# zamling/PSALM

Hardware: AMD Instinct MI355X
Metric: images/sec at 1024x1024 COCO-panoptic inference (higher is better)
Workload: dtype f16x3; 1 GPU; BASELINE.json configs[1]: COCO-panoptic 1024x1024 batch=1 per GPU, PSALM (Swin-B + Phi-1.5 24L + Mask2Former head), 134 class prompts, 100 queries, full semantic+instance+panoptic post-processing; parallelism=image-sharded x1 (replicated weights, RCCL broadcast at init), launch=hipGraph replay (one graph per input signature)

## Files before the change

### include/psalm_hip.h

```cpp
#ifndef PSALM_HIP_H
#define PSALM_HIP_H
#include <stdint.h>
#ifdef __cplusplus
extern "C" {
#endif

#define PSALM_F32 0
#define PSALM_BF16 1

const char* psalm_last_error(void);
#define PSALM_ABI_VERSION 18
int psalm_abi_version(void);
const char* psalm_backend(void);

#define PSALM_TUNE_GEMM_XCD_KSPLIT 0
#define PSALM_TUNE_ATTN_XCD_HEADS 1
#define PSALM_TUNE_GEMM_MID 2
#define PSALM_TUNE_DECODER_FUSE 3
#define PSALM_TUNE_ROW_GROUPS 4
#define PSALM_TUNE_MHA_QTILE_WAVES 5
#define PSALM_TUNE_PHI_ROPE_EPILOGUE 6
#define PSALM_TUNE_COUNT 8
int psalm_set_tuning(int key, int value);
int psalm_get_tuning(int key);

int psalm_msda_forward(const void* value, int value_dtype, const int64_t* spatial_shapes_host,
                       const int64_t* level_start_host, const float* sampling_loc, const float* attn_weight, void* out,
                       int out_dtype, int B, int S, int M, int D, int L, int Lq, int P, void* stream);
int psalm_msda_forward_dev(const void* value, int value_dtype, const int64_t* spatial_shapes_dev, const int64_t* level_start_dev,
                           const float* sampling_loc, const float* attn_weight, void* out, int out_dtype, int B, int S, int M, int D,
                           int L, int Lq, int P, void* stream);


int psalm_msda_fused(const void* value, int value_dtype, const int64_t* spatial_shapes_host,
                     const int64_t* level_start_host, const float* offsets_logits, void* out, int out_dtype, int B, int S,
                     int M, int D, int L, int P, void* stream);
int psalm_msda_set_policy(int v);


int psalm_gemm(const void* A, int a_dtype, long lda, const void* W, int w_dtype, long ldw, const float* bias,
               const void* residual, long ldr, void* C, int c_dtype, long ldc, int M, int N, int K, int act,
               int act_col_start, void* workspace, long workspace_bytes, void* stream);

int psalm_gemm_ln(const void* A, int a_dtype, long lda, const void* W, int w_dtype, long ldw, const float* bias,
                  const void* residual, long ldr, void* C, int c_dtype, long ldc, int M, int N, int K, int act, int act_col_start,
                  const float* ln_gamma, const float* ln_beta, float ln_eps, void* ln_out, int ln_dtype, long ld_ln, void* workspace,
                  long workspace_bytes, void* stream);
int psalm_conv2d_nhwc(const void* x, int B, int H, int W, int Cin, const void* Wt, int Cout, int ksize, int stride, int pad,
                      const float* bias, const void* residual, long ldr, void* out, int c_dtype, long ldc, int act,
                      const void* zeros, void* workspace, long workspace_bytes, void* stream);
int psalm_split_f16(const float* x, long ldx, void* out, long ldo, float* inv_scale, int rows, int K, void* stream);
int psalm_gemm_x3_set_products(int n);
int psalm_im2col_split_f16(const float* x, void* out, float* inv_scale, int B, int H, int W, int C, int k, int stride, int pad, void* stream);
int psalm_layernorm_split(const float* x, long ldx, float* y, long ldy, const float* gamma, const float* beta, int rows, int C, float eps,
                          void* split1, float* inv1, const float* add, long add_rows, void* split2, float* inv2, void* stream);
int psalm_swin_window_gather_split(const float* x, void* out, float* inv_out, const float* gamma, const float* beta, int B, int H, int W, int C,
                                   int ws, int shift, float eps, void* stream);
int psalm_swin_window_merge_ln_split(const float* win, const float* shortcut, float* out_x, void* h_split, float* h_inv, const float* gamma,
                                     const float* beta, int B, int H, int W, int C, int ws, int shift, float eps, void* stream);
int psalm_gemm_x3(const void* A2, long lda, const float* a_scale, const void* W2, long ldw, const float* w_scale, int Kp,
                  const float* bias, const void* residual, long ldr, void* C, long ldc, int M, int N, int act, int act_col_start,
                  void* workspace, long workspace_bytes, void* stream);
int psalm_gemm_x3_ln_split(const void* A2, long lda, const float* a_scale, const void* W2, long ldw, const float* w_scale, int Kp,
                           const float* bias, const void* residual, long ldr, void* C, long ldc, int M, int N, const float* ln_gamma,
                           const float* ln_beta, float ln_eps, void* ln_out, long ld_ln, void* split_out, float* split_inv,
                           void* workspace, long workspace_bytes, void* stream);
int psalm_gemm_x3_split(const void* A2, long lda, const float* a_scale, const void* W2, long ldw, const float* w_scale, int Kp,
                        const float* bias, void* C, long ldc, int M, int N, int act, int act_col_start, void* split_out, long ld_split,
                        int split_kp, int split_col_off, int split_col_start, int paired, float* split_inv, const float* bound_par,
                        int global_rows, void* workspace, long workspace_bytes, void* stream);
typedef struct psalm_rope_out {
    float* Qr;
    float* Kr;
    const float* cos_table;
    const float* sin_table;
    int q_col, k_col, heads, B, L, Lp;
    float scale;
    int pad_;
} psalm_rope_out;
int psalm_gemm_x3_split_rope(const void* A2, long lda, const float* a_scale, const void* W2, long ldw, const float* w_scale, int Kp,
                             const float* bias, void* C, long ldc, int M, int N, int act, int act_col_start, void* split_out, long ld_split,
                             int split_kp, int split_col_off, int split_col_start, int paired, float* split_inv, const float* bound_par,
                             int global_rows, const psalm_rope_out* rope, void* workspace, long workspace_bytes, void* stream);

int psalm_image_preprocess(const unsigned char* img, int H, int W, float* out, unsigned char* pad_mask, int S, int nh, int nw,
                           const int* bounds_h, const int* kk_h, int ksize_h, const int* bounds_v, const int* kk_v, int ksize_v,
                           unsigned char* tmp, const float* mean3_host, const float* std3_host, void* stream);

int psalm_semantic_labels(const float* sem, int* labels, int C, long HW, void* stream);
int psalm_confusion_accumulate(const int* pred, const int* gt, long n, int num_classes, int ignore_label, long long* conf, void* stream);
int psalm_panoptic_rgb(const int* ids, unsigned char* rgb, long n, void* stream);
int psalm_mask_rle_count(const void* masks, int dtype_is_u8, int n, int H, int W, int* col_cnt, int* col_off, int* total, void* stream);
int psalm_mask_rle_emit(const void* masks, int dtype_is_u8, int n, int H, int W, const int* col_off, const long* base, int* out, void* stream);
int psalm_iou_counts(const void* pred, int pred_is_u8, const unsigned char* tgt, const int* pred_idx, const int* tgt_idx, int npairs, long HW,
                     long long* counts_zeroed, void* stream);
int psalm_fuse_masks(const void* masks, int dtype_is_u8, const float* scores, int n, long HW, float thr, unsigned char* out, void* stream);

long psalm_mha_attention_f32_workspace(int B, int heads, int Lq, int Lk);
int psalm_mha_attention_f32(const float* q, long ldq, const float* k, long ldk, const float* v, long ldv, float* out, long ldo,
                            const unsigned char* mask, const unsigned char* row_all_masked, void* workspace, int B, int Lq, int Lk, int heads,
                            int head_dim, void* stream);
long psalm_mha_attention_f32_shared_workspace(int B, int heads, int Lq, int Lk);
int psalm_mha_attention_f32_shared(const float* q, long ldq, const float* k, long ldk, const float* v, long ldv, float* out, long ldo,
                                   const unsigned char* mask, const unsigned char* row_all_masked, void* workspace, int B, int Lq, int Lk,
                                   int heads, int head_dim, void* stream);

long psalm_causal_attention_f32_workspace(int B, int L, int heads);
int psalm_causal_attention_f32(const float* qkv, long ld, int q_off, int k_off, int v_off, float* out, long ldo, int o_off,
                               const float* cos_table, const float* sin_table, const unsigned char* key_mask, void* workspace, int B, int L,
                               int heads, int head_dim, int rot, void* stream);
int psalm_causal_attention_f32_split(const float* qkv, long ld, int q_off, int k_off, int v_off, void* split_out, long ld_split, int split_kp,
                                     int split_col_off, const float* split_inv, const float* cos_table, const float* sin_table,
                                     const unsigned char* key_mask, void* workspace, int B, int L, int heads, int head_dim, int rot,
                                     void* stream);
int psalm_phi_attention_tables(const unsigned char* key_mask, void* workspace, int B, int L, int heads, void* stream);
int psalm_causal_attention_f32_split_prepared(const float* qkv, long ld, int v_off, void* split_out, long ld_split, int split_kp,
                                              int split_col_off, const float* split_inv, void* workspace, int B, int L, int heads,
                                              int head_dim, void* stream);

long psalm_causal_attention_f32_prefix_workspace(int N, int S, int heads);
int psalm_causal_attention_f32_prefix(const float* qkv, long ld, int q_off, int k_off, int v_off, const float* k_cache, const float* v_cache,
                                      long ldv, float* out, long ldo, int o_off, const float* cos_table, const float* sin_table,
                                      const unsigned char* key_mask, void* workspace, int N, int S, int P, int heads, int head_dim, int rot,
                                      void* stream);
int psalm_causal_attention_f32_prefix_split(const float* qkv, long ld, int q_off, int k_off, int v_off, const float* k_cache,
                                            const float* v_cache, long ldv, void* split_out, long ld_split, int split_kp, int split_col_off,
                                            const float* split_inv, const float* cos_table, const float* sin_table,
                                            const unsigned char* key_mask, void* workspace, int N, int S, int P, int heads, int head_dim,
                                            int rot, void* stream);
typedef struct {
    const float* k_cache;
    const float* v_cache;
    long ldv;
    int P;
    int pad;
} psalm_prefix_ref;
long psalm_causal_attention_f32_prefix_grouped_workspace(int N, int S, int heads);
int psalm_causal_attention_f32_prefix_grouped(const float* qkv, long ld, int q_off, int k_off, int v_off, const psalm_prefix_ref* refs, int P_max,
                                              float* out, long ldo, int o_off, const float* cos_table, const float* sin_table,
                                              const unsigned char* key_mask, void* workspace, int N, int S, int heads, int head_dim, int rot,
                                              void* stream);
int psalm_causal_attention_f32_prefix_grouped_split(const float* qkv, long ld, int q_off, int k_off, int v_off, const psalm_prefix_ref* refs,
                                                    int P_max, void* split_out, long ld_split, int split_kp, int split_col_off,
                                                    const float* split_inv, const float* cos_table, const float* sin_table,
                                                    const unsigned char* key_mask, void* workspace, int N, int S, int heads, int head_dim,
                                                    int rot, void* stream);
int psalm_phi_prefix_kv_store(const float* qkv, long ld, int k_off, int v_off, const float* cos_table, const float* sin_table, float* k_cache,
                              float* v_cache, long ldv, int P, int heads, int head_dim, int rot, void* stream);

int psalm_memset_zero(void* p, long bytes, void* stream);
int psalm_copy_d2d(void* dst, const void* src, long bytes, void* stream);
int psalm_cast_i32_i64(const int* src, long long* dst, long n, void* stream);
const char* psalm_gemm_last_kernel(void);
int psalm_gemm_describe(int M, int N, int K, int a_dtype, int w_dtype, long workspace_bytes, int* out4);
int psalm_gemm_set_tile_policy(int bm);

int psalm_layernorm(const void* x, int x_dtype, long ldx, void* y, int y_dtype, long ldy, void* y2_bf16, long ldy2,
                    const float* gamma, const float* beta, int rows, int C, float eps, void* stream);
int psalm_layernorm3(const void* x, int x_dtype, long ldx, void* y, int y_dtype, long ldy, void* y2_bf16, long ldy2, const float* add,
                     long add_rows, void* y3_bf16, long ldy3, const float* gamma, const float* beta, int rows, int C, float eps,
                     void* stream);
int psalm_layernorm_chain(const float* x, long ldx, float* y1, long ldy1, const float* g1, const float* b1, const float* add, long add_rows,
                          float* y2, long ldy2, const float* g2, const float* b2, float* y3, long ldy3, int rows, int C, float eps, void* stream);
int psalm_gemm_f32_pair(const float* A0, const float* W0, const float* bias0, float* C0, int M0, int N0, int K0, int act0, const float* A1,
                        const float* W1, const float* bias1, float* C1, int M1, int N1, int K1, int act1, void* stream);
int psalm_gemm_f32_rows(const float* A, long lda, const float* W, long ldw, const float* bias, const float* residual, long ldr, float* C, long ldc,
                        int M, int N, int K, int act, void* stream);
int psalm_gemm_f32_rows_pair(const float* A0, const float* W0, const float* bias0, float* C0, int M0, int N0, int K0, int act0, const float* A1,
                             const float* W1, const float* bias1, float* C1, int M1, int N1, int K1, int act1, void* stream);
int psalm_gemm_f32_grouped(const float* const* A_host, const float* const* W_host, float* const* C_host, const int* M_host, const int* N_host, int K,
                           int count, void* stream);
int psalm_swin_window_gather(const void* x, int x_dtype, void* out, int out_dtype, const float* gamma,
                             const float* beta, int B, int H, int W, int C, int ws, int shift, float eps, void* stream);
int psalm_swin_window_merge(const void* win, int win_dtype, const void* shortcut, void* out, int x_dtype, int B, int H,
                            int W, int C, int ws, int shift, void* stream);
int psalm_swin_window_merge_ln(const void* win, int win_dtype, const float* shortcut, float* out_x, void* out_h, int h_dtype,
                               const float* gamma, const float* beta, int B, int H, int W, int C, int ws, int shift, float eps,
                               void* stream);
int psalm_patch_merge_ln(const void* x, int x_dtype, void* out, int out_dtype, const float* gamma, const float* beta,
                         int B, int H, int W, int C, float eps, void* stream);
int psalm_groupnorm_nhwc(const void* x, int x_dtype, void* y, int y_dtype, const float* gamma, const float* beta,
                         float* workspace, int B, int HW, int C, int G, float eps, int relu, void* stream);
int psalm_add_bcast(const void* a, int a_dtype, const void* b, int b_dtype, void* out, int out_dtype, long rows, int C,
                    long b_rows, void* stream);
int psalm_gather_rows(const void* src0, int dt0, const void* src1, int dt1, const void* src2, int dt2, const void* src3,
                      int dt3, const int* src_id, const int* src_row, void* dst, int dst_dtype, long rows, int C,
                      void* stream);
int psalm_segment_mean(const void* x, int x_dtype, long ldx, const int* seg_offsets, const int* seg_rows, void* out,
                       int out_dtype, int nseg, int C, void* stream);

// ... 255 lines not shown
```

### psalm_amd/csrc/api.hip

```cpp
#include "common.h"
#include "psalm_hip.h"

#include <atomic>
#include <cstring>

static thread_local char g_err[512] = "";

extern "C" void psalm_set_error(const char* msg) {
    strncpy(g_err, msg ? msg : "", sizeof(g_err) - 1);
    g_err[sizeof(g_err) - 1] = 0;
}
extern "C" const char* psalm_last_error() { return g_err; }
static std::atomic<int> g_tuning[PSALM_TUNE_COUNT] = {{1}, {1}, {1}, {1}, {1}, {1}, {1}, {0}};
extern "C" int psalm_set_tuning(int key, int value) {
    if (key < 0 || key >= PSALM_TUNE_COUNT) { psalm_set_error("psalm_set_tuning: unknown key"); return -1; }
    g_tuning[key].store(value, std::memory_order_relaxed);
    return 0;
}
extern "C" int psalm_get_tuning(int key) {
    if (key < 0 || key >= PSALM_TUNE_COUNT) return 0;
    return g_tuning[key].load(std::memory_order_relaxed);
}
extern "C" int psalm_abi_version() { return PSALM_ABI_VERSION; }
extern "C" const char* psalm_backend() {
#ifdef PSALM_EMU_BUILD
    return "emu";
#else
    return "hip-gfx950";
#endif
}

extern "C" int psalm_memset_zero(void* p, long bytes, void* stream) {
    if (bytes <= 0) return 0;
    PSALM_CHECK_ARG(p != nullptr, "psalm_memset_zero: null pointer");
    hipError_t e = hipMemsetAsync(p, 0, (size_t)bytes, (hipStream_t)stream);
    if (e != hipSuccess) { psalm_set_error("psalm_memset_zero: hipMemsetAsync failed"); return (int)e; }
    return 0;
}
__global__ void cast_i32_i64_kernel(const int* __restrict__ src, long long* __restrict__ dst, long n) {
    const long i = (long)blockIdx.x * blockDim.x + threadIdx.x;
    if (i < n) dst[i] = (long long)src[i];
}
extern "C" int psalm_cast_i32_i64(const int* src, long long* dst, long n, void* stream) {
    if (n <= 0) return 0;
    PSALM_CHECK_ARG(dst != nullptr && src != nullptr, "psalm_cast_i32_i64: null pointer");
    hipLaunchKernelGGL(cast_i32_i64_kernel, dim3((unsigned)((n + 255) / 256)), dim3(256), 0, (hipStream_t)stream, src, dst, n);
    PSALM_LAUNCH_END("psalm_cast_i32_i64");
}
extern "C" int psalm_copy_d2d(void* dst, const void* src, long bytes, void* stream) {
    if (bytes <= 0) return 0;
    PSALM_CHECK_ARG(dst != nullptr && src != nullptr, "psalm_copy_d2d: null pointer");
    hipError_t e = hipMemcpyAsync(dst, src, (size_t)bytes, hipMemcpyDeviceToDevice, (hipStream_t)stream);
    if (e != hipSuccess) { psalm_set_error("psalm_copy_d2d: hipMemcpyAsync failed"); return (int)e; }
    return 0;
}
```

### psalm_amd/csrc/common.h

```cpp
#pragma once
#include <hip/hip_runtime.h>

#include <cstdint>
#include <cstdio>

#define PSALM_F32 0
#define PSALM_BF16 1

typedef unsigned short bf16_t;

__device__ __forceinline__ float bf16_to_f32(bf16_t v) {
    unsigned u = ((unsigned)v) << 16;
    return __builtin_bit_cast(float, u);
}
__device__ __forceinline__ bf16_t f32_to_bf16(float f) {
    unsigned u = __builtin_bit_cast(unsigned, f);
    u += 0x7fffu + ((u >> 16) & 1u);
    return (bf16_t)(u >> 16);
}
typedef float psalm_f32x2_v __attribute__((ext_vector_type(2)));
typedef __bf16 psalm_bf16x2_v __attribute__((ext_vector_type(2)));
__device__ __forceinline__ unsigned pack_bf16x2(float a, float b) {
    const psalm_f32x2_v v = {a, b};
    return __builtin_bit_cast(unsigned, __builtin_convertvector(v, psalm_bf16x2_v));
}
__device__ __forceinline__ float ldf(const float* p) { return *p; }
__device__ __forceinline__ float ldf(const bf16_t* p) { return bf16_to_f32(*p); }
__device__ __forceinline__ void stf(float* p, float v) { *p = v; }
__device__ __forceinline__ void stf(bf16_t* p, float v) { *p = f32_to_bf16(v); }

struct alignas(16) psalm_u32x4 { unsigned x, y, z, w; };
struct alignas(8) psalm_u32x2 { unsigned x, y; };
struct alignas(16) psalm_f32x4 { float x, y, z, w; };
__device__ __forceinline__ void ld8(const float* p, float* d) {
    const psalm_f32x4 a = reinterpret_cast<const psalm_f32x4*>(p)[0], b = reinterpret_cast<const psalm_f32x4*>(p)[1];
    d[0] = a.x; d[1] = a.y; d[2] = a.z; d[3] = a.w; d[4] = b.x; d[5] = b.y; d[6] = b.z; d[7] = b.w;
}
__device__ __forceinline__ void ld8(const bf16_t* p, float* d) {
    const psalm_u32x4 a = *reinterpret_cast<const psalm_u32x4*>(p);
    const unsigned w[4] = {a.x, a.y, a.z, a.w};
#pragma unroll
    for (int i = 0; i < 4; ++i) {
        d[2 * i] = __builtin_bit_cast(float, w[i] << 16);
        d[2 * i + 1] = __builtin_bit_cast(float, w[i] & 0xffff0000u);
    }
}
__device__ __forceinline__ void st8(float* p, const float* v) {
    reinterpret_cast<psalm_f32x4*>(p)[0] = psalm_f32x4{v[0], v[1], v[2], v[3]};
    reinterpret_cast<psalm_f32x4*>(p)[1] = psalm_f32x4{v[4], v[5], v[6], v[7]};
}
__device__ __forceinline__ void st8(bf16_t* p, const float* v) {
    *reinterpret_cast<psalm_u32x4*>(p) =
        psalm_u32x4{pack_bf16x2(v[0], v[1]), pack_bf16x2(v[2], v[3]), pack_bf16x2(v[4], v[5]), pack_bf16x2(v[6], v[7])};
}

__device__ __forceinline__ float wave_sum(float v) {
#pragma unroll
    for (int o = 32; o > 0; o >>= 1) v += __shfl_xor(v, o);
    return v;
}
__device__ __forceinline__ float wave_max(float v) {
#pragma unroll
    for (int o = 32; o > 0; o >>= 1) v = fmaxf(v, __shfl_xor(v, o));
    return v;
}

template <int LPR> __device__ __forceinline__ float seg_sum(float v) {
#pragma unroll
    for (int o = LPR / 2; o > 0; o >>= 1) v += __shfl_xor(v, o);
    return v;
}
template <int LPR> __device__ __forceinline__ float seg_max(float v) {
#pragma unroll
    for (int o = LPR / 2; o > 0; o >>= 1) v = fmaxf(v, __shfl_xor(v, o));
    return v;
}

#ifdef PSALM_EMU_BUILD
#define PSALM_WAVES_PER_EU(n)
#else
#define PSALM_WAVES_PER_EU(n) __attribute__((amdgpu_waves_per_eu(n)))
#endif
#ifdef PSALM_EMU_BUILD
__device__ __forceinline__ void psalm_glds16(const void* g, void* lds_wave_base) { emu::global_load_lds(g, lds_wave_base, 16); }
#else
__device__ __forceinline__ void psalm_glds16(const void* g, void* lds_wave_base) {
    __builtin_amdgcn_global_load_lds((const __attribute__((address_space(1))) void*)g,
                                     (__attribute__((address_space(3))) void*)lds_wave_base, 16, 0, 0);
}
#endif

#ifdef PSALM_EMU_BUILD
#define PSALM_WAIT_VMCNT(N) do { } while (0)
#define PSALM_RAW_BARRIER() __syncthreads()
#define PSALM_SCHED_FENCE() do { } while (0)
#define PSALM_OPAQUE_VGPR(x) do { } while (0)
#define PSALM_OPAQUE_SGPR(x) do { } while (0)
__device__ __forceinline__ float psalm_rcp(float x) { return 1.0f / x; }
__device__ __forceinline__ float psalm_exp2(float x) { return exp2f(x); }
#else
#define PSALM_OPAQUE_VGPR(x) asm volatile("" : "+v"(x))
#define PSALM_OPAQUE_SGPR(x) asm volatile("" : "+s"(x))
#define PSALM_WAIT_VMCNT(N) asm volatile("s_waitcnt vmcnt(" #N ")" ::: "memory")
#define PSALM_RAW_BARRIER() do { asm volatile("s_waitcnt lgkmcnt(0)" ::: "memory"); __builtin_amdgcn_s_barrier(); } while (0)
#define PSALM_SCHED_FENCE() __builtin_amdgcn_sched_barrier(0)
__device__ __forceinline__ float psalm_rcp(float x) { return __builtin_amdgcn_rcpf(x); }
__device__ __forceinline__ float psalm_exp2(float x) { return __builtin_amdgcn_exp2f(x); }
#endif

__device__ __forceinline__ void psalm_split_words(float y, unsigned& hw, unsigned& sw) {
    const _Float16 h = (_Float16)y;
    hw = (unsigned)__builtin_bit_cast(unsigned short, h);
    sw = (unsigned)__builtin_bit_cast(unsigned short, (_Float16)(y - (float)h));
}

#define PSALM_BUF_OOB 0x80000000u
#ifdef PSALM_EMU_BUILD
__device__ __forceinline__ unsigned psalm_swap_adjacent(unsigned v) { return __shfl_xor(v, 1); }
__device__ __forceinline__ unsigned psalm_quad_swap2(unsigned v) { return __shfl_xor(v, 2); }
__device__ __forceinline__ unsigned psalm_swap_row16(unsigned v) { return __shfl_xor(v, 16); }
template <int P> __device__ __forceinline__ unsigned psalm_quad_bcast(unsigned v) { return __shfl(v, ((threadIdx.x & 63) & ~3) | P); }
struct psalm_rsrc { char* base; unsigned bytes; };
__device__ __forceinline__ psalm_rsrc psalm_make_rsrc(const void* p, unsigned bytes) { return psalm_rsrc{(char*)p, bytes}; }
__device__ __forceinline__ void psalm_buf_store_f32(float v, psalm_rsrc r, unsigned off) { if (off < r.bytes && r.bytes - off >= 4u) *reinterpret_cast<float*>(r.base + off) = v; }
__device__ __forceinline__ void psalm_buf_store_u32(unsigned v, psalm_rsrc r, unsigned off) { if (off < r.bytes && r.bytes - off >= 4u) *reinterpret_cast<unsigned*>(r.base + off) = v; }
__device__ __forceinline__ float psalm_buf_load_f32(psalm_rsrc r, unsigned off) { return (off < r.bytes && r.bytes - off >= 4u) ? *reinterpret_cast<const float*>(r.base + off) : 0.f; }
__device__ __forceinline__ psalm_u32x4 psalm_buf_load_b128(psalm_rsrc r, unsigned off) {
    return (off < r.bytes && r.bytes - off >= 16u) ? *reinterpret_cast<const psalm_u32x4*>(r.base + off) : psalm_u32x4{0u, 0u, 0u, 0u};
}
__device__ __forceinline__ void psalm_buf_store_f32_s(float v, psalm_rsrc r, unsigned voff, unsigned soff) { if (voff < PSALM_BUF_OOB) psalm_buf_store_f32(v, r, voff + soff); }
__device__ __forceinline__ float psalm_buf_load_f32_s(psalm_rsrc r, unsigned voff, unsigned soff) { return voff < PSALM_BUF_OOB ? psalm_buf_load_f32(r, voff + soff) : 0.f; }
__device__ __forceinline__ psalm_u32x4 psalm_buf_load_b128_s(psalm_rsrc r, unsigned voff, unsigned soff) {
    return voff < PSALM_BUF_OOB ? psalm_buf_load_b128(r, voff + soff) : psalm_u32x4{0u, 0u, 0u, 0u};
}
#else
__device__ __forceinline__ unsigned psalm_swap_adjacent(unsigned v) {
    return (unsigned)__builtin_amdgcn_mov_dpp((int)v, 0xB1, 0xF, 0xF, true);
}
__device__ __forceinline__ unsigned psalm_quad_swap2(unsigned v) {
    return (unsigned)__builtin_amdgcn_mov_dpp((int)v, 0x4E, 0xF, 0xF, true);
}
__device__ __forceinline__ unsigned psalm_swap_row16(unsigned v) { return (unsigned)__builtin_amdgcn_ds_swizzle((int)v, 0x401F); }
template <int P> __device__ __forceinline__ unsigned psalm_quad_bcast(unsigned v) {
    return (unsigned)__builtin_amdgcn_mov_dpp((int)v, P * 0x55, 0xF, 0xF, true);
}
typedef __amdgpu_buffer_rsrc_t psalm_rsrc;
__device__ __forceinline__ psalm_rsrc psalm_make_rsrc(const void* p, unsigned bytes) {
    return __builtin_amdgcn_make_buffer_rsrc(const_cast<void*>(p), 0, (int)bytes, 0x00020000);
}
__device__ __forceinline__ void psalm_buf_store_f32(float v, psalm_rsrc r, unsigned off) {
    __builtin_amdgcn_raw_buffer_store_b32(__builtin_bit_cast(unsigned, v), r, (int)off, 0, 0);
}
__device__ __forceinline__ void psalm_buf_store_u32(unsigned v, psalm_rsrc r, unsigned off) { __builtin_amdgcn_raw_buffer_store_b32(v, r, (int)off, 0, 0); }
__device__ __forceinline__ float psalm_buf_load_f32(psalm_rsrc r, unsigned off) {
    return __builtin_bit_cast(float, __builtin_amdgcn_raw_buffer_load_b32(r, (int)off, 0, 0));
}
typedef unsigned psalm_u32x4_v __attribute__((ext_vector_type(4)));
__device__ __forceinline__ psalm_u32x4 psalm_buf_load_b128(psalm_rsrc r, unsigned off) {
    const psalm_u32x4_v v = __builtin_amdgcn_raw_buffer_load_b128(r, (int)off, 0, 0);
    return psalm_u32x4{v.x, v.y, v.z, v.w};
}
__device__ __forceinline__ void psalm_buf_store_f32_s(float v, psalm_rsrc r, unsigned voff, unsigned soff) {
    __builtin_amdgcn_raw_buffer_store_b32(__builtin_bit_cast(unsigned, v), r, (int)voff, (int)soff, 0);
}
__device__ __forceinline__ float psalm_buf_load_f32_s(psalm_rsrc r, unsigned voff, unsigned soff) {
    return __builtin_bit_cast(float, __builtin_amdgcn_raw_buffer_load_b32(r, (int)voff, (int)soff, 0));
}
__device__ __forceinline__ psalm_u32x4 psalm_buf_load_b128_s(psalm_rsrc r, unsigned voff, unsigned soff) {
    const psalm_u32x4_v v = __builtin_amdgcn_raw_buffer_load_b128(r, (int)voff, (int)soff, 0);
    return psalm_u32x4{v.x, v.y, v.z, v.w};
}
#endif

__device__ __forceinline__ float psalm_rope_elem(float x, float xo, float cs, float sn, bool neg, bool fused) {
#pragma clang fp contract(off)
    const float t = (neg ? -xo : xo) * sn;
    const float p = x * cs;
    return fused ? fmaf(x, cs, t) : p + t;
}
__device__ __forceinline__ bool psalm_rope_fused_dim(int c) { return (c & 7) < 6; }

extern "C" void psalm_set_error(const char* msg);
extern "C" int psalm_get_tuning(int key);
#ifndef PSALM_TUNE_COUNT
#define PSALM_TUNE_GEMM_XCD_KSPLIT 0
#define PSALM_TUNE_ATTN_XCD_HEADS 1
#define PSALM_TUNE_GEMM_MID 2
#define PSALM_TUNE_DECODER_FUSE 3
#define PSALM_TUNE_ROW_GROUPS 4
#define PSALM_TUNE_MHA_QTILE_WAVES 5
#define PSALM_TUNE_PHI_ROPE_EPILOGUE 6
#define PSALM_TUNE_COUNT 8
#endif

#define PSALM_CHECK_ARG(cond, msg)                                  \
    do {                                                            \
        if (!(cond)) { psalm_set_error(msg); return -1; }           \
    } while (0)

#define PSALM_LAUNCH_END(name)                                      \
    do {                                                            \
        hipError_t e__ = hipGetLastError();                         \
        if (e__ != hipSuccess) {                                    \
            char buf__[256];                                        \
            snprintf(buf__, sizeof(buf__), "%s: launch failed: %s", name, hipGetErrorString(e__)); \
            psalm_set_error(buf__);                                 \
            return (int)e__ ? (int)e__ : -2;                        \
        }                                                           \
        return 0;                                                   \
    } while (0)

#define PSALM_DISPATCH(code, T, ...)                                \
    do {                                                            \
        if ((code) == PSALM_F32) { typedef float T; __VA_ARGS__; }  \
        else if ((code) == PSALM_BF16) { typedef bf16_t T; __VA_ARGS__; } \
        else { psalm_set_error("bad dtype code"); return -1; }      \
    } while (0)

static inline int cdiv(long a, long b) { return (int)((a + b - 1) / b); }
```

### psalm_amd/csrc/msda.hip

```cpp
#include "common.h"
#include <atomic>

struct alignas(16) f32x4_s { float x, y, z, w; };
struct alignas(8) bf16x4_s { bf16_t x, y, z, w; };

__device__ __forceinline__ f32x4_s ld4(const float* p) { return *reinterpret_cast<const f32x4_s*>(p); }
__device__ __forceinline__ f32x4_s ld4(const bf16_t* p) {
    bf16x4_s v = *reinterpret_cast<const bf16x4_s*>(p);
    return f32x4_s{bf16_to_f32(v.x), bf16_to_f32(v.y), bf16_to_f32(v.z), bf16_to_f32(v.w)};
}
__device__ __forceinline__ void st4(float* p, f32x4_s v) { *reinterpret_cast<f32x4_s*>(p) = v; }
__device__ __forceinline__ void st4(bf16_t* p, f32x4_s v) {
    *reinterpret_cast<bf16x4_s*>(p) = bf16x4_s{f32_to_bf16(v.x), f32_to_bf16(v.y), f32_to_bf16(v.z), f32_to_bf16(v.w)};
}

template <int V> struct msda_ic { static constexpr int value = V; };
#define MSDA_MAX_LEVELS 8
struct MsdaLevels {
    int H[MSDA_MAX_LEVELS], W[MSDA_MAX_LEVELS], start[MSDA_MAX_LEVELS];
};

template <typename TV>
__device__ __forceinline__ void msda_sample(const TV* __restrict__ vbase, int Hl, int Wl, int row_stride, float loc_x,
                                            float loc_y, float wgt, f32x4_s& acc) {
    const float h_im = loc_y * Hl - 0.5f;
    const float w_im = loc_x * Wl - 0.5f;
    const bool inb = h_im > -1.f && w_im > -1.f && h_im < (float)Hl && w_im < (float)Wl;
    const int h_low = (int)floorf(inb ? h_im : 0.f), w_low = (int)floorf(inb ? w_im : 0.f);
    const float lh = h_im - h_low, lw = w_im - w_low;
    const float hh = 1.f - lh, hw = 1.f - lw;
    const bool h0 = h_low >= 0, h1 = h_low + 1 <= Hl - 1, w0 = w_low >= 0, w1 = w_low + 1 <= Wl - 1;
    const int ha = max(h_low, 0), hb = min(h_low + 1, Hl - 1), wa = max(w_low, 0), wb = min(w_low + 1, Wl - 1);
    const f32x4_s v1 = ld4(vbase + ((long)ha * Wl + wa) * row_stride);
    const f32x4_s v2 = ld4(vbase + ((long)ha * Wl + wb) * row_stride);
    const f32x4_s v3 = ld4(vbase + ((long)hb * Wl + wa) * row_stride);
    const f32x4_s v4 = ld4(vbase + ((long)hb * Wl + wb) * row_stride);
    const float w1c = (inb && h0 && w0) ? hh * hw : 0.f, w2c = (inb && h0 && w1) ? hh * lw : 0.f;
    const float w3c = (inb && h1 && w0) ? lh * hw : 0.f, w4c = (inb && h1 && w1) ? lh * lw : 0.f;
    const float wg = inb ? wgt : 0.f;
    acc.x += wg * (w1c * v1.x + w2c * v2.x + w3c * v3.x + w4c * v4.x);
    acc.y += wg * (w1c * v1.y + w2c * v2.y + w3c * v3.y + w4c * v4.y);
    acc.z += wg * (w1c * v1.z + w2c * v2.z + w3c * v3.z + w4c * v4.z);
    acc.w += wg * (w1c * v1.w + w2c * v2.w + w3c * v3.w + w4c * v4.w);
}

template <typename TV>
struct MsdaTaps8 {
    const TV* p[4];
    float w[4];
};
template <typename TV>
__device__ __forceinline__ MsdaTaps8<TV> msda_taps8(const TV* __restrict__ vbase, int Hl, int Wl, int row_stride, float loc_x, float loc_y) {
    const float h_im = loc_y * Hl - 0.5f;
    const float w_im = loc_x * Wl - 0.5f;
    const bool inb = h_im > -1.f && w_im > -1.f && h_im < (float)Hl && w_im < (float)Wl;
    const int h_low = (int)floorf(inb ? h_im : 0.f), w_low = (int)floorf(inb ? w_im : 0.f);
    const float lh = h_im - h_low, lw = w_im - w_low;
    const float hh = 1.f - lh, hw = 1.f - lw;
    const bool h0 = h_low >= 0, h1 = h_low + 1 <= Hl - 1, w0 = w_low >= 0, w1 = w_low + 1 <= Wl - 1;
    const int ha = max(h_low, 0), hb = min(h_low + 1, Hl - 1), wa = max(w_low, 0), wb = min(w_low + 1, Wl - 1);
    MsdaTaps8<TV> t;
    t.p[0] = vbase + ((long)ha * Wl + wa) * row_stride;
    t.p[1] = vbase + ((long)ha * Wl + wb) * row_stride;
    t.p[2] = vbase + ((long)hb * Wl + wa) * row_stride;
    t.p[3] = vbase + ((long)hb * Wl + wb) * row_stride;
    t.w[0] = (inb && h0 && w0) ? hh * hw : 0.f;
    t.w[1] = (inb && h0 && w1) ? hh * lw : 0.f;
    t.w[2] = (inb && h1 && w0) ? lh * hw : 0.f;
    t.w[3] = (inb && h1 && w1) ? lh * lw : 0.f;
    return t;
}

template <typename TV, typename TO, int L, int P, bool XCD_BANDS = false, bool QUAD = false>
__global__ void __launch_bounds__(256) msda_fused8_kernel(const TV* __restrict__ value, MsdaLevels lv,
                                                          const float* __restrict__ ow, TO* __restrict__ out, int B, int S,
                                                          int M, int D) {
    const int G = D >> 3;
    const int Lq = S;
    const long total = (long)B * Lq * M * G;
    constexpr int LP = L * P;
    for (long idx0 = (long)blockIdx.x * blockDim.x + threadIdx.x; idx0 < total; idx0 += (long)gridDim.x * blockDim.x) {
        long idx = idx0;
        if constexpr (XCD_BANDS)
            idx = ((long)(blockIdx.x >> 3) * blockDim.x + threadIdx.x);
        const int g = (int)(idx % G);
        long t = idx / G;
        const int m = (int)(t % M);
        t /= M;
        int q = (int)(t % Lq);
        const int b = XCD_BANDS ? 0 : (int)(t / Lq);
        if constexpr (XCD_BANDS) {
            const int band = blockIdx.x & 7;
            int r = (int)t, lq_ = 0, base = 0;
#pragma unroll
            for (int l = 0; l < L; ++l) {
                const int nb = lv.H[l] * lv.W[l] / 8;
                if (l == lq_ && r >= nb && l + 1 < L) { r -= nb; ++lq_; }
            }
#pragma unroll
            for (int l = 0; l < L; ++l)
                if (l == lq_) base = lv.start[l] + band * (lv.H[l] * lv.W[l] / 8);
            q = base + r;
        }
        int lq = 0;
#pragma unroll
        for (int l = 1; l < L; ++l)
            if (q >= lv.start[l]) lq = l;
        const int qi = q - lv.start[lq];
        const float ref_x = ((qi % lv.W[lq]) + 0.5f) / lv.W[lq];
        const float ref_y = ((qi / lv.W[lq]) + 0.5f) / lv.H[lq];
        const float* row = ow + ((long)b * Lq + q) * (M * LP * 3);
        const float* offp = row + m * LP * 2;
        const float* lgp = row + M * LP * 2 + m * LP;
        const int row_stride = M * D;
        const TV* vb = value + (long)b * S * row_stride + m * D + g * 8;
        float acc[8];
#pragma unroll
        for (int k = 0; k < 8; ++k) acc[k] = 0.f;
        if constexpr (QUAD) {
            static_assert(P == 4, "one sampling point per lane of the quad");
            float lgq[L];
            float mx = -3.4e38f;
#pragma unroll
            for (int l = 0; l < L; ++l) { lgq[l] = lgp[l * P + g]; mx = fmaxf(mx, lgq[l]); }
            mx = fmaxf(mx, __builtin_bit_cast(float, psalm_swap_adjacent(__builtin_bit_cast(unsigned, mx))));
            mx = fmaxf(mx, __builtin_bit_cast(float, psalm_quad_swap2(__builtin_bit_cast(unsigned, mx))));
            float den = 0.f;
#pragma unroll
            for (int l = 0; l < L; ++l) { lgq[l] = __expf(lgq[l] - mx); den += lgq[l]; }
            den += __builtin_bit_cast(float, psalm_swap_adjacent(__builtin_bit_cast(unsigned, den)));
            den += __builtin_bit_cast(float, psalm_quad_swap2(__builtin_bit_cast(unsigned, den)));
            const float inv = 1.f / den;
            const psalm_rsrc vr = psalm_make_rsrc(value, (unsigned)((long)B * S * row_stride * (long)sizeof(TV)));
            const unsigned lane_b = (unsigned)(((long)b * S * row_stride + m * D + g * 8) * (long)sizeof(TV));
            auto fetch = [&](unsigned off, float* v8) {
                if constexpr (sizeof(TV) == 4) {
                    const psalm_u32x4 a = psalm_buf_load_b128(vr, lane_b + off), b2 = psalm_buf_load_b128(vr, lane_b + off + 16u);
                    v8[0] = __builtin_bit_cast(float, a.x); v8[1] = __builtin_bit_cast(float, a.y); v8[2] = __builtin_bit_cast(float, a.z);
                    v8[3] = __builtin_bit_cast(float, a.w); v8[4] = __builtin_bit_cast(float, b2.x); v8[5] = __builtin_bit_cast(float, b2.y);
                    v8[6] = __builtin_bit_cast(float, b2.z); v8[7] = __builtin_bit_cast(float, b2.w);
                } else {
                    const psalm_u32x4 a = psalm_buf_load_b128(vr, lane_b + off);
                    const unsigned w4[4] = {a.x, a.y, a.z, a.w};
#pragma unroll
                    for (int e = 0; e < 4; ++e) {
                        v8[2 * e] = __builtin_bit_cast(float, w4[e] << 16);
                        v8[2 * e + 1] = __builtin_bit_cast(float, w4[e] & 0xffff0000u);
                    }
                }
            };
#pragma unroll 1
            for (int l = 0; l < L; ++l) {
                int Hl = lv.H[0], Wl = lv.W[0], sl = lv.start[0];
                float lgl = lgq[0];
#pragma unroll
                for (int j = 1; j < L; ++j)
                    if (l == j) { Hl = lv.H[j]; Wl = lv.W[j]; sl = lv.start[j]; lgl = lgq[j]; }
                const int i = l * P + g;
                const float lx = ref_x + offp[2 * i] / Wl, ly = ref_y + offp[2 * i + 1] / Hl;
                const MsdaTaps8<TV> tp = msda_taps8<TV>(vb + (long)sl * row_stride, Hl, Wl, row_stride, lx, ly);
                const float wgt = lgl * inv;
                unsigned toff[4];
                float tw[4];
#pragma unroll
                for (int c = 0; c < 4; ++c) { toff[c] = (unsigned)((tp.p[c] - vb) * (long)sizeof(TV)); tw[c] = tp.w[c] * wgt; }
                auto pair = [&](auto PC0) {
                    constexpr int p0 = decltype(PC0)::value;
                    float w[2][4], v[2][4][8];
#pragma unroll
                    for (int c = 0; c < 4; ++c) {
                        fetch(psalm_quad_bcast<p0>(toff[c]), v[0][c]);
                        fetch(psalm_quad_bcast<p0 + 1>(toff[c]), v[1][c]);
                        w[0][c] = __builtin_bit_cast(float, psalm_quad_bcast<p0>(__builtin_bit_cast(unsigned, tw[c])));
                        w[1][c] = __builtin_bit_cast(float, psalm_quad_bcast<p0 + 1>(__builtin_bit_cast(unsigned, tw[c])));
                    }
#pragma unroll
                    for (int pp = 0; pp < 2; ++pp)
#pragma unroll
                        for (int k = 0; k < 8; ++k)
                            acc[k] += w[pp][0] * v[pp][0][k] + w[pp][1] * v[pp][1][k] + w[pp][2] * v[pp][2][k] + w[pp][3] * v[pp][3][k];
                };
                pair(msda_ic<0>{});
                pair(msda_ic<2>{});
            }
            static_assert(L <= 3, "levels of the quad form");
            st8(out + (((long)b * Lq + q) * M + m) * D + g * 8, acc);
            continue;
        }
        float lg[LP];
        float mx = -3.4e38f;
#pragma unroll
        for (int i = 0; i < LP; ++i) { lg[i] = lgp[i]; mx = fmaxf(mx, lg[i]); }
        float den = 0.f;
#pragma unroll
        for (int i = 0; i < LP; ++i) { lg[i] = __expf(lg[i] - mx); den += lg[i]; }
        const float inv = 1.f / den;
        constexpr int PB = (P % 2 == 0) ? 2 : 1;
#pragma unroll 1
        for (int l = 0; l < L; ++l) {
            int Hl = lv.H[0], Wl = lv.W[0], sl = lv.start[0];
#pragma unroll
            for (int j = 1; j < L; ++j)
                if (l == j) { Hl = lv.H[j]; Wl = lv.W[j]; sl = lv.start[j]; }
            const TV* vl = vb + (long)sl * row_stride;
#pragma unroll
            for (int p0 = 0; p0 < P; p0 += PB) {
                MsdaTaps8<TV> tp[PB];
                float v[PB][4][8];
#pragma unroll
                for (int pp = 0; pp < PB; ++pp) {
                    const int i = l * P + p0 + pp;
                    const float lx = ref_x + offp[2 * i] / Wl;
                    const float ly = ref_y + offp[2 * i + 1] / Hl;
                    tp[pp] = msda_taps8<TV>(vl, Hl, Wl, row_stride, lx, ly);
#pragma unroll
                    for (int c = 0; c < 4; ++c) ld8(tp[pp].p[c], v[pp][c]);
                }
                __builtin_amdgcn_sched_barrier(0);
#pragma unroll
                for (int pp = 0; pp < PB; ++pp) {
                    const float wgt = lg[l * P + p0 + pp] * inv;
#pragma unroll
                    for (int k = 0; k < 8; ++k)
                        acc[k] += wgt * (tp[pp].w[0] * v[pp][0][k] + tp[pp].w[1] * v[pp][1][k] + tp[pp].w[2] * v[pp][2][k] +
                                         tp[pp].w[3] * v[pp][3][k]);
                }
            }
        }
        st8(out + (((long)b * Lq + q) * M + m) * D + g * 8, acc);
    }
}

template <typename TV, typename TO, int LP_UNROLL, bool DEV = false>
__global__ void __launch_bounds__(256) msda_forward_kernel(const TV* __restrict__ value, MsdaLevels lv,
                                                           const float* __restrict__ loc, const float* __restrict__ attw,
                                                           TO* __restrict__ out, int B, int S, int M, int D, int L, int Lq,
                                                           int P, const long* __restrict__ shapes_dev = nullptr,
                                                           const long* __restrict__ starts_dev = nullptr) {
    const int G = D >> 2;
    const long total = (long)B * Lq * M * G;
    for (long idx = (long)blockIdx.x * blockDim.x + threadIdx.x; idx < total; idx += (long)gridDim.x * blockDim.x) {
        const int g = (int)(idx % G);
        long t = idx / G;
        const int m = (int)(t % M);
        t /= M;
        const int q = (int)(t % Lq);
        const int b = (int)(t / Lq);
        const long qm = ((long)b * Lq + q) * M + m;
        const float* lp = loc + qm * L * P * 2;
        const float* wp = attw + qm * L * P;
        const int row_stride = M * D;
        const TV* vb = value + (long)b * S * row_stride + m * D + g * 4;
        f32x4_s acc{0.f, 0.f, 0.f, 0.f};
        for (int l = 0; l < L; ++l) {
            const int Hl = DEV ? (int)shapes_dev[2 * l] : lv.H[l], Wl = DEV ? (int)shapes_dev[2 * l + 1] : lv.W[l];
            const long sl = DEV ? starts_dev[l] : (long)lv.start[l];
            if (DEV && !(Hl > 0 && Wl > 0 && sl >= 0 && sl + (long)Hl * Wl <= (long)S)) continue;
            const TV* vl = vb + sl * row_stride;
#pragma unroll LP_UNROLL
            for (int p = 0; p < P; ++p) {
                const int i = l * P + p;
                msda_sample<TV>(vl, Hl, Wl, row_stride, lp[2 * i], lp[2 * i + 1], wp[i], acc);
            }
        }
        st4(out + qm * D + g * 4, acc);
    }
}

template <typename TV, typename TO, int L, int P>
__global__ void __launch_bounds__(256) msda_fused_kernel(const TV* __restrict__ value, MsdaLevels lv,
                                                         const float* __restrict__ ow, TO* __restrict__ out, int B, int S,
                                                         int M, int D) {
    const int G = D >> 2;
    const int Lq = S;
    const long total = (long)B * Lq * M * G;
    constexpr int LP = L * P;
    for (long idx = (long)blockIdx.x * blockDim.x + threadIdx.x; idx < total; idx += (long)gridDim.x * blockDim.x) {
        const int g = (int)(idx % G);
        long t = idx / G;
        const int m = (int)(t % M);
        t /= M;
        const int q = (int)(t % Lq);
        const int b = (int)(t / Lq);
        int lq = 0;
#pragma unroll
        for (int l = 1; l < L; ++l)
            if (q >= lv.start[l]) lq = l;
        const int qi = q - lv.start[lq];
        const float ref_x = ((qi % lv.W[lq]) + 0.5f) / lv.W[lq];
        const float ref_y = ((qi / lv.W[lq]) + 0.5f) / lv.H[lq];
        const float* row = ow + ((long)b * Lq + q) * (M * LP * 3);
        const float* offp = row + m * LP * 2;
        const float* lgp = row + M * LP * 2 + m * LP;
        float lg[LP];
        float mx = -3.4e38f;
#pragma unroll
        for (int i = 0; i < LP; ++i) { lg[i] = lgp[i]; mx = fmaxf(mx, lg[i]); }
        float den = 0.f;
#pragma unroll
        for (int i = 0; i < LP; ++i) { lg[i] = __expf(lg[i] - mx); den += lg[i]; }
        const float inv = 1.f / den;
        const int row_stride = M * D;
        const TV* vb = value + (long)b * S * row_stride + m * D + g * 4;
        f32x4_s acc{0.f, 0.f, 0.f, 0.f};
#pragma unroll
        for (int l = 0; l < L; ++l) {
            const TV* vl = vb + (long)lv.start[l] * row_stride;
#pragma unroll
            for (int p = 0; p < P; ++p) {
                const int i = l * P + p;
                const float lx = ref_x + offp[2 * i] / lv.W[l];
                const float ly = ref_y + offp[2 * i + 1] / lv.H[l];
                msda_sample<TV>(vl, lv.H[l], lv.W[l], row_stride, lx, ly, lg[i] * inv, acc);
            }
        }
        st4(out + (((long)b * Lq + q) * M + m) * D + g * 4, acc);
    }
}

static std::atomic<int> g_msda_quad{1};
extern "C" int psalm_msda_set_policy(int v) {
    if (v != 0 && v != 1) { psalm_set_error("psalm_msda_set_policy: 0 / 1 (quad-shared taps off / on)"); return -1; }
    g_msda_quad = v;
    return 0;
}

static int fill_levels(MsdaLevels& lv, const int64_t* shapes, const int64_t* starts, int L, int S) {
    if (L > MSDA_MAX_LEVELS) return -1;
    long tot = 0;
    for (int l = 0; l < L; ++l) {
        lv.H[l] = (int)shapes[2 * l];
        lv.W[l] = (int)shapes[2 * l + 1];
        lv.start[l] = (int)starts[l];
        tot += (long)lv.H[l] * lv.W[l];
    }
    return tot == S ? 0 : -2;
}

extern "C" int psalm_msda_forward(const void* value, int value_dtype, const int64_t* spatial_shapes_host,
                                  const int64_t* level_start_host, const float* sampling_loc, const float* attn_weight,
                                  void* out, int out_dtype, int B, int S, int M, int D, int L, int Lq, int P, void* stream) {
    PSALM_CHECK_ARG(D % 4 == 0 && D > 0, "psalm_msda_forward: head dim must be a multiple of 4");
    MsdaLevels lv = {};
    int rc = fill_levels(lv, spatial_shapes_host, level_start_host, L, S);
    PSALM_CHECK_ARG(rc != -1, "psalm_msda_forward: too many levels (max 8)");
    PSALM_CHECK_ARG(rc == 0, "psalm_msda_forward: sum(H_l*W_l) != S");
    const long total = (long)B * Lq * M * (D / 4);
    if (total == 0) return 0;
    const int block = 256;
    const int grid = (int)((total + block - 1) / block < 65536 * 8 ? (total + block - 1) / block : 65536 * 8);
    PSALM_DISPATCH(value_dtype, TV, PSALM_DISPATCH(out_dtype, TO, {
        hipLaunchKernelGGL((msda_forward_kernel<TV, TO, 4>), dim3(grid), dim3(block), 0, (hipStream_t)stream,
                           (const TV*)value, lv, sampling_loc, attn_weight, (TO*)out, B, S, M, D, L, Lq, P);
    }));
    PSALM_LAUNCH_END("psalm_msda_forward");
}

extern "C" int psalm_msda_forward_dev(const void* value, int value_dtype, const int64_t* spatial_shapes_dev,
                                      const int64_t* level_start_dev, const float* sampling_loc, const float* attn_weight, void* out,
                                      int out_dtype, int B, int S, int M, int D, int L, int Lq, int P, void* stream) {
    PSALM_CHECK_ARG(D % 4 == 0 && D > 0, "psalm_msda_forward_dev: head dim must be a multiple of 4");
    PSALM_CHECK_ARG(L >= 1 && spatial_shapes_dev && level_start_dev, "psalm_msda_forward_dev: level table missing");
    MsdaLevels lv = {};
    const long total = (long)B * Lq * M * (D / 4);
    if (total == 0) return 0;
    const int block = 256;
    const int grid = (int)((total + block - 1) / block < 65536 * 8 ? (total + block - 1) / block : 65536 * 8);
    PSALM_DISPATCH(value_dtype, TV, PSALM_DISPATCH(out_dtype, TO, {
        hipLaunchKernelGGL((msda_forward_kernel<TV, TO, 4, true>), dim3(grid), dim3(block), 0, (hipStream_t)stream,
                           (const TV*)value, lv, sampling_loc, attn_weight, (TO*)out, B, S, M, D, L, Lq, P,
                           (const long*)spatial_shapes_dev, (const long*)level_start_dev);
    }));
    PSALM_LAUNCH_END("psalm_msda_forward_dev");
}

extern "C" int psalm_msda_fused(const void* value, int value_dtype, const int64_t* spatial_shapes_host,
                                const int64_t* level_start_host, const float* offsets_logits, void* out, int out_dtype,
                                int B, int S, int M, int D, int L, int P, void* stream) {
    PSALM_CHECK_ARG(D % 4 == 0 && D > 0, "psalm_msda_fused: head dim must be a multiple of 4");
    PSALM_CHECK_ARG(L == 3 && P == 4, "psalm_msda_fused: specialised for L=3 levels, P=4 points (PSALM pixel decoder)");
    MsdaLevels lv = {};
    int rc = fill_levels(lv, spatial_shapes_host, level_start_host, L, S);
    PSALM_CHECK_ARG(rc == 0, "psalm_msda_fused: bad level table");
    const int block = 256;
    if (D % 8 == 0 && (uintptr_t)value % 16 == 0 && (uintptr_t)out % 16 == 0) {
        const long total8 = (long)B * S * M * (D / 8);
        if (total8 == 0) return 0;
        bool bands = B == 1 && total8 % (block * 8) == 0;
        for (int l = 0; l < L; ++l) bands = bands && lv.H[l] % 8 == 0;
        const bool quad = g_msda_quad && D == 32 && value_dtype == PSALM_BF16 && (long)B * S * M * D * 2 < (1L << 31);
#define MSDA_LAUNCH8(BANDS_, QUAD_, GRID_)                                                                                              \
        PSALM_DISPATCH(value_dtype, TV, PSALM_DISPATCH(out_dtype, TO, {                                                                 \
            hipLaunchKernelGGL((msda_fused8_kernel<TV, TO, 3, 4, BANDS_, QUAD_>), dim3((unsigned)(GRID_)), dim3(block), 0,              \
                               (hipStream_t)stream, (const TV*)value, lv, offsets_logits, (TO*)out, B, S, M, D);                        \
        }))
        if (bands) {
            if (quad) MSDA_LAUNCH8(true, true, total8 / block); else MSDA_LAUNCH8(true, false, total8 / block);
            PSALM_LAUNCH_END("psalm_msda_fused");
        }
        if (quad) MSDA_LAUNCH8(false, true, (total8 + block - 1) / block); else MSDA_LAUNCH8(false, false, (total8 + block - 1) / block);
#undef MSDA_LAUNCH8
        PSALM_LAUNCH_END("psalm_msda_fused");
    }
    const long total = (long)B * S * M * (D / 4);
    if (total == 0) return 0;
    const int grid = (int)((total + block - 1) / block);
    PSALM_DISPATCH(value_dtype, TV, PSALM_DISPATCH(out_dtype, TO, {
        hipLaunchKernelGGL((msda_fused_kernel<TV, TO, 3, 4>), dim3(grid), dim3(block), 0, (hipStream_t)stream,
                           (const TV*)value, lv, offsets_logits, (TO*)out, B, S, M, D);
    }));
    PSALM_LAUNCH_END("psalm_msda_fused");
}
```

### psalm_amd/csrc/rowops.hip

```cpp
#include "common.h"
#include <type_traits>

__device__ __forceinline__ void emit_split8(const float* o8, float sc, unsigned short* hi_dst, unsigned short* lo_dst) {
    unsigned hw[4], lw[4];
#pragma unroll
    for (int k = 0; k < 4; ++k) {
        unsigned h0, h1, l0, l1;
        psalm_split_words(o8[2 * k] * sc, h0, l0);
        psalm_split_words(o8[2 * k + 1] * sc, h1, l1);
        hw[k] = h0 | (h1 << 16);
        lw[k] = l0 | (l1 << 16);
    }
    *reinterpret_cast<psalm_u32x4*>(hi_dst) = psalm_u32x4{hw[0], hw[1], hw[2], hw[3]};
    *reinterpret_cast<psalm_u32x4*>(lo_dst) = psalm_u32x4{lw[0], lw[1], lw[2], lw[3]};
}
__device__ __forceinline__ void split_scale(float amax, float& sc, float& inv) {
    int e = (int)((__builtin_bit_cast(unsigned, amax) >> 23) & 0xffu) - 127;
    int se = 13 - e;
    se = se > 100 ? 100 : (se < -100 ? -100 : se);
    const bool zero = !(amax > 0.f) || !(amax < 3.0e38f);
    sc = zero ? 1.f : __builtin_bit_cast(float, (unsigned)(127 + se) << 23);
    inv = zero ? 1.f : __builtin_bit_cast(float, (unsigned)(127 - se) << 23);
}
template <typename TI>
__device__ __forceinline__ void row_stats(const TI* __restrict__ x, int C, int lane, float eps, float& mean, float& rstd) {
    float s = 0.f;
    for (int c = lane; c < C; c += 64) s += ldf(x + c);
    mean = wave_sum(s) / C;
    float v = 0.f;
    for (int c = lane; c < C; c += 64) { const float d = ldf(x + c) - mean; v += d * d; }
    rstd = rsqrtf(wave_sum(v) / C + eps);
}

template <typename TI, typename TO>
__global__ void __launch_bounds__(256) layernorm_kernel(const TI* __restrict__ x, long ldx, TO* __restrict__ y, long ldy,
                                                        bf16_t* __restrict__ y2, long ldy2, const float* __restrict__ add, long add_rows,
                                                        bf16_t* __restrict__ y3, long ldy3, const float* __restrict__ gamma,
                                                        const float* __restrict__ beta, int rows, int C, float eps) {
    const int lane = threadIdx.x & 63;
    const long row = (long)blockIdx.x * 4 + (threadIdx.x >> 6);
    if (row >= rows) return;
    const TI* xr = x + row * ldx;
    float mean, rstd;
    row_stats(xr, C, lane, eps, mean, rstd);
    TO* yr = y + row * ldy;
    for (int c = lane; c < C; c += 64) {
        const float v = (ldf(xr + c) - mean) * rstd * gamma[c] + beta[c];
        stf(yr + c, v);
        if (y2) y2[row * ldy2 + c] = f32_to_bf16(v);
        if (y3) y3[row * ldy3 + c] = f32_to_bf16(v + add[(row % add_rows) * C + c]);
    }
}

template <typename TI, typename TO>
__global__ void __launch_bounds__(256) layernorm_vec_kernel(const TI* __restrict__ x, long ldx, TO* __restrict__ y, long ldy,
                                                            bf16_t* __restrict__ y2, long ldy2, const float* __restrict__ add,
                                                            long add_rows, bf16_t* __restrict__ y3, long ldy3,
                                                            const float* __restrict__ gamma, const float* __restrict__ beta, int rows,
                                                            int C, float eps) {
    const int lane = threadIdx.x & 63;
    const long row = (long)blockIdx.x * 4 + (threadIdx.x >> 6);
    if (row >= rows) return;
    const TI* xr = x + row * ldx;
    float v[4][8];
    float s = 0.f;
#pragma unroll
    for (int i = 0; i < 4; ++i) {
        const int c = (i * 64 + lane) * 8;
        if (c < C) {
            ld8(xr + c, v[i]);
#pragma unroll
            for (int k = 0; k < 8; ++k) s += v[i][k];
        }
    }
    const float mean = wave_sum(s) / C;
    float q = 0.f;
#pragma unroll
    for (int i = 0; i < 4; ++i) {
        const int c = (i * 64 + lane) * 8;
        if (c < C) {
#pragma unroll
            for (int k = 0; k < 8; ++k) { const float d = v[i][k] - mean; q += d * d; }
        }
    }
    const float rstd = rsqrtf(wave_sum(q) / C + eps);
#pragma unroll
    for (int i = 0; i < 4; ++i) {
        const int c = (i * 64 + lane) * 8;
        if (c < C) {
            float g8[8], b8[8], o8[8];
            ld8(gamma + c, g8);
            ld8(beta + c, b8);
#pragma unroll
            for (int k = 0; k < 8; ++k) o8[k] = (v[i][k] - mean) * rstd * g8[k] + b8[k];
            st8(y + row * ldy + c, o8);
            if (y2) st8(y2 + row * ldy2 + c, o8);
            if (y3) {
                float a8[8];
                ld8(add + (row % add_rows) * C + c, a8);
#pragma unroll
                for (int k = 0; k < 8; ++k) o8[k] += a8[k];
                st8(y3 + row * ldy3 + c, o8);
            }
        }
    }
}

extern "C" int psalm_layernorm3(const void* x, int x_dtype, long ldx, void* y, int y_dtype, long ldy, void* y2_bf16, long ldy2,
                                const float* add, long add_rows, void* y3_bf16, long ldy3, const float* gamma, const float* beta,
                                int rows, int C, float eps, void* stream) {
    if (rows == 0) return 0;
    const long xs = x_dtype == PSALM_F32 ? 4 : 2, ys = y_dtype == PSALM_F32 ? 4 : 2;
    PSALM_CHECK_ARG(!y3_bf16 || (add && add_rows > 0), "psalm_layernorm3: y3 needs the `add` table");
    const bool vec = C % 8 == 0 && C <= 2048 && (uintptr_t)x % 16 == 0 && (ldx * xs) % 16 == 0 && (uintptr_t)y % 16 == 0 &&
                     (ldy * ys) % 16 == 0 && (uintptr_t)gamma % 16 == 0 && (uintptr_t)beta % 16 == 0 &&
                     (!y2_bf16 || ((uintptr_t)y2_bf16 % 16 == 0 && (ldy2 * 2) % 16 == 0)) &&
                     (!y3_bf16 || ((uintptr_t)y3_bf16 % 16 == 0 && (ldy3 * 2) % 16 == 0 && (uintptr_t)add % 16 == 0));
    PSALM_DISPATCH(x_dtype, TI, PSALM_DISPATCH(y_dtype, TO, {
        if (vec)
            hipLaunchKernelGGL((layernorm_vec_kernel<TI, TO>), dim3(cdiv(rows, 4)), dim3(256), 0, (hipStream_t)stream,
                               (const TI*)x, ldx, (TO*)y, ldy, (bf16_t*)y2_bf16, ldy2, add, add_rows, (bf16_t*)y3_bf16, ldy3, gamma, beta,
                               rows, C, eps);
        else
            hipLaunchKernelGGL((layernorm_kernel<TI, TO>), dim3(cdiv(rows, 4)), dim3(256), 0, (hipStream_t)stream,
                               (const TI*)x, ldx, (TO*)y, ldy, (bf16_t*)y2_bf16, ldy2, add, add_rows, (bf16_t*)y3_bf16, ldy3, gamma, beta,
                               rows, C, eps);
    }));
    PSALM_LAUNCH_END("psalm_layernorm");
}

__global__ void __launch_bounds__(256) layernorm_chain_kernel(const float* __restrict__ x, long ldx, float* __restrict__ y1, long ldy1,
                                                              const float* __restrict__ g1, const float* __restrict__ b1,
                                                              const float* __restrict__ add, long add_rows, float* __restrict__ y2, long ldy2,
                                                              const float* __restrict__ g2, const float* __restrict__ b2, float* __restrict__ y3,
                                                              long ldy3, int rows, int C, float eps) {
    const int lane = threadIdx.x & 63;
    const long row = (long)blockIdx.x * 4 + (threadIdx.x >> 6);
    if (row >= rows) return;
    const float* xr = x + row * ldx;
    float v[4][8];
    auto stats = [&](float& mean, float& rstd) {
        float s = 0.f;
#pragma unroll
        for (int i = 0; i < 4; ++i) {
            const int c = (i * 64 + lane) * 8;
            if (c < C) {
#pragma unroll
                for (int k = 0; k < 8; ++k) s += v[i][k];
            }
        }
        mean = wave_sum(s) / C;
        float q = 0.f;
#pragma unroll
        for (int i = 0; i < 4; ++i) {
            const int c = (i * 64 + lane) * 8;
            if (c < C) {
#pragma unroll
                for (int k = 0; k < 8; ++k) { const float d = v[i][k] - mean; q += d * d; }
            }
        }
        rstd = rsqrtf(wave_sum(q) / C + eps);
    };
#pragma unroll
    for (int i = 0; i < 4; ++i) {
        const int c = (i * 64 + lane) * 8;
        if (c < C) ld8(xr + c, v[i]);
    }
    float mean, rstd;
    stats(mean, rstd);
#pragma unroll
    for (int i = 0; i < 4; ++i) {
        const int c = (i * 64 + lane) * 8;
        if (c < C) {
            float g8[8], b8[8];
            ld8(g1 + c, g8);
            ld8(b1 + c, b8);
// ... 386 lines not shown
}
extern "C" int psalm_swin_window_gather_split(const float* x, void* out, float* inv_out, const float* gamma, const float* beta, int B, int H,
                                              int W, int C, int ws, int shift, float eps, void* stream) {
    const long rows = (long)B * ((H + ws - 1) / ws) * ((W + ws - 1) / ws) * ws * ws;
    if (rows == 0) return 0;
    PSALM_CHECK_ARG(C % 8 == 0 && C <= 2048 && (uintptr_t)x % 16 == 0 && (uintptr_t)out % 16 == 0, "psalm_swin_window_gather_split: C % 8 == 0, C <= 2048, aligned");
#define WGS_LAUNCH(LPR_) hipLaunchKernelGGL((swin_window_gather_split_kernel<LPR_>), dim3(cdiv(rows, 4 * (64 / LPR_))), dim3(256), 0, (hipStream_t)stream, x, \
                                            (unsigned short*)out, inv_out, gamma, beta, B, H, W, C, ws, shift, eps, (C + 63) / 64 * 64)
    const int lpr = !psalm_get_tuning(PSALM_TUNE_ROW_GROUPS) ? 64 : (C <= 128 ? 16 : (C <= 256 ? 32 : 64));
    if (lpr == 16) WGS_LAUNCH(16); else if (lpr == 32) WGS_LAUNCH(32); else WGS_LAUNCH(64);
#undef WGS_LAUNCH
    PSALM_LAUNCH_END("psalm_swin_window_gather_split");
}

template <typename TI, typename TO>
__global__ void __launch_bounds__(256) patch_merge_ln_kernel(const TI* __restrict__ x, TO* __restrict__ out,
                                                             const float* __restrict__ gamma, const float* __restrict__ beta,
                                                             int B, int H, int W, int C, float eps) {
    const int lane = threadIdx.x & 63;
    const int H2 = (H + 1) / 2, W2 = (W + 1) / 2;
    const long rows = (long)B * H2 * W2;
    const long r = (long)blockIdx.x * 4 + (threadIdx.x >> 6);
    if (r >= rows) return;
    const int x2 = (int)(r % W2), y2 = (int)((r / W2) % H2), b = (int)(r / ((long)W2 * H2));
    const int C4 = 4 * C;
    auto get = [&](int c4) -> float {
        const int blk = c4 / C, c = c4 % C;
        const int y = 2 * y2 + (blk & 1), xx = 2 * x2 + (blk >> 1);
        return (y < H && xx < W) ? ldf(x + (((long)b * H + y) * W + xx) * C + c) : 0.f;
    };
    float s = 0.f;
    for (int c = lane; c < C4; c += 64) s += get(c);
    const float mean = wave_sum(s) / C4;
    float v = 0.f;
    for (int c = lane; c < C4; c += 64) { const float d = get(c) - mean; v = fmaf(d, d, v); }
    const float rstd = rsqrtf(wave_sum(v) / C4 + eps);
    TO* o = out + r * C4;
    for (int c = lane; c < C4; c += 64) stf(o + c, fmaf((get(c) - mean) * rstd, gamma[c], beta[c]));
}

template <int NJ>
__global__ void __launch_bounds__(256) patch_merge_ln_regs_kernel(const float* __restrict__ x, float* __restrict__ out, const float* __restrict__ gamma,
                                                                  const float* __restrict__ beta, int B, int H, int W, float eps) {
    constexpr int C4 = 64 * NJ, C = C4 / 4;
    const int lane = threadIdx.x & 63;
    const int H2 = (H + 1) / 2, W2 = (W + 1) / 2;
    const long rows = (long)B * H2 * W2;
    const long r = (long)blockIdx.x * 4 + (threadIdx.x >> 6);
    if (r >= rows) return;
    const int x2 = (int)(r % W2), y2 = (int)((r / W2) % H2), b = (int)(r / ((long)W2 * H2));
    float val[NJ];
#pragma unroll
    for (int j = 0; j < NJ; ++j) {
        const int blk = (64 * j) / C, c = (64 * j) % C + lane;
        const int y = 2 * y2 + (blk & 1), xx = 2 * x2 + (blk >> 1);
        val[j] = (y < H && xx < W) ? x[(((long)b * H + y) * W + xx) * C + c] : 0.f;
    }
    float s = 0.f;
#pragma unroll
    for (int j = 0; j < NJ; ++j) s += val[j];
    const float mean = wave_sum(s) / C4;
    float v = 0.f;
#pragma unroll
    for (int j = 0; j < NJ; ++j) { const float d = val[j] - mean; v = fmaf(d, d, v); }
    const float rstd = rsqrtf(wave_sum(v) / C4 + eps);
    float* o = out + r * C4;
#pragma unroll
    for (int j = 0; j < NJ; ++j) o[lane + 64 * j] = fmaf((val[j] - mean) * rstd, gamma[lane + 64 * j], beta[lane + 64 * j]);
}

extern "C" int psalm_patch_merge_ln(const void* x, int x_dtype, void* out, int out_dtype, const float* gamma,
                                    const float* beta, int B, int H, int W, int C, float eps, void* stream) {
    const long rows = (long)B * ((H + 1) / 2) * ((W + 1) / 2);
    if (rows == 0) return 0;
    if (x_dtype == PSALM_F32 && out_dtype == PSALM_F32 && (C == 128 || C == 256 || C == 512) && psalm_get_tuning(PSALM_TUNE_ROW_GROUPS)) {
#define PML_LAUNCH(NJ_) hipLaunchKernelGGL((patch_merge_ln_regs_kernel<NJ_>), dim3(cdiv(rows, 4)), dim3(256), 0, (hipStream_t)stream, (const float*)x, (float*)out, \
                                           gamma, beta, B, H, W, eps)
        if (C == 128) PML_LAUNCH(8); else if (C == 256) PML_LAUNCH(16); else PML_LAUNCH(32);
#undef PML_LAUNCH
        PSALM_LAUNCH_END("psalm_patch_merge_ln");
    }
    PSALM_DISPATCH(x_dtype, TI, PSALM_DISPATCH(out_dtype, TO, {
        hipLaunchKernelGGL((patch_merge_ln_kernel<TI, TO>), dim3(cdiv(rows, 4)), dim3(256), 0, (hipStream_t)stream,
                           (const TI*)x, (TO*)out, gamma, beta, B, H, W, C, eps);
    }));
    PSALM_LAUNCH_END("psalm_patch_merge_ln");
}

template <typename TI>
__global__ void __launch_bounds__(256) groupnorm_stats_kernel(const TI* __restrict__ x, float* __restrict__ partial, int HW,
                                                              int C, int G, int rows_per_chunk, int nchunks) {
    __shared__ float ssum[256], ssq[256];
    const int b = blockIdx.y, chunk = blockIdx.x, tid = threadIdx.x;
    const int cpg = C / G;
    const int r0 = chunk * rows_per_chunk;
    const int r1 = min(HW, r0 + rows_per_chunk);
    for (int c0 = 0; c0 < C; c0 += 256) {
        const int c = c0 + tid;
        float s = 0.f, q = 0.f;
        if (c < C)
            for (int r = r0; r < r1; ++r) { const float v = ldf(x + ((long)b * HW + r) * C + c); s += v; q += v * v; }
        ssum[tid] = s;
        ssq[tid] = q;
        __syncthreads();
        if (c < C && (c % cpg) == 0) {
            float gs = 0.f, gq = 0.f;
            for (int i = 0; i < cpg; ++i) { gs += ssum[tid + i]; gq += ssq[tid + i]; }
            float* p = partial + (((long)b * nchunks + chunk) * G + c / cpg) * 2;
            p[0] = gs;
            p[1] = gq;
        }
        __syncthreads();
    }
}

__global__ void __launch_bounds__(64) groupnorm_finalize_kernel(const float* __restrict__ partial, float* __restrict__ stats,
                                                                int HW, int C, int G, int nchunks, float eps) {
    const int g = blockIdx.x, b = blockIdx.y, lane = threadIdx.x;
    double s = 0.0, q = 0.0;
    for (int k = lane; k < nchunks; k += 64) {
        const float* p = partial + (((long)b * nchunks + k) * G + g) * 2;
        s += p[0];
        q += p[1];
    }
#pragma unroll
    for (int o = 32; o > 0; o >>= 1) { s += __shfl_xor(s, o); q += __shfl_xor(q, o); }
    if (lane == 0) {
        const double n = (double)HW * (C / G);
        const double m = s / n;
        double var = q / n - m * m;
        if (var < 0) var = 0;
        stats[((long)b * G + g) * 2] = (float)m;
        stats[((long)b * G + g) * 2 + 1] = (float)(1.0 / sqrt(var + (double)eps));
    }
}

template <typename TI, typename TO>
__global__ void __launch_bounds__(256) groupnorm_apply_kernel(const TI* __restrict__ x, TO* __restrict__ y,
                                                              const float* __restrict__ stats,
                                                              const float* __restrict__ gamma, const float* __restrict__ beta,
                                                              int HW, int C, int G, int relu) {
    const int b = blockIdx.y;
    const int cpg = C / G;
    const long total8 = (long)HW * C / 8;
    for (long i = (long)blockIdx.x * 256 + threadIdx.x; i < total8; i += (long)gridDim.x * 256) {
        const long e = i * 8;
        const int c0 = (int)(e % C);
        float v[8];
        ld8(x + (long)b * HW * C + e, v);
#pragma unroll
        for (int k = 0; k < 8; ++k) {
            const int c = c0 + k, g = c / cpg;
            const float m = stats[((long)b * G + g) * 2], r = stats[((long)b * G + g) * 2 + 1];
            float o = (v[k] - m) * r * gamma[c] + beta[c];
            if (relu) o = fmaxf(o, 0.f);
            v[k] = o;
        }
        st8(y + (long)b * HW * C + e, v);
    }
}

extern "C" int psalm_groupnorm_nhwc(const void* x, int x_dtype, void* y, int y_dtype, const float* gamma, const float* beta,
                                    float* workspace, int B, int HW, int C, int G, float eps, int relu, void* stream) {
    if (B == 0 || HW == 0) return 0;
    PSALM_CHECK_ARG(G <= 256 && C % G == 0 && C % 8 == 0, "psalm_groupnorm_nhwc: need G <= 256, C % G == 0, C % 8 == 0");
    PSALM_CHECK_ARG((uintptr_t)x % 16 == 0 && (uintptr_t)y % 16 == 0, "psalm_groupnorm_nhwc: 16-byte aligned tensors");
    const int rows_per_chunk = 64;
    const int nchunks = cdiv(HW, rows_per_chunk);
    float* stats = workspace + (long)B * nchunks * G * 2;
    hipStream_t s = (hipStream_t)stream;
    PSALM_DISPATCH(x_dtype, TI, {
        hipLaunchKernelGGL((groupnorm_stats_kernel<TI>), dim3(nchunks, B), dim3(256), 0, s, (const TI*)x, workspace, HW, C, G,
                           rows_per_chunk, nchunks);
    });
    hipLaunchKernelGGL(groupnorm_finalize_kernel, dim3(G, B), dim3(64), 0, s, workspace, stats, HW, C, G, nchunks, eps);
    long gx = ((long)HW * C / 8 + 255) / 256;
    if (gx > 8192) gx = 8192;
    PSALM_DISPATCH(x_dtype, TI, PSALM_DISPATCH(y_dtype, TO, {
        hipLaunchKernelGGL((groupnorm_apply_kernel<TI, TO>), dim3((unsigned)(gx < 1 ? 1 : gx), B), dim3(256), 0, s, (const TI*)x,
                           (TO*)y, stats, gamma, beta, HW, C, G, relu);
    }));
    PSALM_LAUNCH_END("psalm_groupnorm_nhwc");
}

template <typename TA, typename TB, typename TO>
__global__ void __launch_bounds__(256) add_bcast_kernel(const TA* __restrict__ a, const TB* __restrict__ b, TO* __restrict__ out,
                                                        long rows, int C, long b_rows) {
    const long total = rows * C;
    for (long i = (long)blockIdx.x * 256 + threadIdx.x; i < total; i += (long)gridDim.x * 256) {
        const long r = i / C;
        const int c = (int)(i % C);
        stf(out + i, ldf(a + i) + ldf(b + (r % b_rows) * C + c));
    }
}

extern "C" int psalm_add_bcast(const void* a, int a_dtype, const void* b, int b_dtype, void* out, int out_dtype, long rows,
                               int C, long b_rows, void* stream) {
    if (rows == 0) return 0;
    const long total = rows * C;
    const int grid = (int)((total + 2047) / 2048);
    PSALM_DISPATCH(a_dtype, TA, PSALM_DISPATCH(b_dtype, TB, PSALM_DISPATCH(out_dtype, TO, {
        hipLaunchKernelGGL((add_bcast_kernel<TA, TB, TO>), dim3(grid), dim3(256), 0, (hipStream_t)stream, (const TA*)a,
                           (const TB*)b, (TO*)out, rows, C, b_rows);
    })));
    PSALM_LAUNCH_END("psalm_add_bcast");
}

struct GatherSrc { const void* p[4]; int dtype[4]; };
template <typename TO>
__global__ void __launch_bounds__(256) gather_rows_kernel(GatherSrc src, const int* __restrict__ src_id,
                                                          const int* __restrict__ src_row, TO* __restrict__ dst, long rows,
                                                          int C) {
    const int lane = threadIdx.x & 63;
    const long r = (long)blockIdx.x * 4 + (threadIdx.x >> 6);
    if (r >= rows) return;
    const int id = src_id[r];
    TO* o = dst + r * C;
    if (id < 0) {
        for (int c = lane; c < C; c += 64) stf(o + c, 0.f);
    } else if (src.dtype[id] == PSALM_F32) {
        const float* s = (const float*)src.p[id] + (long)src_row[r] * C;
        for (int c = lane; c < C; c += 64) stf(o + c, s[c]);
    } else {
        const bf16_t* s = (const bf16_t*)src.p[id] + (long)src_row[r] * C;
        for (int c = lane; c < C; c += 64) stf(o + c, bf16_to_f32(s[c]));
    }
}

extern "C" int psalm_gather_rows(const void* src0, int dt0, const void* src1, int dt1, const void* src2, int dt2,
                                 const void* src3, int dt3, const int* src_id, const int* src_row, void* dst, int dst_dtype,
                                 long rows, int C, void* stream) {
    if (rows == 0) return 0;
    GatherSrc s;
    s.p[0] = src0; s.p[1] = src1; s.p[2] = src2; s.p[3] = src3;
    s.dtype[0] = dt0; s.dtype[1] = dt1; s.dtype[2] = dt2; s.dtype[3] = dt3;
    PSALM_DISPATCH(dst_dtype, TO, {
        hipLaunchKernelGGL((gather_rows_kernel<TO>), dim3(cdiv(rows, 4)), dim3(256), 0, (hipStream_t)stream, s, src_id,
                           src_row, (TO*)dst, rows, C);
    });
    PSALM_LAUNCH_END("psalm_gather_rows");
}

template <typename TI, typename TO>
__global__ void __launch_bounds__(256) segment_mean_kernel(const TI* __restrict__ x, long ldx, const int* __restrict__ off,
                                                           const int* __restrict__ rows, TO* __restrict__ out, int nseg,
                                                           int C) {
    const int lane = threadIdx.x & 63;
    const int s = blockIdx.x * 4 + (threadIdx.x >> 6);
    if (s >= nseg) return;
    const int i0 = off[s], i1 = off[s + 1];
    const float inv = i1 > i0 ? 1.f / (i1 - i0) : 0.f;
    if constexpr (std::is_same<TI, float>::value) {
        if (C % 256 == 0 && C <= 4096 && ldx % 4 == 0 && (uintptr_t)x % 16 == 0) {
            float acc[16][4];
            const int nv = C / 256;
#pragma unroll
            for (int v = 0; v < 16; ++v) acc[v][0] = acc[v][1] = acc[v][2] = acc[v][3] = 0.f;
            for (int i = i0; i < i1; ++i) {
                const float* xr = x + (long)rows[i] * ldx + lane * 4;
                psalm_f32x4 t[16];
#pragma unroll
                for (int v = 0; v < 16; ++v)
                    if (v < nv) t[v] = *reinterpret_cast<const psalm_f32x4*>(xr + v * 256);
#pragma unroll
                for (int v = 0; v < 16; ++v)
                    if (v < nv) { acc[v][0] += t[v].x; acc[v][1] += t[v].y; acc[v][2] += t[v].z; acc[v][3] += t[v].w; }
            }
#pragma unroll
            for (int v = 0; v < 16; ++v)
                if (v < nv) {
#pragma unroll
                    for (int k = 0; k < 4; ++k) stf(out + (long)s * C + v * 256 + lane * 4 + k, acc[v][k] * inv);
                }
            return;
        }
    }
    for (int c = lane; c < C; c += 64) {
        float acc = 0.f;
        for (int i = i0; i < i1; ++i) acc += ldf(x + (long)rows[i] * ldx + c);
        stf(out + (long)s * C + c, acc * inv);
    }
}

extern "C" int psalm_segment_mean(const void* x, int x_dtype, long ldx, const int* seg_offsets, const int* seg_rows, void* out,
                                  int out_dtype, int nseg, int C, void* stream) {
    if (nseg == 0) return 0;
    PSALM_DISPATCH(x_dtype, TI, PSALM_DISPATCH(out_dtype, TO, {
        hipLaunchKernelGGL((segment_mean_kernel<TI, TO>), dim3(cdiv(nseg, 4)), dim3(256), 0, (hipStream_t)stream,
                           (const TI*)x, ldx, seg_offsets, seg_rows, (TO*)out, nseg, C);
    }));
    PSALM_LAUNCH_END("psalm_segment_mean");
}
```

### psalm_amd/csrc/stages.hip

```cpp
#include "common.h"
#include "psalm_hip.h"

static inline long al256(long v) { return (v + 255) / 256 * 256; }

struct PhiLayout {
    long x0, x1, h, hinv, big, a2, inv2, attn, total;
    int Kp;
};
static PhiLayout phi_layout(const psalm_phi_desc* d, int B, int L) {
    PhiLayout o;
    const long M = (long)B * L, H = d->hidden, I = d->intermediate;
    o.Kp = (int)((H + 63) / 64 * 64);
    long p = 0;
    o.x0 = p; p += al256(M * H * 4);
    o.x1 = p; p += al256(M * H * 4);
    o.h = p; p += al256(M * 2 * o.Kp * 2);
    o.hinv = p; p += al256(M * 4);
    o.big = p; p += al256(M * 3 * H * 4);
    o.a2 = p; p += al256(M * 2 * (H + I) * 2);
    o.inv2 = p; p += al256(M * 4);
    o.attn = p; p += al256(psalm_causal_attention_f32_workspace(B, L, d->heads));
    o.total = p;
    return o;
}
// ... 365 lines not shown
            PSALM_CHECK_ARG(st->ds_w && st->ds_ws && st->ds_g && st->ds_b, "psalm_swin_forward: downsample weights missing");
            const int M2 = (int)g.rows[s + 1], K = 4 * C, Kq = c64(K), C2 = g.C[s + 1];
            SW(psalm_patch_merge_ln(x, PSALM_F32, cols, PSALM_F32, st->ds_g, st->ds_b, B, Hc, Wc, C, eps, stream));
            SW(psalm_split_f16(cols, K, colsp, 2L * Kq, colsinv, M2, K, stream));
            float* xn = X[(cur + 1) % 3];
            SW(psalm_gemm_x3(colsp, 2L * Kq, colsinv, st->ds_w, 2L * Kq, st->ds_ws, Kq, nullptr, nullptr, 0, xn, C2, M2, C2, 0, 0, gemm_workspace,
                             gemm_workspace_bytes, stream));
            cur = (cur + 1) % 3;
        }
    }
#undef SW
    return 0;
}

struct ProjLayout { long colsA, invA, y1, colsB, invB, y2, ds, y3, y3p, y3inv, total; int ho, wo; };
static ProjLayout proj_layout(const psalm_projector_desc* d, int B, int h, int w) {
    ProjLayout o;
    o.ho = (h + 2 - 3) / 2 + 1; o.wo = (w + 2 - 3) / 2 + 1;
    const long Mi = (long)B * o.ho * o.wo, Cin = d->in_dim, Cm = d->mid_dim;
    long p = 0;
    o.colsA = p; p += al256(Mi * 2 * c64((int)(9 * Cin)) * 2);
    o.invA = p; p += al256(Mi * 4);
    o.y1 = p; p += al256(Mi * Cm * 4);
    o.colsB = p; p += al256(Mi * 2 * c64((int)(9 * Cm)) * 2);
    o.invB = p; p += al256(Mi * 4);
    o.y2 = p; p += al256(Mi * Cm * 4);
    o.ds = p; p += al256(Mi * Cm * 4);
    o.y3 = p; p += al256(Mi * Cm * 4);
    o.y3p = p; p += al256(Mi * 2 * c64((int)Cm) * 2);
    o.y3inv = p; p += al256(Mi * 4);
    o.total = p;
    return o;
}
extern "C" long psalm_projector_forward_workspace(const psalm_projector_desc* d, int B, int h, int w) {
    if (!d || B <= 0 || h <= 0 || w <= 0 || d->in_dim % 8 || d->mid_dim % 8) return -1;
    return proj_layout(d, B, h, w).total;
}
extern "C" int psalm_projector_forward(const psalm_projector_desc* d, const float* res5, int B, int h, int w, float* out, void* workspace,
                                       long workspace_bytes, void* gemm_workspace, long gemm_workspace_bytes, void* stream) {
    PSALM_CHECK_ARG(d && res5 && out && workspace && B > 0 && d->in_dim % 8 == 0 && d->mid_dim % 8 == 0, "psalm_projector_forward: arguments (channel counts multiples of 8)");
    const ProjLayout lo = proj_layout(d, B, h, w);
    PSALM_CHECK_ARG(workspace_bytes >= lo.total && (uintptr_t)workspace % 256 == 0, "psalm_projector_forward: workspace of psalm_projector_forward_workspace() bytes, 256-byte aligned");
    char* ws = (char*)workspace;
    const int Mi = B * lo.ho * lo.wo, Cin = d->in_dim, Cm = d->mid_dim, KA = 9 * Cin, KB = 9 * Cm;
    void* colsA = ws + lo.colsA; float* invA = (float*)(ws + lo.invA);
    void* colsB = ws + lo.colsB; float* invB = (float*)(ws + lo.invB);
    float* y1 = (float*)(ws + lo.y1); float* y2 = (float*)(ws + lo.y2); float* ds = (float*)(ws + lo.ds); float* y3 = (float*)(ws + lo.y3);
    void* y3p = ws + lo.y3p; float* y3inv = (float*)(ws + lo.y3inv);
    int rc;
#define PJ(call) do { rc = (call); if (rc) return rc; } while (0)
    PJ(psalm_im2col_split_f16(res5, colsA, invA, B, h, w, Cin, 3, 2, 1, stream));
    PJ(psalm_gemm_x3(colsA, 2L * c64(KA), invA, d->c1_w, 2L * c64(KA), d->c1_ws, c64(KA), d->c1_b, nullptr, 0, y1, Cm, Mi, Cm,  1, 0, gemm_workspace, gemm_workspace_bytes, stream));
    PJ(psalm_im2col_split_f16(y1, colsB, invB, B, lo.ho, lo.wo, Cm, 3, 1, 1, stream));
    PJ(psalm_gemm_x3(colsB, 2L * c64(KB), invB, d->c2_w, 2L * c64(KB), d->c2_ws, c64(KB), nullptr, nullptr, 0, y2, Cm, Mi, Cm, 0, 0, gemm_workspace, gemm_workspace_bytes, stream));
    PJ(psalm_im2col_split_f16(res5, colsA, invA, B, h, w, Cin, 1, 2, 0, stream));
    PJ(psalm_gemm_x3(colsA, 2L * c64(Cin), invA, d->ds_w, 2L * c64(Cin), d->ds_ws, c64(Cin), d->ds_b, nullptr, 0, ds, Cm, Mi, Cm, 0, 0, gemm_workspace, gemm_workspace_bytes, stream));
    PJ(psalm_im2col_split_f16(y2, colsB, invB, B, lo.ho, lo.wo, Cm, 3, 1, 1, stream));
    PJ(psalm_gemm_x3(colsB, 2L * c64(KB), invB, d->c2f_w, 2L * c64(KB), d->c2f_ws, c64(KB), d->c2f_b, ds, Cm, y3, Cm, Mi, Cm,  1 | 16, 0,
                     gemm_workspace, gemm_workspace_bytes, stream));
    PJ(psalm_split_f16(y3, Cm, y3p, 2L * c64(Cm), y3inv, Mi, Cm, stream));
    PJ(psalm_gemm_x3(y3p, 2L * c64(Cm), y3inv, d->fc_w, 2L * c64(Cm), d->fc_ws, c64(Cm), d->fc_b, nullptr, 0, out, d->out_dim, Mi, d->out_dim, 0, 0, gemm_workspace,
                     gemm_workspace_bytes, stream));
#undef PJ
    return 0;
}

struct PdGeom { int h[4], w[4]; long start[3], S, HW2; };
static PdGeom pd_geom(const int* hw_host) {
    PdGeom g;
    for (int i = 0; i < 4; ++i) { g.h[i] = hw_host[2 * i]; g.w[i] = hw_host[2 * i + 1]; }
    g.start[0] = 0;
    g.start[1] = (long)g.h[3] * g.w[3];
    g.start[2] = g.start[1] + (long)g.h[2] * g.w[2];
    g.S = g.start[2] + (long)g.h[1] * g.w[1];
    g.HW2 = (long)g.h[0] * g.w[0];
    return g;
}
struct PdLayout { long tokp, tokinv, t, gnws, src[2], x1, sp1, inv1, sp2, inv2, sp3, inv3, qin, value, ow, att, hdd, hddinv, lat, lat2, y, cols, colsinv, y2, total; };
static PdLayout pd_layout(const psalm_pd_desc* d, const PdGeom& g) {
    const long D = d->D, S = g.S, HW2 = g.HW2, KpD = c64((int)D), Kf = c64(d->ffn);
    long mtok = 0, mrows = 0;
    for (int i = 0; i < 4; ++i) {
        const long r = (long)g.h[i] * g.w[i];
        mtok = std::max(mtok, r * 2 * c64(d->in_dims[i]) * 2);
        mrows = std::max(mrows, r);
    }
    mrows = std::max(mrows, S);
    PdLayout o;
    long p = 0;
    o.tokp = p; p += al256(mtok);
    o.tokinv = p; p += al256(mrows * 4);
    o.t = p; p += al256(std::max(S, HW2) * D * 4);
    o.gnws = p; p += al256((std::max(S, HW2) / 64 + 2) * (long)d->G * 2 * 4);
    o.src[0] = p; p += al256(S * D * 4);
    o.src[1] = p; p += al256(S * D * 4);
    o.x1 = p; p += al256(S * D * 4);
    o.sp1 = p; p += al256(S * 2 * KpD * 2); o.inv1 = p; p += al256(S * 4);
    o.sp2 = p; p += al256(S * 2 * KpD * 2); o.inv2 = p; p += al256(S * 4);
    o.sp3 = p; p += al256(S * 2 * KpD * 2); o.inv3 = p; p += al256(S * 4);
    o.qin = p; p += al256(S * D * 4);
    o.value = p; p += al256(S * D * 4);
    o.ow = p; p += al256(S * (long)d->M * 3 * 4 * 3 * 4);
    o.att = p; p += al256(S * D * 4);
    o.hdd = p; p += al256(S * 2 * Kf * 2); o.hddinv = p; p += al256(S * 4);
    o.lat = p; p += al256(HW2 * D * 4);
    o.lat2 = p; p += al256(HW2 * D * 4);
    o.y = p; p += al256(HW2 * D * 4);
    o.cols = p; p += al256(HW2 * 2 * c64((int)(9 * D)) * 2); o.colsinv = p; p += al256(HW2 * 4);
    o.y2 = p; p += al256(HW2 * D * 4);
    o.total = p;
    return o;
}
static int pd_check(const psalm_pd_desc* d) {
    PSALM_CHECK_ARG(d && d->layers && d->num_layers >= 1 && d->D % 8 == 0 && d->D <= 2048 && d->D == d->M * 32 && d->ffn % 8 == 0 && d->mask_dim % 8 == 0,
                    "psalm_pixel_decoder_forward: descriptor (D = 32 * heads, multiples of 8)");
    for (int i = 0; i < 4; ++i) PSALM_CHECK_ARG(d->in_dims[i] % 8 == 0, "psalm_pixel_decoder_forward: input channel counts multiples of 8");
    return 0;
}
extern "C" long psalm_pixel_decoder_forward_workspace(const psalm_pd_desc* d, const int* hw_host) {
    if (pd_check(d) != 0 || !hw_host) return -1;
    return pd_layout(d, pd_geom(hw_host)).total;
}
extern "C" int psalm_pixel_decoder_forward(const psalm_pd_desc* d, const float* const* feats_host, const int* hw_host, const float* lvl_pos,
                                           float* mask_features, float* ms_out, void* workspace, long workspace_bytes, void* gemm_workspace,
                                           long gemm_workspace_bytes, void* stream) {
    if (pd_check(d) != 0) return -1;
    PSALM_CHECK_ARG(feats_host && hw_host && lvl_pos && mask_features && ms_out && workspace, "psalm_pixel_decoder_forward: null argument");
    const PdGeom g = pd_geom(hw_host);
    const PdLayout lo = pd_layout(d, g);
    PSALM_CHECK_ARG(workspace_bytes >= lo.total && (uintptr_t)workspace % 256 == 0, "psalm_pixel_decoder_forward: workspace of psalm_pixel_decoder_forward_workspace() bytes, 256-byte aligned");
    char* ws = (char*)workspace;
    const int D = d->D, S = (int)g.S, HW2 = (int)g.HW2, KpD = c64(D), F = d->ffn, Kf = c64(F), NOW = d->M * 3 * 4 * 3;
    const float eps = 1e-5f;
    void* tokp = ws + lo.tokp; float* tokinv = (float*)(ws + lo.tokinv);
    float* t = (float*)(ws + lo.t); float* gnws = (float*)(ws + lo.gnws);
    float* src[2] = {(float*)(ws + lo.src[0]), (float*)(ws + lo.src[1])};
    float* x1 = (float*)(ws + lo.x1);
    void* sp1 = ws + lo.sp1; float* inv1 = (float*)(ws + lo.inv1);
    void* sp2 = ws + lo.sp2; float* inv2 = (float*)(ws + lo.inv2);
    void* sp3 = ws + lo.sp3; float* inv3 = (float*)(ws + lo.inv3);
    float* qin = (float*)(ws + lo.qin); float* value = (float*)(ws + lo.value); float* ow = (float*)(ws + lo.ow); float* att = (float*)(ws + lo.att);
    void* hdd = ws + lo.hdd; float* hddinv = (float*)(ws + lo.hddinv);
    float* lat = (float*)(ws + lo.lat); float* lat2 = (float*)(ws + lo.lat2); float* y = (float*)(ws + lo.y); float* y2 = (float*)(ws + lo.y2);
    void* cols = ws + lo.cols; float* colsinv = (float*)(ws + lo.colsinv);
    int rc;
#define PD(call) do { rc = (call); if (rc) return rc; } while (0)
    float* s0 = src[0];
    for (int l = 0; l < 3; ++l) {
        const int fi = 3 - l, hwl = g.h[fi] * g.w[fi], Cin = d->in_dims[fi], Kp = c64(Cin);
        PD(psalm_split_f16(feats_host[fi], Cin, tokp, 2L * Kp, tokinv, hwl, Cin, stream));
        PD(psalm_gemm_x3(tokp, 2L * Kp, tokinv, d->ip_w[l], 2L * Kp, d->ip_ws[l], Kp, d->ip_b[l], nullptr, 0, t, D, hwl, D, 0, 0, gemm_workspace, gemm_workspace_bytes, stream));
        PD(psalm_groupnorm_nhwc(t, PSALM_F32, s0 + g.start[l] * D, PSALM_F32, d->ip_gn_g[l], d->ip_gn_b[l], gnws, 1, hwl, D, d->G, eps, 0, stream));
    }
    PD(psalm_add_bcast(s0, PSALM_F32, lvl_pos, PSALM_F32, qin, PSALM_F32, S, D, S, stream));
    const int64_t shapes[6] = {g.h[3], g.w[3], g.h[2], g.w[2], g.h[1], g.w[1]};
    const int64_t starts[3] = {g.start[0], g.start[1], g.start[2]};
    int cur = 0;
    for (int i = 0; i < d->num_layers; ++i) {
        const psalm_pd_enc_layer* ly = &d->layers[i];
        const bool more = i + 1 < d->num_layers;
        float* sc = src[cur];
        float* sn = src[cur ^ 1];
        if (i == 0) {
            PD(psalm_split_f16(sc, D, sp2, 2L * KpD, inv2, S, D, stream));
            PD(psalm_gemm_x3(sp2, 2L * KpD, inv2, ly->value_w, 2L * KpD, ly->value_ws, KpD, ly->value_b, nullptr, 0, value, D, S, D, 0, 0, gemm_workspace, gemm_workspace_bytes, stream));
            PD(psalm_split_f16(qin, D, sp3, 2L * KpD, inv3, S, D, stream));
            PD(psalm_gemm_x3(sp3, 2L * KpD, inv3, ly->ow_w, 2L * KpD, ly->ow_ws, KpD, ly->ow_b, nullptr, 0, ow, NOW, S, NOW, 0, 0, gemm_workspace, gemm_workspace_bytes, stream));
        } else {
            PD(psalm_gemm_x3(sp2, 2L * KpD, inv2, ly->value_w, 2L * KpD, ly->value_ws, KpD, ly->value_b, nullptr, 0, value, D, S, D, 0, 0, gemm_workspace, gemm_workspace_bytes, stream));
            PD(psalm_gemm_x3(sp3, 2L * KpD, inv3, ly->ow_w, 2L * KpD, ly->ow_ws, KpD, ly->ow_b, nullptr, 0, ow, NOW, S, NOW, 0, 0, gemm_workspace, gemm_workspace_bytes, stream));
        }
        PD(psalm_msda_fused(value, PSALM_F32, shapes, starts, ow, att, PSALM_F32, 1, S, d->M, 32, 3, 4, stream));
        PD(psalm_split_f16(att, D, sp1, 2L * KpD, inv1, S, D, stream));
        PD(psalm_gemm_x3(sp1, 2L * KpD, inv1, ly->out_w, 2L * KpD, ly->out_ws, KpD, ly->out_b, sc, D, x1, D, S, D, 0, 0, gemm_workspace, gemm_workspace_bytes, stream));
        PD(psalm_layernorm_split(x1, D, sn, D, ly->n1_g, ly->n1_b, S, D, eps, sp1, inv1, nullptr, 0, nullptr, nullptr, stream));
        if (Kf != F) PD(psalm_memset_zero(hdd, (long)S * 2 * Kf * 2, stream));
        PD(psalm_gemm_x3_split(sp1, 2L * KpD, inv1, ly->l1_w, 2L * KpD, ly->l1_ws, KpD, ly->l1_b, nullptr, 0, S, F,  1, 0, hdd, 2L * Kf, Kf, 0, 0, ly->l1_paired, hddinv,
                               ly->l1_bnd, 0, gemm_workspace, gemm_workspace_bytes, stream));
        PD(psalm_gemm_x3(hdd, 2L * Kf, hddinv, ly->l2_w, 2L * Kf, ly->l2_ws, Kf, ly->l2_b, sn, D, x1, D, S, D, 0, 0, gemm_workspace, gemm_workspace_bytes, stream));
        PD(psalm_layernorm_split(x1, D, more ? sc : ms_out, D, ly->n2_g, ly->n2_b, S, D, eps, more ? sp2 : nullptr, more ? inv2 : nullptr, more ? lvl_pos : nullptr,
                                 more ? S : 0, more ? sp3 : nullptr, more ? inv3 : nullptr, stream));
    }
    {
        const int C2 = d->in_dims[0], Kp2 = c64(C2), hs = g.h[1], ws_ = g.w[1], H2 = g.h[0], W2 = g.w[0], K9 = 9 * D, Kp9 = c64(K9);
        PD(psalm_split_f16(feats_host[0], C2, tokp, 2L * Kp2, tokinv, HW2, C2, stream));
        PD(psalm_gemm_x3(tokp, 2L * Kp2, tokinv, d->adapter_w, 2L * Kp2, d->adapter_ws, Kp2, d->adapter_b, nullptr, 0, lat, D, HW2, D, 0, 0, gemm_workspace, gemm_workspace_bytes, stream));
        PD(psalm_groupnorm_nhwc(lat, PSALM_F32, lat2, PSALM_F32, d->adapter_gn_g, d->adapter_gn_b, gnws, 1, HW2, D, d->G, eps, 1, stream));
        PD(psalm_upsample_add_nhwc(lat2, PSALM_F32, ms_out + g.start[2] * D, PSALM_F32, y, PSALM_F32, 1, hs, ws_, H2, W2, D, stream));
        PD(psalm_im2col_split_f16(y, cols, colsinv, 1, H2, W2, D, 3, 1, 1, stream));
        PD(psalm_gemm_x3(cols, 2L * Kp9, colsinv, d->layer_w, 2L * Kp9, d->layer_ws, Kp9, d->layer_b, nullptr, 0, y2, D, HW2, D, 0, 0, gemm_workspace, gemm_workspace_bytes, stream));
        PD(psalm_groupnorm_nhwc(y2, PSALM_F32, y, PSALM_F32, d->layer_gn_g, d->layer_gn_b, gnws, 1, HW2, D, d->G, eps, 1, stream));
        PD(psalm_split_f16(y, D, cols, 2L * KpD, colsinv, HW2, D, stream));
        PD(psalm_gemm_x3(cols, 2L * KpD, colsinv, d->mf_w, 2L * KpD, d->mf_ws, KpD, d->mf_b, nullptr, 0, mask_features, d->mask_dim, HW2, d->mask_dim, 0, 0, gemm_workspace,
                         gemm_workspace_bytes, stream));
    }
#undef PD
    return 0;
}

struct PrLayout { long kin, vin, sp, spinv, K[3], V[3], mfp, mfinv, dec, me0, me1, me2, mes, mesinv, masks, amask, flags, outq, qp, a, x1, out[2], qk, v, hdd, mha, t0, t1, total; };
static PrLayout pr_layout(const psalm_pr_desc* d, const int* hwl, int H2, int W2, int n_extra) {
    const long D = d->D, Q = d->Q, HW2 = (long)H2 * W2;
    long mhw = 0, mmha = 0;
    for (int l = 0; l < d->num_levels; ++l) {
        const long hw = (long)hwl[2 * l] * hwl[2 * l + 1];
        mhw = std::max(mhw, hw);
        mmha = std::max(mmha, psalm_mha_attention_f32_workspace(1, d->heads, (int)Q, (int)hw));
    }
    mmha = std::max(mmha, psalm_mha_attention_f32_workspace(1, d->heads, (int)Q, (int)Q));
    PrLayout o;
    long p = 0;
    o.kin = p; p += al256(mhw * D * 4);
    o.vin = p; p += al256(mhw * D * 4);
    o.sp = p; p += al256(mhw * 2 * c64((int)D) * 2); o.spinv = p; p += al256(mhw * 4);
    for (int l = 0; l < 3; ++l) {
        const long hw = l < d->num_levels ? (long)hwl[2 * l] * hwl[2 * l + 1] : 0;
        const long nl_l = l < d->num_levels ? (d->num_layers - l + d->num_levels - 1) / d->num_levels : 0;
        o.K[l] = p; p += al256(hw * nl_l * D * 4);
        o.V[l] = p; p += al256(hw * nl_l * D * 4);
    }
    o.mfp = p; p += al256(HW2 * 2 * c64(d->mask_dim) * 2); o.mfinv = p; p += al256(HW2 * 4);
    o.dec = p; p += al256(Q * D * 4);
    o.me0 = p; p += al256(Q * D * 4); o.me1 = p; p += al256(Q * D * 4); o.me2 = p; p += al256(Q * std::max<long>(D, d->mask_dim) * 4);
    o.mes = p; p += al256(Q * 2 * c64(d->mask_dim) * 2); o.mesinv = p; p += al256(Q * 4);
    o.masks = p; p += al256(Q * HW2 * 4);
    o.amask = p; p += al256(Q * mhw); o.flags = p; p += al256(Q);
    o.outq = p; p += al256(Q * D * 4); o.qp = p; p += al256(Q * D * 4); o.a = p; p += al256(Q * D * 4); o.x1 = p; p += al256(Q * D * 4);
    o.out[0] = p; p += al256(Q * D * 4); o.out[1] = p; p += al256(Q * D * 4);
    o.qk = p; p += al256(Q * 2 * D * 4); o.v = p; p += al256(Q * D * 4);
    o.hdd = p; p += al256(Q * (long)d->ffn * 4);
    o.mha = p; p += al256(mmha);
    o.t0 = p; p += al256(std::max<long>(Q, n_extra) * D * 4); o.t1 = p; p += al256(std::max<long>(Q, n_extra) * D * 4);
    o.total = p;
    return o;
}
static int pr_check(const psalm_pr_desc* d) {
    PSALM_CHECK_ARG(d && d->layers && d->num_layers >= 1 && d->num_levels >= 1 && d->num_levels <= 3 && d->Q >= 1 && d->Q <= 128 && d->D == 32 * d->heads &&
                        d->D % 8 == 0 && d->mask_dim % 8 == 0 && d->ffn % 8 == 0, "psalm_predictor_forward: descriptor (Q <= 128, D = 32 * heads, <= 3 levels)");
    return 0;
}
extern "C" long psalm_predictor_forward_workspace(const psalm_pr_desc* d, const int* hw_levels_host, int H2, int W2, int n_extra_rows) {
    if (pr_check(d) != 0 || !hw_levels_host || H2 <= 0 || W2 <= 0) return -1;
    return pr_layout(d, hw_levels_host, H2, W2, n_extra_rows).total;
}
static int predictor_kv_impl(const psalm_pr_desc* d, const PrLayout& lo, const float* const* ms_host, const int* hw_levels_host, const float* const* prpos_host,
                             const float* mask_features, int H2, int W2, char* ws, void* gemm_workspace, long gemm_workspace_bytes, void* stream) {
    const int D = d->D, nl = d->num_layers, nlev = d->num_levels, HW2 = H2 * W2, MD = d->mask_dim;
    float* kin = (float*)(ws + lo.kin); float* vin = (float*)(ws + lo.vin);
    void* sp = ws + lo.sp; float* spinv = (float*)(ws + lo.spinv);
    const int KpD = c64(D), KpM = c64(MD);
    int rc;
#define PR(call) do { rc = (call); if (rc) return rc; } while (0)
    for (int l = 0; l < nlev; ++l) {
        const int hw = hw_levels_host[2 * l] * hw_levels_host[2 * l + 1];
        const int N = ((nl - l + nlev - 1) / nlev) * D;
        float* Kl = (float*)(ws + lo.K[l]); float* Vl = (float*)(ws + lo.V[l]);
        PR(psalm_add_bcast(ms_host[l], PSALM_F32, prpos_host[l], PSALM_F32, kin, PSALM_F32, hw, D, hw, stream));
        PR(psalm_add_bcast(ms_host[l], PSALM_F32, d->level_embed + (long)l * D, PSALM_F32, vin, PSALM_F32, hw, D, 1, stream));
        PR(psalm_split_f16(kin, D, sp, 2L * KpD, spinv, hw, D, stream));
        PR(psalm_gemm_x3(sp, 2L * KpD, spinv, d->lvl_k_w[l], 2L * KpD, d->lvl_k_ws[l], KpD, d->lvl_k_b[l], nullptr, 0, Kl, N, hw, N, 0, 0, gemm_workspace, gemm_workspace_bytes, stream));
        PR(psalm_split_f16(vin, D, sp, 2L * KpD, spinv, hw, D, stream));
        PR(psalm_gemm_x3(sp, 2L * KpD, spinv, d->lvl_v_w[l], 2L * KpD, d->lvl_v_ws[l], KpD, d->lvl_v_b[l], nullptr, 0, Vl, N, hw, N, 0, 0, gemm_workspace, gemm_workspace_bytes, stream));
    }
    if (HW2 > 4096) PR(psalm_split_f16(mask_features, MD, ws + lo.mfp, 2L * KpM, (float*)(ws + lo.mfinv), HW2, MD, stream));
#undef PR
    return 0;
}
extern "C" int psalm_predictor_kv(const psalm_pr_desc* d, const float* const* ms_host, const int* hw_levels_host, const float* const* prpos_host,
                                  const float* mask_features, int H2, int W2, int n_extra_rows, void* workspace, long workspace_bytes,
                                  void* gemm_workspace, long gemm_workspace_bytes, void* stream) {
    if (pr_check(d) != 0) return -1;
    PSALM_CHECK_ARG(ms_host && hw_levels_host && prpos_host && mask_features && workspace, "psalm_predictor_kv: null argument");
    const PrLayout lo = pr_layout(d, hw_levels_host, H2, W2, std::max(n_extra_rows, 0));
    PSALM_CHECK_ARG(workspace_bytes >= lo.total && (uintptr_t)workspace % 256 == 0, "psalm_predictor_kv: workspace of psalm_predictor_forward_workspace() bytes, 256-byte aligned");
    return predictor_kv_impl(d, lo, ms_host, hw_levels_host, prpos_host, mask_features, H2, W2, (char*)workspace, gemm_workspace, gemm_workspace_bytes, stream);
}
extern "C" int psalm_predictor_forward(const psalm_pr_desc* d, const float* const* ms_host, const int* hw_levels_host, const float* const* prpos_host,
                                       const float* mask_features, int H2, int W2, const float* seg_query, const float* class_emb, int n_cls,
                                       const float* seg_emb, int n_seg, const float* region_emb, int n_reg, float* pred_masks, float* cls_logits,
                                       float* seg_logits, float* region_logits, void* workspace, long workspace_bytes, void* gemm_workspace,
                                       long gemm_workspace_bytes, int kv_ready, void* stream) {
    if (pr_check(d) != 0) return -1;
    PSALM_CHECK_ARG(ms_host && hw_levels_host && prpos_host && mask_features && seg_query && pred_masks && workspace, "psalm_predictor_forward: null argument");
    const int D = d->D, Q = d->Q, nh = d->heads, nl = d->num_layers, nlev = d->num_levels, HW2 = H2 * W2, MD = d->mask_dim, F = d->ffn;
    const PrLayout lo = pr_layout(d, hw_levels_host, H2, W2, std::max(n_reg, 0));
    PSALM_CHECK_ARG(workspace_bytes >= lo.total && (uintptr_t)workspace % 256 == 0, "psalm_predictor_forward: workspace of psalm_predictor_forward_workspace() bytes, 256-byte aligned");
    char* ws = (char*)workspace;
    const float eps = 1e-5f;
    float* Kl[3]; float* Vl[3];
    for (int l = 0; l < 3; ++l) { Kl[l] = (float*)(ws + lo.K[l]); Vl[l] = (float*)(ws + lo.V[l]); }
    void* mfp = ws + lo.mfp; float* mfinv = (float*)(ws + lo.mfinv);
    float* dec = (float*)(ws + lo.dec); float* me0 = (float*)(ws + lo.me0); float* me1 = (float*)(ws + lo.me1); float* me2 = (float*)(ws + lo.me2);
    void* mes = ws + lo.mes; float* mesinv = (float*)(ws + lo.mesinv);
    float* masks = (float*)(ws + lo.masks);
    unsigned char* amask = (unsigned char*)(ws + lo.amask); unsigned char* flags = (unsigned char*)(ws + lo.flags);
    float* outq = (float*)(ws + lo.outq); float* qp = (float*)(ws + lo.qp); float* a = (float*)(ws + lo.a); float* x1 = (float*)(ws + lo.x1);
    float* outb[2] = {(float*)(ws + lo.out[0]), (float*)(ws + lo.out[1])};
    float* qk = (float*)(ws + lo.qk); float* v = (float*)(ws + lo.v); float* hdd = (float*)(ws + lo.hdd);
    void* mha = ws + lo.mha;
    float* t0 = (float*)(ws + lo.t0); float* t1 = (float*)(ws + lo.t1);
    int rc;
#define PR(call) do { rc = (call); if (rc) return rc; } while (0)
    auto g32 = [&](const float* A, int M, int K, const float* W, const float* b, const float* res, float* C, int N, int act) -> int {
        return psalm_gemm(A, PSALM_F32, K, W, PSALM_F32, K, b, res, res ? N : 0, C, PSALM_F32, N, M, N, K, act, 0, gemm_workspace, gemm_workspace_bytes, stream);
    };
    auto ln = [&](const float* x, const float* g_, const float* b_, float* y, int rows) -> int {
        return psalm_layernorm3(x, PSALM_F32, D, y, PSALM_F32, D, nullptr, 0, nullptr, 0, nullptr, 0, g_, b_, rows, D, eps, stream);
    };
    const int KpM = c64(MD);
    int nl_l[3] = {0, 0, 0};
    for (int l = 0; l < nlev; ++l) nl_l[l] = (nl - l + nlev - 1) / nlev;
    if (!kv_ready) PR(predictor_kv_impl(d, lo, ms_host, hw_levels_host, prpos_host, mask_features, H2, W2, ws, gemm_workspace, gemm_workspace_bytes, stream));
    const bool mf_split = HW2 > 4096;
    const bool fuse = D % 8 == 0 && D <= 2048 && Q <= 192 && psalm_get_tuning(PSALM_TUNE_DECODER_FUSE) != 0;
    auto mask_head = [&](const float* out_, bool have_dec, const psalm_pr_layer* next, float* dst) -> int {
        int r;
        if (!have_dec && (r = ln(out_, d->dn_g, d->dn_b, dec, Q))) return r;
        if (fuse && next) {
            if ((r = psalm_gemm_f32_pair(dec, d->mask_embed_w[0], d->mask_embed_b[0], me0, Q, D, D, 1, outq, next->cq_w, next->cq_b, qp, Q, D, D, 0, stream))) return r;
        } else if ((r = g32(dec, Q, D, d->mask_embed_w[0], d->mask_embed_b[0], nullptr, me0, D, 1))) return r;
        if ((r = g32(me0, Q, D, d->mask_embed_w[1], d->mask_embed_b[1], nullptr, me1, D, 1))) return r;
        if ((r = g32(me1, Q, D, d->mask_embed_w[2], d->mask_embed_b[2], nullptr, me2, MD, 0))) return r;
        if (mf_split) {
            if ((r = psalm_split_f16(me2, MD, mes, 2L * KpM, mesinv, Q, MD, stream))) return r;
            return psalm_gemm_x3(mes, 2L * KpM, mesinv, mfp, 2L * KpM, mfinv, KpM, nullptr, nullptr, 0, dst, HW2, Q, HW2, 0, 0, gemm_workspace, gemm_workspace_bytes, stream);
        }
        return g32(me2, Q, MD, mask_features, nullptr, nullptr, dst, HW2, 0);
    };
    const float* out = seg_query;
    if (fuse) PR(psalm_add_bcast(out, PSALM_F32, d->query_embed, PSALM_F32, outq, PSALM_F32, Q, D, Q, stream));
    PR(mask_head(out, false, &d->layers[0], masks));
    if (!fuse) PR(psalm_add_bcast(out, PSALM_F32, d->query_embed, PSALM_F32, outq, PSALM_F32, Q, D, Q, stream));
    int cur = 0;
    for (int i = 0; i < nl; ++i) {
        const psalm_pr_layer* ly = &d->layers[i];
        const int l = i % nlev, j = i / nlev, h = hw_levels_host[2 * l], w = hw_levels_host[2 * l + 1], hw = h * w, N = nl_l[l] * D;
        PR(psalm_attn_mask(masks, amask, flags, Q, H2, W2, h, w, stream));
        if (!fuse) PR(g32(outq, Q, D, ly->cq_w, ly->cq_b, nullptr, qp, D, 0));
        PR(psalm_mha_attention_f32(qp, D, Kl[l] + (long)j * D, N, Vl[l] + (long)j * D, N, a, D, amask, flags, mha, 1, Q, hw, nh, 32, stream));
        PR(g32(a, Q, D, ly->co_w, ly->co_b, out, x1, D, 0));
        float* o1 = outb[cur];
        if (fuse) {
            PR(psalm_layernorm_chain(x1, D, o1, D, ly->cn_g, ly->cn_b, d->query_embed, Q, outq, D, nullptr, nullptr, nullptr, 0, Q, D, eps, stream));
            PR(psalm_gemm_f32_pair(outq, ly->sqk_w, ly->sqk_b, qk, Q, 2 * D, D, 0, o1, ly->sv_w, ly->sv_b, v, Q, D, D, 0, stream));
        } else {
            PR(ln(x1, ly->cn_g, ly->cn_b, o1, Q));
            PR(psalm_add_bcast(o1, PSALM_F32, d->query_embed, PSALM_F32, outq, PSALM_F32, Q, D, Q, stream));
            PR(g32(outq, Q, D, ly->sqk_w, ly->sqk_b, nullptr, qk, 2 * D, 0));
            PR(g32(o1, Q, D, ly->sv_w, ly->sv_b, nullptr, v, D, 0));
        }
        PR(psalm_mha_attention_f32(qk, 2L * D, qk + D, 2L * D, v, D, a, D, nullptr, nullptr, mha, 1, Q, Q, nh, 32, stream));
        PR(g32(a, Q, D, ly->so_w, ly->so_b, o1, x1, D, 0));
        float* o2 = outb[cur ^ 1];
        PR(ln(x1, ly->sn_g, ly->sn_b, o2, Q));
        PR(g32(o2, Q, D, ly->f1_w, ly->f1_b, nullptr, hdd, F, 1));
        PR(g32(hdd, Q, F, ly->f2_w, ly->f2_b, o2, x1, D, 0));
        if (fuse) {
            PR(psalm_layernorm_chain(x1, D, o1, D, ly->fn_g, ly->fn_b, d->query_embed, Q, outq, D, d->dn_g, d->dn_b, dec, D, Q, D, eps, stream));
        } else {
            PR(ln(x1, ly->fn_g, ly->fn_b, o1, Q));
            PR(psalm_add_bcast(o1, PSALM_F32, d->query_embed, PSALM_F32, outq, PSALM_F32, Q, D, Q, stream));
        }
        out = o1;
        PR(mask_head(out, fuse, i + 1 < nl ? &d->layers[i + 1] : nullptr, i + 1 < nl ? masks : pred_masks));
        cur ^= 1;
    }
    struct Head { const float* w0; const float* b0; const float* w1; const float* b1; const float* A; const float* W; float* C; int M, N; float* h0; float* h1; };
    Head hd[3];
    int nh_ = 0;
    if (class_emb && n_cls > 0) {
        PSALM_CHECK_ARG(cls_logits != nullptr, "psalm_predictor_forward: cls_logits output missing");
        hd[nh_++] = Head{d->CLASS_w[0], d->CLASS_b[0], d->CLASS_w[1], d->CLASS_b[1], nullptr, class_emb, cls_logits, Q, n_cls, nullptr, nullptr};
    }
    if (seg_emb && n_seg > 0) {
        PSALM_CHECK_ARG(seg_logits != nullptr, "psalm_predictor_forward: seg_logits output missing");
        hd[nh_++] = Head{d->SEG_w[0], d->SEG_b[0], d->SEG_w[1], d->SEG_b[1], nullptr, seg_emb, seg_logits, Q, n_seg, nullptr, nullptr};
    }
    if (region_emb && n_reg > 0) {
        PSALM_CHECK_ARG(region_logits != nullptr, "psalm_predictor_forward: region_logits output missing");
        hd[nh_++] = Head{d->REGION_w[0], d->REGION_b[0], d->REGION_w[1], d->REGION_b[1], region_emb, nullptr, region_logits, n_reg, Q, nullptr, nullptr};
    }
    auto emb = [&](const Head& x) -> int {
        return g32(x.A ? x.A : x.h1, x.M, D, x.W ? x.W : x.h1, nullptr, nullptr, x.C, x.N, 0);
    };
    const bool pair = fuse && nh_ >= 2;
    int first = 0;
    if (pair) {
        Head& x = hd[0]; Head& y = hd[1];
        x.h0 = t0; x.h1 = t1; y.h0 = me0; y.h1 = me1;
        PR(psalm_gemm_f32_pair(dec, x.w0, x.b0, x.h0, Q, D, D, 1, dec, y.w0, y.b0, y.h0, Q, D, D, 1, stream));
        PR(psalm_gemm_f32_pair(x.h0, x.w1, x.b1, x.h1, Q, D, D, 0, y.h0, y.w1, y.b1, y.h1, Q, D, D, 0, stream));
        if (x.M <= 192 && y.M <= 192 && x.N <= 8192 && y.N <= 8192)
            PR(psalm_gemm_f32_pair(x.A ? x.A : x.h1, x.W ? x.W : x.h1, nullptr, x.C, x.M, x.N, D, 0, y.A ? y.A : y.h1, y.W ? y.W : y.h1, nullptr, y.C, y.M, y.N, D, 0, stream));
        else { PR(emb(x)); PR(emb(y)); }
        first = 2;
    }
    for (int i = first; i < nh_; ++i) {
        Head& x = hd[i];
        x.h0 = t0; x.h1 = t1;
        PR(g32(dec, Q, D, x.w0, x.b0, nullptr, x.h0, D, 1));
        PR(g32(x.h0, Q, D, x.w1, x.b1, nullptr, x.h1, D, 0));
        PR(emb(x));
    }
#undef PR
    return 0;
}

int gemm_x3_select_rows(const void* A2, long lda, const float* a_scale, const void* W2, long ldw, const float* w_scale, int Kp, void* C, long ldc,
                        int M, int N, int select_m, void* workspace, long workspace_bytes, void* stream);
// ... 334 lines not shown
```

### psalm_amd/hip_ops.py

```python
from __future__ import annotations

import ctypes
import math
import os
import sys
from ctypes import c_char_p, c_float, c_int, c_long, c_void_p
from typing import Optional, Sequence

import numpy as np
import torch

_HERE = os.path.dirname(os.path.abspath(__file__))
DEFAULT_LIB = os.path.join(_HERE, "lib", "libpsalm_hip.so")

F32, BF16 = 0, 1
ACT_NONE, ACT_RELU, ACT_GELU, ACT_GELU_NEW = 0, 1, 2, 3
ACT_POST_RESIDUAL = 16
ACT_BIAS_ROW = 32
_DT = {torch.float32: F32, torch.bfloat16: BF16}


_DEBUG_SYNC = os.environ.get("PSALM_DEBUG_SYNC", "0") not in ("", "0")
_DEBUG_BOUNDS = os.environ.get("PSALM_DEBUG_BOUNDS", "0") not in ("", "0")
BOUND_LOOSENESS_LIMIT = 2.0 ** 14


class PsalmHipError(RuntimeError):
    pass


def _dt(t: torch.Tensor) -> int:
    try:
        return _DT[t.dtype]
    except KeyError:
        raise PsalmHipError(f"unsupported dtype {t.dtype} (float32 / bfloat16 only)")


ABI_VERSION = 18


class _ProfiledLib:

    def __init__(self, cdll):
        object.__setattr__(self, "_cdll", cdll)
        object.__setattr__(self, "records", None)
        object.__setattr__(self, "calls", None)

    def __getattr__(self, name):
        fn = getattr(self._cdll, name)
        if not name.startswith("psalm_") or name in ("psalm_last_error", "psalm_backend", "psalm_abi_version", "psalm_gemm_last_kernel",
                                                         "psalm_gemm_set_tile_policy", "psalm_gemm_x3_set_products", "psalm_set_tuning",
                                                         "psalm_get_tuning") or name.endswith("_workspace"):
            return fn

        def call(*args):
            rec = self.records
            if self.calls is not None:
                self.calls.append(name)
            if _DEBUG_SYNC:
                sys.stderr.write(f"[psalm launch] {name}\n"); sys.stderr.flush()
                rc = fn(*args)
                if torch.cuda.is_available() and not torch.cuda.is_current_stream_capturing():
                    torch.cuda.synchronize()
                sys.stderr.write(f"[psalm ok] {name}\n"); sys.stderr.flush()
                return rc
            if rec is None:
                return fn(*args)
            e0, e1 = torch.cuda.Event(enable_timing=True), torch.cuda.Event(enable_timing=True)
            e0.record()
            rc = fn(*args)
            e1.record()
            kern = None
            if name.startswith(("psalm_gemm", "psalm_conv2d")):
                kern = self._cdll.psalm_gemm_last_kernel().decode()
            rec.append((name, tuple(a.value if hasattr(a, "value") else a for a in args), e0, e1, kern))
            return rc
        return call

    def __setattr__(self, k, v):
        if k in ("records", "calls"):
            object.__setattr__(self, k, v)
        else:
            setattr(self._cdll, k, v)


class SplitF16:
    __slots__ = ("t", "inv_scale", "K", "Kp")

    def __init__(self, t, inv_scale, K):
        self.t, self.inv_scale, self.K, self.Kp = t, inv_scale, K, t.shape[1] // 2

    @property
    def shape(self):
        return (self.t.shape[0], self.K)

    @property
    def dtype(self):
        return torch.float32


class _PostDesc(ctypes.Structure):
    _fields_ = [(n, c_int) for n in ("task", "Q", "h", "w", "Hpad", "Wpad", "crop_h", "crop_w", "out_h", "out_w", "C1", "n_region")] + \
               [("obj_thr", c_float), ("overlap_thr", c_float)]


class _PostIO(ctypes.Structure):
    _fields_ = [(n, c_void_p) for n in ("pred_masks", "mask_up", "cls_logits", "seg_logits", "region_logits", "is_thing", "mask_pred", "sem_seg", "scores",
                                        "classes", "query", "inst_masks", "boxes", "pan", "counts")]


class _PhiLayer(ctypes.Structure):
    _fields_ = [("w1", c_void_p), ("w1_scale", c_void_p), ("b1", c_void_p), ("w2", c_void_p), ("w2_scale", c_void_p), ("b2", c_void_p),
                ("ln_g", c_void_p), ("ln_b", c_void_p), ("bnd", c_void_p), ("paired", c_int)]


class _RopeOut(ctypes.Structure):
    _fields_ = [("Qr", c_void_p), ("Kr", c_void_p), ("cos_table", c_void_p), ("sin_table", c_void_p), ("q_col", c_int), ("k_col", c_int),
                ("heads", c_int), ("B", c_int), ("L", c_int), ("Lp", c_int), ("scale", c_float), ("pad_", c_int)]


class _PhiDesc(ctypes.Structure):
    _fields_ = [("num_layers", c_int), ("hidden", c_int), ("intermediate", c_int), ("heads", c_int), ("head_dim", c_int), ("rot", c_int),
                ("ln_eps", c_float), ("layers", ctypes.POINTER(_PhiLayer)), ("final_g", c_void_p), ("final_b", c_void_p)]


class _SwinBlock(ctypes.Structure):
    _fields_ = [(n, c_void_p) for n in ("n1_g", "n1_b", "n2_g", "n2_b", "qkv_w", "qkv_ws", "qkv_b", "qkv_bnd", "proj_w", "proj_ws", "proj_b",
                                         "fc1_w", "fc1_ws", "fc1_b", "fc1_bnd")] + [("fc1_paired", c_int)] + \
               [(n, c_void_p) for n in ("fc2_w", "fc2_ws", "fc2_b", "rpb")]


class _SwinStage(ctypes.Structure):
    _fields_ = [("depth", c_int), ("heads", c_int), ("dim", c_int), ("blocks", ctypes.POINTER(_SwinBlock)), ("out_g", c_void_p), ("out_b", c_void_p),
                ("ds_g", c_void_p), ("ds_b", c_void_p), ("ds_w", c_void_p), ("ds_ws", c_void_p)]


class _SwinDesc(ctypes.Structure):
    _fields_ = [("num_stages", c_int), ("patch", c_int), ("window", c_int), ("pe_kpad", c_int), ("mlp_ratio", c_int), ("pe_w", c_void_p),
                ("pe_ws", c_void_p), ("pe_b", c_void_p), ("pe_ln_g", c_void_p), ("pe_ln_b", c_void_p), ("stages", ctypes.POINTER(_SwinStage))]


class _ProjDesc(ctypes.Structure):
    _fields_ = [("in_dim", c_int), ("mid_dim", c_int), ("out_dim", c_int)] + \
               [(n, c_void_p) for n in ("c1_w", "c1_ws", "c1_b", "c2_w", "c2_ws", "c2f_w", "c2f_ws", "c2f_b", "ds_w", "ds_ws", "ds_b", "fc_w", "fc_ws", "fc_b")]


class _PdEncLayer(ctypes.Structure):
    _fields_ = [(n, c_void_p) for n in ("value_w", "value_ws", "value_b", "ow_w", "ow_ws", "ow_b", "out_w", "out_ws", "out_b", "n1_g", "n1_b",
                                         "l1_w", "l1_ws", "l1_b", "l1_bnd")] + [("l1_paired", c_int)] + \
               [(n, c_void_p) for n in ("l2_w", "l2_ws", "l2_b", "n2_g", "n2_b")]


class _PdDesc(ctypes.Structure):
    _fields_ = [("D", c_int), ("G", c_int), ("M", c_int), ("num_layers", c_int), ("ffn", c_int), ("mask_dim", c_int), ("in_dims", c_int * 4),
                ("ip_w", c_void_p * 3), ("ip_ws", c_void_p * 3), ("ip_b", c_void_p * 3), ("ip_gn_g", c_void_p * 3), ("ip_gn_b", c_void_p * 3)] + \
               [(n, c_void_p) for n in ("adapter_w", "adapter_ws", "adapter_b", "adapter_gn_g", "adapter_gn_b", "layer_w", "layer_ws", "layer_b",
                                         "layer_gn_g", "layer_gn_b", "mf_w", "mf_ws", "mf_b")] + [("layers", ctypes.POINTER(_PdEncLayer))]


class _PrLayer(ctypes.Structure):
    _fields_ = [(n, c_void_p) for n in ("cq_w", "cq_b", "co_w", "co_b", "cn_g", "cn_b", "sqk_w", "sqk_b", "sv_w", "sv_b", "so_w", "so_b", "sn_g", "sn_b",
                                         "f1_w", "f1_b", "f2_w", "f2_b", "fn_g", "fn_b")]


class _PrDesc(ctypes.Structure):
    _fields_ = [(n, c_int) for n in ("D", "heads", "Q", "num_layers", "num_levels", "ffn", "mask_dim")] + \
               [(n, c_void_p * 3) for n in ("lvl_k_w", "lvl_k_ws", "lvl_k_b", "lvl_v_w", "lvl_v_ws", "lvl_v_b")] + \
               [(n, c_void_p) for n in ("level_embed", "query_embed", "dn_g", "dn_b")] + [("mask_embed_w", c_void_p * 3), ("mask_embed_b", c_void_p * 3)] + \
               [(n, c_void_p * 2) for n in ("SEG_w", "SEG_b", "CLASS_w", "CLASS_b", "REGION_w", "REGION_b")] + [("layers", ctypes.POINTER(_PrLayer))]


class Ops:
    GEMM_X3_256_DEFAULT = 2582

    def __init__(self, lib_path: str = DEFAULT_LIB):
        if not os.path.exists(lib_path):
            raise PsalmHipError(
                f"{lib_path} not found: build the HIP kernels first (python -m psalm_amd.build). "
                "psalm_amd has no CPU / PyTorch fallback by design.")
        cdll = ctypes.CDLL(lib_path)
        got = cdll.psalm_abi_version() if hasattr(cdll, "psalm_abi_version") else -1
        if got != ABI_VERSION:
            raise PsalmHipError(f"{lib_path}: psalm_abi_version() = {got}, this binding needs {ABI_VERSION}: rebuild the library "
                                "(python -m psalm_amd.build --force)")
        cdll.psalm_last_error.restype = c_char_p
        cdll.psalm_backend.restype = c_char_p
        cdll.psalm_gemm_last_kernel.restype = c_char_p
        self._cdll_raw = cdll
        self.lib = _ProfiledLib(cdll)
        self.backend = self.lib.psalm_backend().decode()
        self.is_emu = self.backend == "emu"
# ... 526 lines not shown

    def postprocess(self, task, sizes, pred_masks=None, mask_up=None, cls_logits=None, seg_logits=None, region_logits=None, is_thing=None,
                    obj_thr=0.8, overlap_thr=0.8, counts_extra=0):
        Hpad, Wpad, oh, ow, height, width = [int(v) for v in sizes]
        src = pred_masks if pred_masks is not None else mask_up
        Q = int(src.shape[0])
        h_, w_ = (int(pred_masks.shape[1]), int(pred_masks.shape[2])) if pred_masks is not None else (Hpad, Wpad)
        C1 = int(cls_logits.shape[1]) if cls_logits is not None else 0
        k = int(region_logits.shape[0]) if region_logits is not None else 0
        code = self.POST_TASKS[task]
        d = _PostDesc(code, Q, h_, w_, Hpad, Wpad, oh, ow, height, width, C1, k, float(obj_thr), float(overlap_thr))
        self.lib.psalm_postprocess_workspace.restype = c_long
        nbytes = self.lib.psalm_postprocess_workspace(ctypes.byref(d), 1 if mask_up is not None else 0)
        if nbytes < 0:
            raise PsalmHipError(f"psalm_postprocess_workspace: {self.lib.psalm_last_error().decode()}")
        ws = self._stage_ws("postprocess", nbytes + 256)
        off = (-ws.data_ptr()) % 256
        resize_after = (oh, ow, height, width) != (Hpad, Wpad, Hpad, Wpad)
        out = {}
        if task == "semantic":
            if mask_up is None:
                out["mask_pred"] = self.empty(Q, Hpad, Wpad)
            out["sem_seg"] = self.empty(C1 - 1, height, width)
        else:
            if resize_after or mask_up is None:
                out["mask_pred"] = self.empty(Q, height, width)
            out["scores"] = self.empty(Q, k) if task == "region" else self.empty(Q)
            out["inst_masks"] = self.empty(Q, height, width)
            out["boxes"] = self.empty(Q, 4)
            out["counts"] = self.empty(2 + 3 * Q + int(counts_extra), dtype=torch.int32)
            if task in ("instance", "panoptic"):
                out["classes"] = self.empty(Q, dtype=torch.int64)
            if task != "region":
                out["query"] = self.empty(Q, dtype=torch.int64)
            if task == "panoptic":
                out["sem_seg"] = self.empty(C1 - 1, height, width)
                out["pan"] = self.empty(height, width, dtype=torch.int32)
        io = _PostIO(*[self._pi(t) for t in (pred_masks, mask_up, cls_logits, seg_logits, region_logits, is_thing, out.get("mask_pred"), out.get("sem_seg"),
                                             out.get("scores"), out.get("classes"), out.get("query"), out.get("inst_masks"), out.get("boxes"), out.get("pan"),
                                             out.get("counts"))])
        which = c_int(0)
        fn = getattr(self.lib, "psalm_postprocess_" + task)
        rc = fn(ctypes.byref(d), ctypes.byref(io), ctypes.byref(which), c_void_p(ws.data_ptr() + off), c_long(nbytes), self._stream())
        self._check(rc, "psalm_postprocess_" + task)
        if which.value == 1:
            out["mask_pred"] = mask_up
        return out

    @staticmethod
    def _pi(t):
        return None if t is None else t.data_ptr()

    def phi_forward_plan(self, desc, B, L):
        out = (c_int * 3)()
        self._check(self._cdll_raw.psalm_phi_forward_plan(ctypes.byref(desc), B, L, out), "psalm_phi_forward_plan")
        return bool(out[0]), out[1], out[2]

    def phi_forward(self, desc, embeds, key_mask, cos, sin, B, L):
        if embeds.dtype != torch.float32 or embeds.dim() != 2 or embeds.shape[0] != B * L or embeds.shape[1] != desc.hidden:
            raise PsalmHipError("phi_forward: float32 (B*L, hidden) embeddings")
        self.lib.psalm_phi_forward_workspace.restype = c_long
        nbytes = self.lib.psalm_phi_forward_workspace(ctypes.byref(desc), B, L)
        if nbytes < 0:
            raise PsalmHipError(f"psalm_phi_forward_workspace: {self.lib.psalm_last_error().decode()}")
        ws = self._stage_ws("phi", nbytes + 256)
        off = (-ws.data_ptr()) % 256
        out = self.empty(B * L, desc.hidden, dtype=torch.float32)
        rc = self.lib.psalm_phi_forward(ctypes.byref(desc), self._p(embeds), self._p(key_mask), self._p(cos), self._p(sin), B, L, self._p(out),
                                        c_void_p(ws.data_ptr() + off), c_long(nbytes), self._p(self._gemm_ws()), c_long(self.GEMM_WS_BYTES),
                                        self._stream())
        self._check(rc, "psalm_phi_forward")
        return out

    def phi_prefix_cache(self, hidden, heads, P, num_layers):
        self.lib.psalm_phi_prefix_cache_layer_bytes.restype = c_long
        kb, vb = c_long(0), c_long(0)
        stride = self.lib.psalm_phi_prefix_cache_layer_bytes(hidden, heads, P, ctypes.byref(kb), ctypes.byref(vb))
        if stride <= 0:
            raise PsalmHipError("phi_prefix_cache: hidden, heads, P >= 1")
        kb, Pp = kb.value, (P + 31) // 32 * 32
        raw = torch.empty(stride * num_layers + 256, dtype=torch.uint8, device=self.device)
        off = (-raw.data_ptr()) % 256
        buf = raw[off:off + stride * num_layers]
        views = []
        for i in range(num_layers):
            o0 = stride * i
            views.append((buf[o0:o0 + heads * Pp * 64 * 4].view(torch.float32).view(heads, Pp, 64),
                          buf[o0 + kb:o0 + kb + P * hidden * 4].view(torch.float32).view(P, hidden)))
        return buf, views

    def phi_prefix(self, desc, embeds, key_mask, cos, sin, P, cache):
        if embeds.dtype != torch.float32 or embeds.dim() != 2 or embeds.shape[0] != P or embeds.shape[1] != desc.hidden or key_mask.numel() != P:
            raise PsalmHipError("phi_prefix: float32 (P, hidden) embeddings, key mask of P bytes")
        self.lib.psalm_phi_prefix_workspace.restype = c_long
        self.lib.psalm_phi_prefix_cache_bytes.restype = c_long
        nbytes = self.lib.psalm_phi_prefix_workspace(ctypes.byref(desc), P)
        cbytes = self.lib.psalm_phi_prefix_cache_bytes(ctypes.byref(desc), P)
        if nbytes < 0 or cbytes < 0:
            raise PsalmHipError(f"psalm_phi_prefix_workspace: {self.lib.psalm_last_error().decode()}")
        if cache.numel() < cbytes or cache.data_ptr() % 256:
            raise PsalmHipError("phi_prefix: cache of psalm_phi_prefix_cache_bytes() bytes, 256-byte aligned")
        ws = self._stage_ws("phi_prefix", nbytes + 256)
        off = (-ws.data_ptr()) % 256
        rc = self.lib.psalm_phi_prefix(ctypes.byref(desc), self._p(embeds), self._p(key_mask), self._p(cos), self._p(sin), P, self._p(cache),
                                       c_long(cache.numel()), c_void_p(ws.data_ptr() + off), c_long(nbytes), self._p(self._gemm_ws()),
                                       c_long(self.GEMM_WS_BYTES), self._stream())
        self._check(rc, "psalm_phi_prefix")

    def phi_suffix(self, desc, embeds, key_mask, cos, sin, N, S, P, cache):
        if embeds.dtype != torch.float32 or embeds.dim() != 2 or embeds.shape[0] != N * S or embeds.shape[1] != desc.hidden or key_mask.numel() != N * S \
                or cos.shape[0] < P + S:
            raise PsalmHipError("phi_suffix: float32 (N*S, hidden) embeddings, key mask (N, S), tables of >= P + S rows")
        self.lib.psalm_phi_suffix_workspace.restype = c_long
        self.lib.psalm_phi_prefix_cache_bytes.restype = c_long
        nbytes = self.lib.psalm_phi_suffix_workspace(ctypes.byref(desc), N, S)
        cbytes = self.lib.psalm_phi_prefix_cache_bytes(ctypes.byref(desc), P)
        if nbytes < 0 or cbytes < 0:
            raise PsalmHipError(f"psalm_phi_suffix_workspace: {self.lib.psalm_last_error().decode()}")
        if cache.numel() < cbytes or cache.data_ptr() % 256:
            raise PsalmHipError("phi_suffix: cache of psalm_phi_prefix_cache_bytes() bytes, 256-byte aligned")
        ws = self._stage_ws("phi_suffix", nbytes + 256)
        off = (-ws.data_ptr()) % 256
        out = self.empty(N * S, desc.hidden, dtype=torch.float32)
        rc = self.lib.psalm_phi_suffix(ctypes.byref(desc), self._p(embeds), self._p(key_mask), self._p(cos), self._p(sin), N, S, P, self._p(cache),
                                       c_long(cache.numel()), self._p(out), c_void_p(ws.data_ptr() + off), c_long(nbytes),
                                       self._p(self._gemm_ws()), c_long(self.GEMM_WS_BYTES), self._stream())
        self._check(rc, "psalm_phi_suffix")
        return out

    def phi_suffix_grouped(self, desc, embeds, key_mask, cos, sin, N, S, refs, P_max, table=None):
        if embeds.dtype != torch.float32 or embeds.dim() != 2 or embeds.shape[0] != N * S or embeds.shape[1] != desc.hidden or key_mask.numel() != N * S \
                or cos.shape[0] < P_max + S:
            raise PsalmHipError("phi_suffix_grouped: float32 (N*S, hidden) embeddings, key mask (N, S), tables of >= P_max + S rows")
        refs = self._prefix_refs(refs, table, desc.num_layers * N, P_max, desc.heads, "phi_suffix_grouped")
        self.lib.psalm_phi_suffix_grouped_workspace.restype = c_long
        nbytes = self.lib.psalm_phi_suffix_grouped_workspace(ctypes.byref(desc), N, S)
        if nbytes < 0:
            raise PsalmHipError(f"psalm_phi_suffix_grouped_workspace: {self.lib.psalm_last_error().decode()}")
        ws = self._stage_ws("phi_suffix", nbytes + 256)
        off = (-ws.data_ptr()) % 256
        out = self.empty(N * S, desc.hidden, dtype=torch.float32)
        rc = self.lib.psalm_phi_suffix_grouped(ctypes.byref(desc), self._p(embeds), self._p(key_mask), self._p(cos), self._p(sin), N, S,
                                               self._p(refs) if refs is not None else None, P_max, self._p(out),
                                               c_void_p(ws.data_ptr() + off), c_long(nbytes), self._p(self._gemm_ws()),
                                               c_long(self.GEMM_WS_BYTES), self._stream())
        self._check(rc, "psalm_phi_suffix_grouped")
        return out

    def x3_products(self, n: int):
        self._check(self.lib.psalm_gemm_x3_set_products(int(n)), "psalm_gemm_x3_set_products")

    TUNE_GEMM_XCD_KSPLIT, TUNE_ATTN_XCD_HEADS, TUNE_GEMM_MID, TUNE_DECODER_FUSE, TUNE_ROW_GROUPS, TUNE_MHA_QTILE_WAVES = 0, 1, 2, 3, 4, 5
    TUNE_PHI_ROPE_EPILOGUE = 6

    def set_tuning(self, key: int, value: int):
        self._check(self.lib.psalm_set_tuning(int(key), int(value)), "psalm_set_tuning")

    def get_tuning(self, key: int) -> int:
        return int(self.lib.psalm_get_tuning(int(key)))

    def gemm_tile_policy(self, bm: int):
        self._check(self.lib.psalm_gemm_set_tile_policy(bm), "psalm_gemm_set_tile_policy")

    def layernorm(self, x, gamma, beta, eps=1e-5, out=None, out_dtype=None, out2=None, add=None, out3=None):
        rows, C = x.shape
        if out is None:
            out = self.empty(rows, C, dtype=out_dtype or x.dtype)
        for t in (out2, out3):
            if t is not None and t.dtype != torch.bfloat16:
                raise PsalmHipError("layernorm: out2 / out3 must be bfloat16")
        if out3 is not None and (add is None or add.dtype != torch.float32 or add.shape[1] != C):
            raise PsalmHipError("layernorm: out3 needs a float32 (r,C) `add` table")
        rc = self.lib.psalm_layernorm3(self._pv(x), _dt(x), c_long(x.stride(0)), self._pv(out), _dt(out), c_long(out.stride(0)),
                                       self._pv(out2), c_long(out2.stride(0) if out2 is not None else 0),
                                       self._p(add) if out3 is not None else c_void_p(0), c_long(add.shape[0] if out3 is not None else 0),
                                       self._pv(out3), c_long(out3.stride(0) if out3 is not None else 0),
                                       self._p(gamma), self._p(beta), rows, C, c_float(eps), self._stream())
        self._check(rc, "psalm_layernorm3")
        return out

    def layernorm_split(self, x, gamma, beta, eps=1e-5, want_y=False, want_split=True, add=None):
        rows, C = x.shape
        if x.dtype != torch.float32 or x.stride(1) != 1:
            raise PsalmHipError("layernorm_split: float32 rows")
        Kp = (C + 63) // 64 * 64
        y = self.empty(rows, C, dtype=torch.float32) if want_y else None
        s1 = i1 = s2 = i2 = None
        if want_split:
            s1, i1 = self.empty(rows, 2 * Kp, dtype=torch.float16), self.empty(rows, dtype=torch.float32)
        if add is not None:
            if add.dtype != torch.float32 or add.shape[1] != C:
                raise PsalmHipError("layernorm_split: float32 (r,C) `add` table")
            s2, i2 = self.empty(rows, 2 * Kp, dtype=torch.float16), self.empty(rows, dtype=torch.float32)
        rc = self.lib.psalm_layernorm_split(self._pv(x), c_long(x.stride(0)), self._p(y), c_long(C), self._p(gamma), self._p(beta), rows, C,
                                            c_float(eps), self._p(s1), self._p(i1), self._p(add), c_long(add.shape[0] if add is not None else 0),
                                            self._p(s2), self._p(i2), self._stream())
        self._check(rc, "psalm_layernorm_split")
        return y, (SplitF16(s1, i1, C) if want_split else None), (SplitF16(s2, i2, C) if add is not None else None)

    def swin_window_gather(self, x, gamma, beta, B, H, W, ws, shift, eps=1e-5, out_dtype=None):
        C = x.shape[-1]
        nWh, nWw = (H + ws - 1) // ws, (W + ws - 1) // ws
        out = self.empty(B * nWh * nWw * ws * ws, C, dtype=out_dtype or x.dtype)
        rc = self.lib.psalm_swin_window_gather(self._p(x), _dt(x), self._p(out), _dt(out), self._p(gamma), self._p(beta), B, H, W,
                                               C, ws, shift, c_float(eps), self._stream())
        self._check(rc, "psalm_swin_window_gather")
        return out

    def swin_window_gather_split(self, x, gamma, beta, B, H, W, ws, shift, eps=1e-5):
        C = x.shape[-1]
        if x.dtype != torch.float32 or C % 8 or C > 2048:
            raise PsalmHipError("swin_window_gather_split: float32, C % 8 == 0, C <= 2048")
        nWh, nWw = (H + ws - 1) // ws, (W + ws - 1) // ws
        rows, Kp = B * nWh * nWw * ws * ws, (C + 63) // 64 * 64
        t = self.empty(rows, 2 * Kp, dtype=torch.float16)
        inv = self.empty(rows, dtype=torch.float32)
        rc = self.lib.psalm_swin_window_gather_split(self._p(x), self._p(t), self._p(inv), self._p(gamma), self._p(beta), B, H, W, C, ws, shift,
                                                     c_float(eps), self._stream())
        self._check(rc, "psalm_swin_window_gather_split")
        return SplitF16(t, inv, C)

    def swin_window_merge_ln_split(self, win, shortcut, gamma, beta, B, H, W, ws, shift, eps=1e-5):
        C = shortcut.shape[-1]
        if shortcut.dtype != torch.float32 or win.dtype != torch.float32 or C % 8 or C > 2048:
            raise PsalmHipError("swin_window_merge_ln_split: float32 operands, C % 8 == 0, C <= 2048")
        rows, Kp = shortcut.shape[0], (C + 63) // 64 * 64
        out_x = torch.empty_like(shortcut)
        t = self.empty(rows, 2 * Kp, dtype=torch.float16)
        inv = self.empty(rows, dtype=torch.float32)
        rc = self.lib.psalm_swin_window_merge_ln_split(self._p(win), self._p(shortcut), self._p(out_x), self._p(t), self._p(inv), self._p(gamma),
                                                       self._p(beta), B, H, W, C, ws, shift, c_float(eps), self._stream())
        self._check(rc, "psalm_swin_window_merge_ln_split")
        return out_x, SplitF16(t, inv, C)

    def swin_window_merge(self, win, shortcut, B, H, W, ws, shift, out=None):
        C = shortcut.shape[-1]
        if out is None:
            out = torch.empty_like(shortcut)
        rc = self.lib.psalm_swin_window_merge(self._p(win), _dt(win), self._p(shortcut), self._p(out), _dt(shortcut), B, H, W, C,
                                              ws, shift, self._stream())
        self._check(rc, "psalm_swin_window_merge")
        return out

    def swin_window_merge_ln(self, win, shortcut, gamma, beta, B, H, W, ws, shift, eps=1e-5, h_dtype=None):
        C = shortcut.shape[-1]
        if shortcut.dtype != torch.float32:
            raise PsalmHipError("swin_window_merge_ln: the residual stream must be float32")
        out_x = torch.empty_like(shortcut)
        out_h = self.empty(shortcut.shape[0], C, dtype=h_dtype or win.dtype)
        rc = self.lib.psalm_swin_window_merge_ln(self._p(win), _dt(win), self._p(shortcut), self._p(out_x), self._p(out_h), _dt(out_h),
                                                 self._p(gamma), self._p(beta), B, H, W, C, ws, shift, c_float(eps), self._stream())
        self._check(rc, "psalm_swin_window_merge_ln")
        return out_x, out_h

    def patch_merge_ln(self, x, gamma, beta, B, H, W, eps=1e-5, out_dtype=None):
        C = x.shape[-1]
        out = self.empty(B * ((H + 1) // 2) * ((W + 1) // 2), 4 * C, dtype=out_dtype or x.dtype)
        rc = self.lib.psalm_patch_merge_ln(self._p(x), _dt(x), self._p(out), _dt(out), self._p(gamma), self._p(beta), B, H, W, C,
                                           c_float(eps), self._stream())
        self._check(rc, "psalm_patch_merge_ln")
        return out

    def groupnorm_nhwc(self, x, gamma, beta, B, HW, groups, eps=1e-5, relu=False, out_dtype=None, out=None):
        C = x.shape[-1]
        if out is None:
            out = self.empty(B * HW, C, dtype=out_dtype or x.dtype)
        ws = self.empty(B * ((HW + 63) // 64 + 1) * groups * 2, dtype=torch.float32)
        rc = self.lib.psalm_groupnorm_nhwc(self._p(x), _dt(x), self._p(out), _dt(out), self._p(gamma), self._p(beta), self._p(ws),
                                           B, HW, C, groups, c_float(eps), int(relu), self._stream())
        self._check(rc, "psalm_groupnorm_nhwc")
        return out

    def layernorm_chain(self, x, g1, b1, add=None, g2=None, b2=None, eps=1e-5):
        rows, C = x.shape
        y1 = self.empty(rows, C, dtype=torch.float32)
        y2 = self.empty(rows, C, dtype=torch.float32) if add is not None else None
        y3 = self.empty(rows, C, dtype=torch.float32) if g2 is not None else None
        rc = self.lib.psalm_layernorm_chain(self._p(x), c_long(x.stride(0)), self._p(y1), c_long(C), self._p(g1), self._p(b1), self._pv(add),
                                            c_long(add.shape[0] if add is not None else 0), self._pv(y2), c_long(C), self._pv(g2), self._pv(b2),
                                            self._pv(y3), c_long(C), rows, C, c_float(eps), self._stream())
        self._check(rc, "psalm_layernorm_chain")
        return y1, y2, y3

    def gemm_f32_pair(self, a0, w0, bias0, a1, w1, bias1, act0=ACT_NONE, act1=ACT_NONE):
        c0 = self.empty(a0.shape[0], w0.shape[0], dtype=torch.float32)
        c1 = self.empty(a1.shape[0], w1.shape[0], dtype=torch.float32)
        rc = self.lib.psalm_gemm_f32_pair(self._p(a0), self._p(w0), self._pv(bias0), self._p(c0), a0.shape[0], w0.shape[0], a0.shape[1], act0,
                                          self._p(a1), self._p(w1), self._pv(bias1), self._p(c1), a1.shape[0], w1.shape[0], a1.shape[1], act1, self._stream())
        self._check(rc, "psalm_gemm_f32_pair")
        return c0, c1

    def gemm_f32_rows(self, a, w, bias=None, residual=None, act=ACT_NONE):
        M, K = a.shape
        N = w.shape[0]
        out = self.empty(M, N, dtype=torch.float32)
        rc = self.lib.psalm_gemm_f32_rows(self._pv(a), c_long(a.stride(0)), self._pv(w), c_long(w.stride(0)), self._pv(bias), self._pv(residual),
                                          c_long(residual.stride(0) if residual is not None else 0), self._p(out), c_long(N), M, N, K, act, self._stream())
        self._check(rc, "psalm_gemm_f32_rows")
        return out

    def gemm_f32_rows_pair(self, a0, w0, bias0, a1, w1, bias1, act0=ACT_NONE, act1=ACT_NONE):
        c0 = self.empty(a0.shape[0], w0.shape[0], dtype=torch.float32)
        c1 = self.empty(a1.shape[0], w1.shape[0], dtype=torch.float32)
        rc = self.lib.psalm_gemm_f32_rows_pair(self._p(a0), self._p(w0), self._pv(bias0), self._p(c0), a0.shape[0], w0.shape[0], a0.shape[1], act0,
                                               self._p(a1), self._p(w1), self._pv(bias1), self._p(c1), a1.shape[0], w1.shape[0], a1.shape[1], act1, self._stream())
        self._check(rc, "psalm_gemm_f32_rows_pair")
        return c0, c1

    def gemm_f32_grouped(self, a_list, w_list):
        n = len(a_list)
        if n != len(w_list) or not 1 <= n <= 16:
            raise PsalmHipError("gemm_f32_grouped: 1..16 problems")
        K = int(a_list[0].shape[1])
        for a, w in zip(a_list, w_list):
            if a.dtype != torch.float32 or w.dtype != torch.float32 or a.dim() != 2 or w.dim() != 2 or a.shape[1] != K or w.shape[1] != K:
                raise PsalmHipError("gemm_f32_grouped: float32 (M_i, K) x (N_i, K) operands of one K")
        outs = [self.empty(a.shape[0], w.shape[0], dtype=torch.float32) for a, w in zip(a_list, w_list)]
        VP, VI = c_void_p * n, c_int * n
        rc = self.lib.psalm_gemm_f32_grouped(VP(*[self._p(a).value or 0 for a in a_list]), VP(*[self._p(w).value or 0 for w in w_list]),
                                             VP(*[self._p(c).value or 0 for c in outs]), VI(*[int(a.shape[0]) for a in a_list]),
                                             VI(*[int(w.shape[0]) for w in w_list]), K, n, self._stream())
        self._check(rc, "psalm_gemm_f32_grouped")
        return outs

    def add_bcast(self, a, b, out_dtype=None):
        rows, C = a.shape
        out = self.empty(rows, C, dtype=out_dtype or a.dtype)
        rc = self.lib.psalm_add_bcast(self._p(a), _dt(a), self._p(b), _dt(b), self._p(out), _dt(out), c_long(rows), C,
                                      c_long(b.shape[0]), self._stream())
        self._check(rc, "psalm_add_bcast")
        return out

    def gather_rows(self, srcs, src_id, src_row, C, out_dtype=torch.float32):
        srcs = list(srcs) + [None] * (4 - len(srcs))
        rows = src_id.numel()
        out = self.empty(rows, C, dtype=out_dtype)
        args = []
        for t in srcs:
            args += [self._p(t), _dt(t) if t is not None else 0]
        rc = self.lib.psalm_gather_rows(*args, self._p(src_id), self._p(src_row), self._p(out), _dt(out), c_long(rows), C,
                                        self._stream())
        self._check(rc, "psalm_gather_rows")
        return out

    def segment_mean(self, x, seg_offsets, seg_rows, out_dtype=None):
        nseg = seg_offsets.numel() - 1
        C = x.shape[-1]
        out = self.empty(nseg, C, dtype=out_dtype or x.dtype)
        rc = self.lib.psalm_segment_mean(self._pv(x), _dt(x), c_long(x.stride(0)), self._p(seg_offsets), self._p(seg_rows),
                                         self._p(out), _dt(out), nseg, C, self._stream())
        self._check(rc, "psalm_segment_mean")
        return out

    def window_attention(self, qkv, bias_table, B, nWh, nWw, heads, ws, shift):
        C = qkv.shape[-1] // 3
        out = self.empty(qkv.shape[0], C, dtype=qkv.dtype)
        if qkv.dtype == torch.bfloat16 and ws == 12:
            rc = self.lib.psalm_window_attention_mfma(self._p(qkv), self._p(bias_table), self._p(out), B, nWh, nWw, C, heads, ws,
                                                      shift, self._stream())
            self._check(rc, "psalm_window_attention_mfma")
            return out
        rc = self.lib.psalm_window_attention(self._p(qkv), self._p(bias_table), self._p(out), _dt(qkv), B, nWh, nWw, C, heads, ws,
                                             shift, self._stream())
        self._check(rc, "psalm_window_attention")
        return out

    def window_attention_split(self, qkv, bias_table, a_inv, bound_par, B, nWh, nWw, heads, ws, shift):
        C = qkv.shape[-1] // 3
        if qkv.dtype != torch.float32 or ws != 12 or a_inv.numel() != qkv.shape[0]:
            raise PsalmHipError("window_attention_split: float32 qkv, 12 x 12 windows, one operand scale per row")
        Kp = (C + 63) // 64 * 64
        so = (self.empty if Kp == C else self.zeros)(qkv.shape[0], 2 * Kp, dtype=torch.float16)
        inv = self.empty(qkv.shape[0], dtype=torch.float32)
        rc = self.lib.psalm_window_attention_split(self._p(qkv), self._p(bias_table), self._p(a_inv), self._p(bound_par), self._p(so), Kp,
                                                   self._p(inv), B, nWh, nWw, C, heads, ws, shift, self._stream())
        self._check(rc, "psalm_window_attention_split")
        return SplitF16(so, inv, C)

    def causal_attention(self, buf, q_off, k_off, v_off, out, o_off, cos, sin, key_mask, B, L, heads, head_dim, rot):
        if buf.dtype != out.dtype:
            raise PsalmHipError("causal_attention: buf/out dtype mismatch")
        if buf.dtype == torch.bfloat16:
            self.lib.psalm_causal_attention_mfma_workspace.restype = c_long
            nbytes = self.lib.psalm_causal_attention_mfma_workspace(B, L, heads)
            key = ("causal_ws", nbytes)
            ws = self._ws.get(key)
            if ws is None:
                ws = self._ws[key] = torch.empty(nbytes, dtype=torch.uint8, device=self.device)
            rc = self.lib.psalm_causal_attention_mfma(self._pv(buf), c_long(buf.stride(0)), q_off, k_off, v_off, self._pv(out),
                                                      c_long(out.stride(0)), o_off, self._p(cos), self._p(sin), self._p(key_mask),
                                                      self._p(ws), B, L, heads, head_dim, rot, self._stream())
            self._check(rc, "psalm_causal_attention_mfma")
            return out
        if (buf.dtype == torch.float32 and head_dim == 64 and rot == 32 and buf.stride(0) % 4 == 0 and out.stride(0) % 4 == 0
                and all(v % 4 == 0 for v in (q_off, k_off, v_off, o_off)) and buf.data_ptr() % 16 == 0 and out.data_ptr() % 16 == 0):
            self.lib.psalm_causal_attention_f32_workspace.restype = c_long
            nbytes = self.lib.psalm_causal_attention_f32_workspace(B, L, heads)
            key = ("causal_f32_ws", nbytes)
            ws = self._ws.get(key)
            if ws is None:
                ws = self._ws[key] = torch.empty(nbytes, dtype=torch.uint8, device=self.device)
            rc = self.lib.psalm_causal_attention_f32(self._pv(buf), c_long(buf.stride(0)), q_off, k_off, v_off, self._pv(out),
                                                     c_long(out.stride(0)), o_off, self._p(cos), self._p(sin), self._p(key_mask), self._p(ws),
                                                     B, L, heads, head_dim, rot, self._stream())
            self._check(rc, "psalm_causal_attention_f32")
            return out
        rc = self.lib.psalm_causal_attention(self._pv(buf), _dt(buf), c_long(buf.stride(0)), q_off, k_off, v_off, self._pv(out),
                                             c_long(out.stride(0)), o_off, self._p(cos), self._p(sin), self._p(key_mask), B, L,
                                             heads, head_dim, rot, self._stream())
        self._check(rc, "psalm_causal_attention")
        return out

    def causal_attention_workspace_bytes(self, B, L, heads):
        self.lib.psalm_causal_attention_f32_workspace.restype = c_long
        return self.lib.psalm_causal_attention_f32_workspace(B, L, heads)

    def causal_attention_workspace(self, B, L, heads):
        nbytes = self.causal_attention_workspace_bytes(B, L, heads)
        key = ("causal_f32_ws", nbytes)
        ws = self._ws.get(key)
        if ws is None:
            ws = self._ws[key] = torch.empty(nbytes, dtype=torch.uint8, device=self.device)
        return ws

    def phi_attention_tables(self, key_mask, ws, B, L, heads):
        if key_mask.dtype != torch.uint8 or key_mask.numel() != B * L or not key_mask.is_contiguous():
            raise PsalmHipError("phi_attention_tables: contiguous uint8 key mask (B, L)")
        if ws.dtype != torch.uint8 or ws.numel() < self.causal_attention_workspace_bytes(B, L, heads):
            raise PsalmHipError("phi_attention_tables: workspace of causal_attention_workspace(B, L, heads)")
        self._check(self.lib.psalm_phi_attention_tables(self._p(key_mask), self._p(ws), B, L, heads, self._stream()), "psalm_phi_attention_tables")

    def causal_attention_split_prepared(self, buf, v_off, split_out, split_inv, split_col_off, ws, B, L, heads, head_dim):
        if buf.dtype != torch.float32 or split_out.dtype != torch.float16 or split_inv.dtype != torch.float32:
            raise PsalmHipError("causal_attention_split_prepared: float32 v buffer, float16 split buffer, float32 scales")
        if ws.dtype != torch.uint8 or ws.numel() < self.causal_attention_workspace_bytes(B, L, heads):
            raise PsalmHipError("causal_attention_split_prepared: workspace of causal_attention_workspace(B, L, heads)")
        rc = self.lib.psalm_causal_attention_f32_split_prepared(self._pv(buf), c_long(buf.stride(0)), v_off, self._p(split_out),
                                                                c_long(split_out.stride(0)), split_out.shape[1] // 2, split_col_off,
                                                                self._p(split_inv), self._p(ws), B, L, heads, head_dim, self._stream())
        self._check(rc, "psalm_causal_attention_f32_split_prepared")
        return split_out

    def causal_attention_split(self, buf, q_off, k_off, v_off, split_out, split_inv, split_col_off, cos, sin, key_mask, B, L, heads,
                               head_dim, rot):
        if buf.dtype != torch.float32 or split_out.dtype != torch.float16 or split_inv.dtype != torch.float32:
            raise PsalmHipError("causal_attention_split: float32 qkv buffer, float16 split buffer, float32 scales")
        self.lib.psalm_causal_attention_f32_workspace.restype = c_long
        nbytes = self.lib.psalm_causal_attention_f32_workspace(B, L, heads)
        key = ("causal_f32_ws", nbytes)
        ws = self._ws.get(key)
        if ws is None:
            ws = self._ws[key] = torch.empty(nbytes, dtype=torch.uint8, device=self.device)
        rc = self.lib.psalm_causal_attention_f32_split(self._pv(buf), c_long(buf.stride(0)), q_off, k_off, v_off, self._p(split_out),
                                                       c_long(split_out.stride(0)), split_out.shape[1] // 2, split_col_off,
                                                       self._p(split_inv), self._p(cos), self._p(sin), self._p(key_mask), self._p(ws),
                                                       B, L, heads, head_dim, rot, self._stream())
        self._check(rc, "psalm_causal_attention_f32_split")
        return split_out

    def _prefix_attn_ws(self, N, S, heads):
        self.lib.psalm_causal_attention_f32_prefix_workspace.restype = c_long
        nbytes = self.lib.psalm_causal_attention_f32_prefix_workspace(N, S, heads)
        key = ("causal_prefix_ws", nbytes)
        ws = self._ws.get(key)
        if ws is None:
            ws = self._ws[key] = torch.empty(nbytes, dtype=torch.uint8, device=self.device)
        return ws

    @staticmethod
    def _check_prefix_cache(k_cache, v_cache, P, heads):
        Pp = (P + 31) // 32 * 32
        if (k_cache.dtype != torch.float32 or v_cache.dtype != torch.float32 or not k_cache.is_contiguous() or k_cache.numel() != heads * Pp * 64
                or v_cache.dim() != 2 or v_cache.shape[0] != P or v_cache.shape[1] < heads * 64 or v_cache.stride(1) != 1):
            raise PsalmHipError("prefix cache: K (heads, ceil32(P), 64) float32 contiguous, V (P, >= heads*64) float32 rows")

    def phi_prefix_kv_store(self, buf, k_off, v_off, cos, sin, k_cache, v_cache, P, heads, head_dim, rot):
        if buf.dtype != torch.float32 or buf.shape[0] < P:
            raise PsalmHipError("phi_prefix_kv_store: float32 buffer of >= P rows")
        self._check_prefix_cache(k_cache, v_cache, P, heads)
        rc = self.lib.psalm_phi_prefix_kv_store(self._pv(buf), c_long(buf.stride(0)), k_off, v_off, self._p(cos), self._p(sin), self._p(k_cache),
                                                self._pv(v_cache), c_long(v_cache.stride(0)), P, heads, head_dim, rot, self._stream())
        self._check(rc, "psalm_phi_prefix_kv_store")

    def causal_attention_prefix(self, buf, q_off, k_off, v_off, k_cache, v_cache, out, o_off, cos, sin, key_mask, N, S, P, heads, head_dim, rot):
# ... 237 lines not shown
        self._check(rc, "psalm_upsample_add_nhwc")
        return out

    def region_pool(self, tokens, img_of_region, pts, h, w, n_img):
        R, n = pts.shape[0], pts.shape[1]
        C = tokens.shape[-1]
        out = self.empty(R, C, dtype=torch.float32)
        if tokens.dtype != torch.float32:
            raise PsalmHipError("region_pool expects fp32 image tokens")
        rc = self.lib.psalm_region_pool(self._p(tokens), self._p(img_of_region), self._p(pts), self._p(out), R, h, w, C, n,
                                        self._stream())
        self._check(rc, "psalm_region_pool")
        return out

    def permute_layout(self, x, B, C, HW, to_nhwc, out_dtype=None):
        out = self.empty((B * HW, C) if to_nhwc else (B, C, HW), dtype=out_dtype or x.dtype)
        rc = self.lib.psalm_permute_layout(self._p(x), _dt(x), self._p(out), _dt(out), B, C, c_long(HW), int(to_nhwc), self._stream())
        self._check(rc, "psalm_permute_layout")
        return out

    def class_softmax(self, cls, Kpad, probsT_dtype=torch.float32):
        Q, C1 = cls.shape
        probs = self.empty(Q, C1)
        probsT = self.zeros(C1 - 1, Kpad, dtype=probsT_dtype)
        score = self.empty(Q)
        label = self.empty(Q, dtype=torch.int32)
        rc = self.lib.psalm_class_softmax(self._p(cls), self._p(probs), self._p(probsT), _dt(probsT), self._p(score), self._p(label),
                                          Q, C1, Kpad, self._stream())
        self._check(rc, "psalm_class_softmax")
        return probs, probsT, score, label

    def sigmoid_transpose(self, mask, Kpad, out_dtype):
        Q, HW = mask.shape
        out = self.empty(HW, Kpad, dtype=out_dtype)
        rc = self.lib.psalm_sigmoid_transpose(self._p(mask), self._p(out), _dt(out), Q, c_long(HW), Kpad, self._stream())
        self._check(rc, "psalm_sigmoid_transpose")
        return out

    def semantic_from_masks(self, mask, probsT, want_mask_score=False):
        Q, HW = mask.shape
        C, Kpad = probsT.shape
        if probsT.dtype not in (torch.bfloat16, torch.float32) or mask.dtype != torch.float32:
            raise PsalmHipError("semantic_from_masks: f32 logits, bf16 probsT (bf16 MFMA) or f32 probsT (split-f16, fp32-class)")
        out = self.empty(C, HW, dtype=torch.float32)
        ms = self.empty(Q) if want_mask_score else None
        ws = self.empty(Q * 512 * 2) if want_mask_score else None
        fn = self.lib.psalm_semantic_from_masks_x3 if probsT.dtype == torch.float32 else self.lib.psalm_semantic_from_masks
        rc = fn(self._p(mask), self._p(probsT), self._p(out), self._p(ms) if want_mask_score else None,
                self._p(ws) if want_mask_score else None, Q, C, c_long(HW), Kpad, self._stream())
        self._check(rc, "psalm_semantic_from_masks")
        return (out, ms) if want_mask_score else out

    def mask_scores(self, mask):
        Q, HW = mask.shape
        score = self.empty(Q)
        ws = self.empty(Q * 64 * 2)
        rc = self.lib.psalm_mask_scores(self._p(mask), self._p(score), self._p(ws), Q, c_long(HW), self._stream())
        self._check(rc, "psalm_mask_scores")
        return score

    def topk_select(self, vals, C, k, is_thing=None, mask_score=None, apply_sigmoid=False, count_out=None):
        Q, stride = vals.shape
        sc = self.zeros(k)
        cl = self.zeros(k, dtype=torch.int32)
        qq = self.zeros(k, dtype=torch.int32)
        cnt = count_out if count_out is not None else self.zeros(1, dtype=torch.int32)
        rc = self.lib.psalm_topk_select(self._p(vals), Q, C, stride, k, self._p(is_thing), self._p(mask_score), self._p(sc), self._p(cl),
                                        self._p(qq), self._p(cnt), int(apply_sigmoid), self._stream())
        self._check(rc, "psalm_topk_select")
        return sc, cl, qq, cnt

    def binarize_gather(self, mask, n, query=None, count=None):
        Q, Hh, Ww = mask.shape
        out = self.empty(n, Hh, Ww)
        rc = self.lib.psalm_binarize_gather(self._p(mask), self._p(query), self._p(count), self._p(out), n, c_long(Hh * Ww), self._stream())
        self._check(rc, "psalm_binarize_gather")
        return out

    def panoptic(self, mask, score, label, is_thing, num_classes, obj_thr, overlap_thr, info_out=None, ninfo_out=None):
        Q, Hh, Ww = mask.shape
        HW = Hh * Ww
        argq = self.empty(HW, dtype=torch.int32)
        counts = self.empty(Q * 3, dtype=torch.int32)
        final_id = self.empty(Q + num_classes + 1, dtype=torch.int32)
        pan = self.empty(Hh, Ww, dtype=torch.int32)
        info = info_out if info_out is not None else self.zeros(Q, 3, dtype=torch.int32)
        ninfo = ninfo_out if ninfo_out is not None else self.zeros(1, dtype=torch.int32)
        rc = self.lib.psalm_panoptic(self._p(mask), self._p(score), self._p(label), self._p(is_thing), self._p(argq), self._p(counts),
                                     self._p(final_id), self._p(pan), self._p(info), self._p(ninfo), Q, c_long(HW), num_classes,
                                     c_float(obj_thr), c_float(overlap_thr), self._stream())
        self._check(rc, "psalm_panoptic")
        return pan, info, ninfo

    def region_scores(self, logits, mask_score):
        K, Q = logits.shape
        out = self.empty(Q, K)
        rc = self.lib.psalm_region_scores(self._p(logits), self._p(mask_score), self._p(out), K, Q, self._stream())
        self._check(rc, "psalm_region_scores")
        return out

    def msda_forward(self, value, spatial_shapes: Sequence[Sequence[int]], level_start: Sequence[int], loc, attw,
                     out_dtype=None):
        B, S, M, D = value.shape
        _, Lq, _, L, P, _ = loc.shape
        if loc.dtype != torch.float32 or attw.dtype != torch.float32:
            raise PsalmHipError("sampling locations / attention weights must be float32")
        out = self.empty(B, Lq, M * D, dtype=out_dtype or value.dtype)
        sh = (ctypes.c_int64 * (2 * L))(*[int(x) for hw in spatial_shapes for x in hw])
        st = (ctypes.c_int64 * L)(*[int(x) for x in level_start])
        rc = self.lib.psalm_msda_forward(self._p(value), _dt(value), sh, st, self._p(loc), self._p(attw), self._p(out),
                                         _dt(out), B, S, M, D, L, Lq, P, self._stream())
        self._check(rc, "psalm_msda_forward")
        return out

    def msda_forward_dev(self, value, spatial_shapes, level_start, loc, attw, out_dtype=None):
        B, S, M, D = value.shape
        _, Lq, _, L, P, _ = loc.shape
        for t in (spatial_shapes, level_start):
            if t.dtype != torch.int64 or t.device != value.device:
                raise PsalmHipError("msda_forward_dev: int64 level tensors on the value's device")
        if tuple(spatial_shapes.shape) != (L, 2) or level_start.numel() != L:
            raise PsalmHipError(f"msda_forward_dev: level table shapes {tuple(spatial_shapes.shape)} / {tuple(level_start.shape)} for L = {L}")
        key = (spatial_shapes.data_ptr(), spatial_shapes._version, level_start.data_ptr(), level_start._version, S, L)
        if key not in self._msda_tables and not (value.is_cuda and torch.cuda.is_current_stream_capturing()):
            hw, st = spatial_shapes.cpu().tolist(), level_start.reshape(-1).cpu().tolist()
            if any(h <= 0 or w_ <= 0 or s0 < 0 or s0 + h * w_ > S for (h, w_), s0 in zip(hw, st)) or sum(h * w_ for h, w_ in hw) != S:
                raise PsalmHipError(f"msda_forward_dev: level table {hw} / starts {st} does not describe the {S} rows of value")
            if len(self._msda_tables) > 64:
                self._msda_tables.clear()
            self._msda_tables.add(key)
        out = self.empty(B, Lq, M * D, dtype=out_dtype or value.dtype)
        rc = self.lib.psalm_msda_forward_dev(self._p(value), _dt(value), self._p(spatial_shapes.contiguous()), self._p(level_start.contiguous()),
                                             self._p(loc), self._p(attw), self._p(out), _dt(out), B, S, M, D, L, Lq, P, self._stream())
        self._check(rc, "psalm_msda_forward_dev")
        return out

    def msda_policy(self, v: int):
        self._check(self._cdll_raw.psalm_msda_set_policy(int(v)), "psalm_msda_set_policy")

    def msda_fused(self, value, spatial_shapes, level_start, offsets_logits, M, out_dtype=None):
        B, S, C = value.shape
        L, P = len(spatial_shapes), 4
        D = C // M
        if offsets_logits.dtype != torch.float32 or offsets_logits.shape[-1] != M * L * P * 3:
            raise PsalmHipError("offsets_logits must be float32 (B,S,M*L*P*3)")
        out = self.empty(B, S, C, dtype=out_dtype or value.dtype)
        sh = (ctypes.c_int64 * (2 * L))(*[int(x) for hw in spatial_shapes for x in hw])
        st = (ctypes.c_int64 * L)(*[int(x) for x in level_start])
        rc = self.lib.psalm_msda_fused(self._p(value), _dt(value), sh, st, self._p(offsets_logits), self._p(out), _dt(out),
                                       B, S, M, D, L, P, self._stream())
        self._check(rc, "psalm_msda_fused")
        return out


    @staticmethod
    def _want(t, dtype, shape, what):
        if t.dtype != dtype or tuple(t.shape) != tuple(shape) or not t.is_contiguous():
            raise PsalmHipError(f"{what}: contiguous {dtype} tensor of shape {tuple(shape)}, got {t.dtype} {tuple(t.shape)}")
        return t

    def video_pick(self, scores, pick_query=None, pick_score=None):
        if scores.dim() != 2 or scores.dtype != torch.float32:
            raise PsalmHipError("video_pick: scores (Q,R) float32")
        Q, R = scores.shape
        pick_query = self.empty(R, dtype=torch.int32) if pick_query is None else self._want(pick_query, torch.int32, (R,), "video_pick pick_query")
        pick_score = self.empty(R, dtype=torch.float32) if pick_score is None else self._want(pick_score, torch.float32, (R,), "video_pick pick_score")
        self._check(self.lib.psalm_video_pick(self._p(scores), Q, R, self._p(pick_query), self._p(pick_score), self._stream()), "psalm_video_pick")
        return pick_query, pick_score

    def video_fuse(self, pred_masks, pick_query, fill, inter=None, union=None, nonzero=None, flag=None):
        if pred_masks.dim() != 3 or pred_masks.dtype != torch.float32:
            raise PsalmHipError("video_fuse: pred_masks (Q,H,W) float32")
        Q, Hh, Ww = pred_masks.shape
        R = int(pick_query.numel())
        self._want(pick_query, torch.int32, (R,), "video_fuse pick_query")
        self._want(fill, torch.int32, (R,), "video_fuse fill")
        inter = self.empty(R, R, dtype=torch.int32) if inter is None else self._want(inter, torch.int32, (R, R), "video_fuse inter")
        union = self.empty(R, R, dtype=torch.int32) if union is None else self._want(union, torch.int32, (R, R), "video_fuse union")
        nonzero = self.empty(R, dtype=torch.int32) if nonzero is None else self._want(nonzero, torch.int32, (R,), "video_fuse nonzero")
        flag = self.empty(1, dtype=torch.int32) if flag is None else self._want(flag, torch.int32, (1,), "video_fuse flag")
        self.lib.psalm_video_fuse_workspace.restype = c_long
        nbytes = self.lib.psalm_video_fuse_workspace(R)
        if nbytes < 0:
            raise PsalmHipError(f"video_fuse: {R} objects (1..32)")
        ws = self._stage_ws("video_fuse", nbytes)
        picked = self.empty(R, Hh, Ww, dtype=torch.uint8)
        fused = self.empty(Hh, Ww, dtype=torch.uint8)
        rc = self.lib.psalm_video_fuse(self._p(pred_masks), self._p(pick_query), self._p(fill), Q, R, c_long(Hh * Ww), self._p(picked), self._p(fused),
                                       self._p(inter), self._p(union), self._p(nonzero), self._p(flag), self._p(ws), c_long(nbytes), self._stream())
        self._check(rc, "psalm_video_fuse")
        return picked, fused, inter, union, nonzero, flag

    def mask_resize_nearest_pad(self, masks, row_tab, col_tab, total=None):
        if masks.dim() != 3 or masks.dtype != torch.uint8:
            raise PsalmHipError("mask_resize_nearest_pad: masks (R,h,w) uint8")
        R, h, w = masks.shape
        Sh, Sw = int(row_tab.numel()), int(col_tab.numel())
        self._want(row_tab, torch.int32, (Sh,), "mask_resize_nearest_pad row_tab")
        self._want(col_tab, torch.int32, (Sw,), "mask_resize_nearest_pad col_tab")
        if total is not None:
            self._want(total, torch.int32, (R,), "mask_resize_nearest_pad total")
        out = self.empty(R, Sh, Sw, dtype=torch.uint8)
        row_cnt = self.empty(R, Sh, dtype=torch.int32)
        rc = self.lib.psalm_mask_resize_nearest_pad(self._p(masks), R, h, w, self._p(row_tab), self._p(col_tab), Sh, Sw, self._p(out), self._p(row_cnt),
                                                    self._p(total), self._stream())
        self._check(rc, "psalm_mask_resize_nearest_pad")
        return out, row_cnt

    def mask_select_points(self, masks, row_cnt, idx):
        if masks.dim() != 3 or masks.dtype != torch.uint8:
            raise PsalmHipError("mask_select_points: masks (R,Sh,Sw) uint8")
        R, Sh, Sw = masks.shape
        n = int(idx.shape[-1])
        self._want(row_cnt, torch.int32, (R, Sh), "mask_select_points row_cnt")
        self._want(idx, torch.int32, (R, n), "mask_select_points idx")
        pts = self.empty(R, n, 2, dtype=torch.float32)
        rc = self.lib.psalm_mask_select_points(self._p(masks), self._p(row_cnt), self._p(idx), R, Sh, Sw, n, self._p(pts), self._stream())
        self._check(rc, "psalm_mask_select_points")
        return pts

    def mask_rasterize(self, prims, R, h, w, out=None):
        n = int(prims.shape[0])
        self._want(prims, torch.int32, (n, 6), "mask_rasterize prims")
        out = self.empty(R, h, w, dtype=torch.uint8) if out is None else self._want(out, torch.uint8, (R, h, w), "mask_rasterize out")
        rc = self.lib.psalm_mask_rasterize(self._p(prims) if n else c_void_p(0), n, int(R), int(h), int(w), self._p(out), self._stream())
        self._check(rc, "psalm_mask_rasterize")
        return out

    def mask_dilate_disc(self, masks, radius, max_radius, out=None):
        if masks.dim() != 3 or masks.dtype != torch.uint8:
            raise PsalmHipError("mask_dilate_disc: masks (R,h,w) uint8")
        R, h, w = masks.shape
        self._want(radius, torch.int32, (R,), "mask_dilate_disc radius")
        out = self.empty(R, h, w, dtype=torch.uint8) if out is None else self._want(out, torch.uint8, (R, h, w), "mask_dilate_disc out")
        rc = self.lib.psalm_mask_dilate_disc(self._p(masks), self._p(radius), int(max_radius), R, h, w, self._p(out), self._stream())
        self._check(rc, "psalm_mask_dilate_disc")
        return out

    def region_best(self, scores, best_query=None, best_score=None):
        if scores.dim() != 2 or scores.dtype != torch.float32:
            raise PsalmHipError("region_best: scores (Q,R) float32")
        Q, R = scores.shape
        best_query = self.empty(R, dtype=torch.int32) if best_query is None else self._want(best_query, torch.int32, (R,), "region_best best_query")
        best_score = self.empty(R, dtype=torch.float32) if best_score is None else self._want(best_score, torch.float32, (R,), "region_best best_score")
        self._check(self.lib.psalm_region_best(self._p(scores), Q, R, self._p(best_query), self._p(best_score), self._stream()), "psalm_region_best")
        return best_query, best_score

    def mask_gather_u8(self, masks, query):
        if masks.dim() != 3 or masks.dtype != torch.float32:
            raise PsalmHipError("mask_gather_u8: masks (Q,H,W) float32")
        Q, Hh, Ww = masks.shape
        R = int(query.numel())
        self._want(query, torch.int32, (R,), "mask_gather_u8 query")
        out = self.empty(R, Hh, Ww, dtype=torch.uint8)
        rc = self.lib.psalm_mask_gather_u8(self._p(masks), self._p(query), Q, R, c_long(Hh * Ww), self._p(out), self._stream())
        self._check(rc, "psalm_mask_gather_u8")
        return out

    def mask_boxes(self, masks, index=None, out_boxes=None, out_areas=None, workspace=None):
        if masks.dim() != 3 or masks.dtype not in (torch.float32, torch.uint8, torch.bool):
            raise PsalmHipError(f"mask_boxes: masks (n,H,W) float32 / uint8 / bool, got {masks.dtype} {tuple(masks.shape)}")
        if masks.dtype == torch.bool:
            masks = masks.view(torch.uint8)
        n, Hh, Ww = masks.shape
        m = n if index is None else int(index.numel())
        if index is not None:
            self._want(index, torch.int32, (m,), "mask_boxes index")
        boxes = self.empty(m, 4) if out_boxes is None else self._want(out_boxes, torch.float32, (m, 4), "mask_boxes out_boxes")
        areas = self.empty(m, dtype=torch.int32) if out_areas is None else self._want(out_areas, torch.int32, (m,), "mask_boxes out_areas")
        self.lib.psalm_mask_boxes_workspace.restype = c_long
        nbytes = self.lib.psalm_mask_boxes_workspace(m)
        if nbytes < 0:
            raise PsalmHipError(f"mask_boxes: {m} output rows (at most 65535)")
        if workspace is None:
            ws, have = self._stage_ws("mask_boxes", max(nbytes, 4)), nbytes
        else:
            if workspace.dtype != torch.uint8:
                raise PsalmHipError("mask_boxes: workspace must be a uint8 buffer")
            ws, have = workspace, int(workspace.numel())
        rc = self.lib.psalm_mask_boxes(self._p(masks), 1 if masks.dtype == torch.uint8 else 0, n, Hh, Ww, self._p(index), m, self._p(boxes),
                                       self._p(areas), self._p(ws), c_long(have), self._stream())
        self._check(rc, "psalm_mask_boxes")
        return boxes, areas

    def label_boxes(self, labels, n_ids, out=None):
        if labels.dim() != 2 or labels.dtype not in (torch.int32, torch.uint8):
            raise PsalmHipError(f"label_boxes: labels (H,W) int32 / uint8, got {labels.dtype} {tuple(labels.shape)}")
        n_ids = int(n_ids)
        if not 1 <= n_ids <= 256:
            raise PsalmHipError(f"label_boxes: n_ids = {n_ids} (1..256)")
        Hh, Ww = labels.shape
        table = self.empty(n_ids, 5, dtype=torch.int32) if out is None else self._want(out, torch.int32, (n_ids, 5), "label_boxes out")
        rc = self.lib.psalm_label_boxes(self._p(labels), 1 if labels.dtype == torch.uint8 else 0, Hh, Ww, n_ids, self._p(table), self._stream())
        self._check(rc, "psalm_label_boxes")
        return table

    MASK_PAIRS_MAX = 1024

    def mask_bits_words(self, HW) -> int:
        fn = self._cdll_raw.psalm_mask_bits_words
        fn.restype = c_long
        nw = fn(c_long(int(HW)))
        if nw < 0:
            raise PsalmHipError(f"mask bit planes: {HW} pixels per plane (1 .. 2^31 - 1)")
        return int(nw)

# ... 367 lines not shown
```

Measured before the change: 55.82 images/s.

## Fuse fp16 split emission into MSDA, groupnorm and level-embed adds

Adds fused kernels that emit the hi/lo fp16 split representation (with per-row scale) directly from the MSDA output, from the groupnorm apply pass, and from the broadcast-add of positional/level embeddings for the K and V projections. Separate add_bcast, groupnorm and split_f16 launches, along with their fp32 intermediate round trips, are removed in the pixel decoder and predictor, gated by a new PD_FUSE tuning key that defaults to on. The cost is extra workspace for a second split buffer and new kernels specialised to particular shapes, with fallbacks for other shapes.

```diff
diff --git a/include/psalm_hip.h b/include/psalm_hip.h
--- a/include/psalm_hip.h
+++ b/include/psalm_hip.h
@@ -9,7 +9,7 @@
 #define PSALM_BF16 1
 
 const char* psalm_last_error(void);
-#define PSALM_ABI_VERSION 18
+#define PSALM_ABI_VERSION 19
 int psalm_abi_version(void);
 const char* psalm_backend(void);
 
@@ -20,6 +20,7 @@
 #define PSALM_TUNE_ROW_GROUPS 4
 #define PSALM_TUNE_MHA_QTILE_WAVES 5
 #define PSALM_TUNE_PHI_ROPE_EPILOGUE 6
+#define PSALM_TUNE_PD_FUSE 7
 #define PSALM_TUNE_COUNT 8
 int psalm_set_tuning(int key, int value);
 int psalm_get_tuning(int key);
@@ -36,6 +37,13 @@
                      const int64_t* level_start_host, const float* offsets_logits, void* out, int out_dtype, int B, int S,
                      int M, int D, int L, int P, void* stream);
 int psalm_msda_set_policy(int v);
+int psalm_msda_fused_split_ok(int M, int D);
+int psalm_msda_fused_split(const float* value, const int64_t* spatial_shapes_host, const int64_t* level_start_host, const float* offsets_logits,
+                           void* split_out, float* inv_scale, int B, int S, int M, int D, int L, int P, void* stream);
+int psalm_rows_split2(const float* x, long ldx, const float* add_a, long add_a_rows, const float* add_b, long add_b_rows, void* sp_a, float* inv_a,
+                      void* sp_b, float* inv_b, long ld_sp, int rows, int C, void* stream);
+int psalm_groupnorm_nhwc_split(const float* x, float* y, const float* gamma, const float* beta, float* workspace, void* split_out, float* inv_scale,
+                               int B, int HW, int C, int G, float eps, int relu, void* stream);
 
 
 int psalm_gemm(const void* A, int a_dtype, long lda, const void* W, int w_dtype, long ldw, const float* bias,
diff --git a/psalm_amd/csrc/api.hip b/psalm_amd/csrc/api.hip
--- a/psalm_amd/csrc/api.hip
+++ b/psalm_amd/csrc/api.hip
@@ -11,7 +11,7 @@
     g_err[sizeof(g_err) - 1] = 0;
 }
 extern "C" const char* psalm_last_error() { return g_err; }
-static std::atomic<int> g_tuning[PSALM_TUNE_COUNT] = {{1}, {1}, {1}, {1}, {1}, {1}, {1}, {0}};
+static std::atomic<int> g_tuning[PSALM_TUNE_COUNT] = {{1}, {1}, {1}, {1}, {1}, {1}, {1}, {1}};
 extern "C" int psalm_set_tuning(int key, int value) {
     if (key < 0 || key >= PSALM_TUNE_COUNT) { psalm_set_error("psalm_set_tuning: unknown key"); return -1; }
     g_tuning[key].store(value, std::memory_order_relaxed);
diff --git a/psalm_amd/csrc/common.h b/psalm_amd/csrc/common.h
--- a/psalm_amd/csrc/common.h
+++ b/psalm_amd/csrc/common.h
@@ -112,6 +112,34 @@
     const _Float16 h = (_Float16)y;
     hw = (unsigned)__builtin_bit_cast(unsigned short, h);
     sw = (unsigned)__builtin_bit_cast(unsigned short, (_Float16)(y - (float)h));
+}
+
+__device__ __forceinline__ void emit_split8(const float* o8, float sc, unsigned short* hi_dst, unsigned short* lo_dst) {
+    unsigned hw[4], lw[4];
+#pragma unroll
+    for (int k = 0; k < 4; ++k) {
+        unsigned h0, h1, l0, l1;
+        psalm_split_words(o8[2 * k] * sc, h0, l0);
+        psalm_split_words(o8[2 * k + 1] * sc, h1, l1);
+        hw[k] = h0 | (h1 << 16);
+        lw[k] = l0 | (l1 << 16);
+    }
+    *reinterpret_cast<psalm_u32x4*>(hi_dst) = psalm_u32x4{hw[0], hw[1], hw[2], hw[3]};
+    *reinterpret_cast<psalm_u32x4*>(lo_dst) = psalm_u32x4{lw[0], lw[1], lw[2], lw[3]};
+}
+__device__ __forceinline__ void split_scale(float amax, float& sc, float& inv) {
+    int e = (int)((__builtin_bit_cast(unsigned, amax) >> 23) & 0xffu) - 127;
+    int se = 13 - e;
+    se = se > 100 ? 100 : (se < -100 ? -100 : se);
+    const bool zero = !(amax > 0.f) || !(amax < 3.0e38f);
+    sc = zero ? 1.f : __builtin_bit_cast(float, (unsigned)(127 + se) << 23);
+    inv = zero ? 1.f : __builtin_bit_cast(float, (unsigned)(127 - se) << 23);
+}
+
+__device__ __forceinline__ float psalm_gn_elem(float v, float m, float r, float gm, float bt, int relu) {
+    float o = (v - m) * r * gm + bt;
+    if (relu) o = fmaxf(o, 0.f);
+    return o;
 }
 
 #define PSALM_BUF_OOB 0x80000000u
@@ -190,6 +218,7 @@
 #define PSALM_TUNE_ROW_GROUPS 4
 #define PSALM_TUNE_MHA_QTILE_WAVES 5
 #define PSALM_TUNE_PHI_ROPE_EPILOGUE 6
+#define PSALM_TUNE_PD_FUSE 7
 #define PSALM_TUNE_COUNT 8
 #endif
 
diff --git a/psalm_amd/csrc/msda.hip b/psalm_amd/csrc/msda.hip
--- a/psalm_amd/csrc/msda.hip
+++ b/psalm_amd/csrc/msda.hip
@@ -71,10 +71,12 @@
     return t;
 }
 
-template <typename TV, typename TO, int L, int P, bool XCD_BANDS = false, bool QUAD = false>
+template <typename TV, typename TO, int L, int P, bool XCD_BANDS = false, bool QUAD = false, bool SPLIT = false>
 __global__ void __launch_bounds__(256) msda_fused8_kernel(const TV* __restrict__ value, MsdaLevels lv,
                                                           const float* __restrict__ ow, TO* __restrict__ out, int B, int S,
-                                                          int M, int D) {
+                                                          int M, int D, unsigned short* __restrict__ sp = nullptr,
+                                                          float* __restrict__ sp_inv = nullptr) {
+    static_assert(!(SPLIT && QUAD), "the split output belongs to the per-lane form");
     const int G = D >> 3;
     const int Lq = S;
     const long total = (long)B * Lq * M * G;
@@ -227,7 +229,20 @@
                 }
             }
         }
-        st8(out + (((long)b * Lq + q) * M + m) * D + g * 8, acc);
+        if constexpr (SPLIT) {
+            float amax = 0.f;
+#pragma unroll
+            for (int k = 0; k < 8; ++k) amax = fmaxf(amax, fabsf(acc[k]));
+            for (int o = (M * G) >> 1; o > 0; o >>= 1) amax = fmaxf(amax, __shfl_xor(amax, o));
+            float sc, iv;
+            split_scale(amax, sc, iv);
+            const long r = (long)b * Lq + q;
+            const int Kp = M * D, c = m * D + g * 8;
+            if (c == 0) sp_inv[r] = iv;
+            emit_split8(acc, sc, sp + r * 2L * Kp + c, sp + r * 2L * Kp + Kp + c);
+        } else {
+            st8(out + (((long)b * Lq + q) * M + m) * D + g * 8, acc);
+        }
     }
 }
 
@@ -411,3 +426,32 @@
     }));
     PSALM_LAUNCH_END("psalm_msda_fused");
 }
+
+extern "C" int psalm_msda_fused_split_ok(int M, int D) {
+    const int lpr = M * (D / 8);
+    return M > 0 && D > 0 && D % 8 == 0 && (M * D) % 64 == 0 && lpr <= 64 && (lpr & (lpr - 1)) == 0;
+}
+extern "C" int psalm_msda_fused_split(const float* value, const int64_t* spatial_shapes_host, const int64_t* level_start_host,
+                                      const float* offsets_logits, void* split_out, float* inv_scale, int B, int S, int M, int D, int L, int P,
+                                      void* stream) {
+    PSALM_CHECK_ARG(L == 3 && P == 4, "psalm_msda_fused_split: specialised for L=3 levels, P=4 points (PSALM pixel decoder)");
+    PSALM_CHECK_ARG(psalm_msda_fused_split_ok(M, D), "psalm_msda_fused_split: M * D / 8 a power of two <= 64, M * D % 64 == 0");
+    PSALM_CHECK_ARG(value && offsets_logits && split_out && inv_scale && (uintptr_t)value % 16 == 0 && (uintptr_t)split_out % 16 == 0,
+                    "psalm_msda_fused_split: 16-byte aligned tensors");
+    MsdaLevels lv = {};
+    int rc = fill_levels(lv, spatial_shapes_host, level_start_host, L, S);
+    PSALM_CHECK_ARG(rc == 0, "psalm_msda_fused_split: bad level table");
+    const int block = 256;
+    PSALM_CHECK_ARG(block % (M * (D / 8)) == 0, "psalm_msda_fused_split: a query row's lanes must divide the block");
+    const long total8 = (long)B * S * M * (D / 8);
+    if (total8 == 0) return 0;
+    bool bands = B == 1 && total8 % (block * 8) == 0;
+    for (int l = 0; l < L; ++l) bands = bands && lv.H[l] % 8 == 0;
+    if (bands)
+        hipLaunchKernelGGL((msda_fused8_kernel<float, float, 3, 4, true, false, true>), dim3((unsigned)(total8 / block)), dim3(block), 0, (hipStream_t)stream,
+                           value, lv, offsets_logits, (float*)nullptr, B, S, M, D, (unsigned short*)split_out, inv_scale);
+    else
+        hipLaunchKernelGGL((msda_fused8_kernel<float, float, 3, 4, false, false, true>), dim3((unsigned)((total8 + block - 1) / block)), dim3(block), 0,
+                           (hipStream_t)stream, value, lv, offsets_logits, (float*)nullptr, B, S, M, D, (unsigned short*)split_out, inv_scale);
+    PSALM_LAUNCH_END("psalm_msda_fused_split");
+}
diff --git a/psalm_amd/csrc/rowops.hip b/psalm_amd/csrc/rowops.hip
--- a/psalm_amd/csrc/rowops.hip
+++ b/psalm_amd/csrc/rowops.hip
@@ -1,27 +1,6 @@
 #include "common.h"
 #include <type_traits>
 
-__device__ __forceinline__ void emit_split8(const float* o8, float sc, unsigned short* hi_dst, unsigned short* lo_dst) {
-    unsigned hw[4], lw[4];
-#pragma unroll
-    for (int k = 0; k < 4; ++k) {
-        unsigned h0, h1, l0, l1;
-        psalm_split_words(o8[2 * k] * sc, h0, l0);
-        psalm_split_words(o8[2 * k + 1] * sc, h1, l1);
-        hw[k] = h0 | (h1 << 16);
-        lw[k] = l0 | (l1 << 16);
-    }
-    *reinterpret_cast<psalm_u32x4*>(hi_dst) = psalm_u32x4{hw[0], hw[1], hw[2], hw[3]};
-    *reinterpret_cast<psalm_u32x4*>(lo_dst) = psalm_u32x4{lw[0], lw[1], lw[2], lw[3]};
-}
-__device__ __forceinline__ void split_scale(float amax, float& sc, float& inv) {
-    int e = (int)((__builtin_bit_cast(unsigned, amax) >> 23) & 0xffu) - 127;
-    int se = 13 - e;
-    se = se > 100 ? 100 : (se < -100 ? -100 : se);
-    const bool zero = !(amax > 0.f) || !(amax < 3.0e38f);
-    sc = zero ? 1.f : __builtin_bit_cast(float, (unsigned)(127 + se) << 23);
-    inv = zero ? 1.f : __builtin_bit_cast(float, (unsigned)(127 - se) << 23);
-}
 template <typename TI>
 __device__ __forceinline__ void row_stats(const TI* __restrict__ x, int C, int lane, float eps, float& mean, float& rstd) {
     float s = 0.f;
@@ -714,12 +693,23 @@
         for (int k = 0; k < 8; ++k) {
             const int c = c0 + k, g = c / cpg;
             const float m = stats[((long)b * G + g) * 2], r = stats[((long)b * G + g) * 2 + 1];
-            float o = (v[k] - m) * r * gamma[c] + beta[c];
-            if (relu) o = fmaxf(o, 0.f);
-            v[k] = o;
+            v[k] = psalm_gn_elem(v[k], m, r, gamma[c], beta[c], relu);
         }
         st8(y + (long)b * HW * C + e, v);
     }
+}
+
+static int groupnorm_stats_launch(const void* x, int x_dtype, float* workspace, int B, int HW, int C, int G, float eps, hipStream_t s, float** stats_out) {
+    const int rows_per_chunk = 64;
+    const int nchunks = cdiv(HW, rows_per_chunk);
+    float* stats = workspace + (long)B * nchunks * G * 2;
+    PSALM_DISPATCH(x_dtype, TI, {
+        hipLaunchKernelGGL((groupnorm_stats_kernel<TI>), dim3(nchunks, B), dim3(256), 0, s, (const TI*)x, workspace, HW, C, G,
+                           rows_per_chunk, nchunks);
+    });
+    hipLaunchKernelGGL(groupnorm_finalize_kernel, dim3(G, B), dim3(64), 0, s, workspace, stats, HW, C, G, nchunks, eps);
+    *stats_out = stats;
+    return 0;
 }
 
 extern "C" int psalm_groupnorm_nhwc(const void* x, int x_dtype, void* y, int y_dtype, const float* gamma, const float* beta,
@@ -727,15 +717,9 @@
     if (B == 0 || HW == 0) return 0;
     PSALM_CHECK_ARG(G <= 256 && C % G == 0 && C % 8 == 0, "psalm_groupnorm_nhwc: need G <= 256, C % G == 0, C % 8 == 0");
     PSALM_CHECK_ARG((uintptr_t)x % 16 == 0 && (uintptr_t)y % 16 == 0, "psalm_groupnorm_nhwc: 16-byte aligned tensors");
-    const int rows_per_chunk = 64;
-    const int nchunks = cdiv(HW, rows_per_chunk);
-    float* stats = workspace + (long)B * nchunks * G * 2;
     hipStream_t s = (hipStream_t)stream;
-    PSALM_DISPATCH(x_dtype, TI, {
-        hipLaunchKernelGGL((groupnorm_stats_kernel<TI>), dim3(nchunks, B), dim3(256), 0, s, (const TI*)x, workspace, HW, C, G,
-                           rows_per_chunk, nchunks);
-    });
-    hipLaunchKernelGGL(groupnorm_finalize_kernel, dim3(G, B), dim3(64), 0, s, workspace, stats, HW, C, G, nchunks, eps);
+    float* stats = nullptr;
+    if (groupnorm_stats_launch(x, x_dtype, workspace, B, HW, C, G, eps, s, &stats) != 0) return -1;
     long gx = ((long)HW * C / 8 + 255) / 256;
     if (gx > 8192) gx = 8192;
     PSALM_DISPATCH(x_dtype, TI, PSALM_DISPATCH(y_dtype, TO, {
@@ -743,6 +727,52 @@
                            (TO*)y, stats, gamma, beta, HW, C, G, relu);
     }));
     PSALM_LAUNCH_END("psalm_groupnorm_nhwc");
+}
+
+template <int LPR>
+__global__ void __launch_bounds__(256) groupnorm_apply_split_kernel(const float* __restrict__ x, float* __restrict__ y, const float* __restrict__ stats,
+                                                                    const float* __restrict__ gamma, const float* __restrict__ beta,
+                                                                    unsigned short* __restrict__ sp, float* __restrict__ inv_scale, int HW, int C,
+                                                                    int G, int relu) {
+    constexpr int RPW = 64 / LPR;
+    const int b = blockIdx.y;
+    const int lane = (threadIdx.x & 63) % LPR;
+    const long row = ((long)blockIdx.x * 4 + (threadIdx.x >> 6)) * RPW + (threadIdx.x & 63) / LPR;
+    if (row >= HW) return;
+    const int cpg = C / G, c0 = lane * 8;
+    const long grow = (long)b * HW + row;
+    float v[8];
+    ld8(x + grow * C + c0, v);
+    float amax = 0.f;
+#pragma unroll
+    for (int k = 0; k < 8; ++k) {
+        const int c = c0 + k, g = c / cpg;
+        const float m = stats[((long)b * G + g) * 2], r = stats[((long)b * G + g) * 2 + 1];
+        v[k] = psalm_gn_elem(v[k], m, r, gamma[c], beta[c], relu);
+        amax = fmaxf(amax, fabsf(v[k]));
+    }
+    if (y) st8(y + grow * C + c0, v);
+    float sc, iv;
+    split_scale(seg_max<LPR>(amax), sc, iv);
+    if (lane == 0) inv_scale[grow] = iv;
+    emit_split8(v, sc, sp + grow * 2L * C + c0, sp + grow * 2L * C + C + c0);
+}
+
+extern "C" int psalm_groupnorm_nhwc_split(const float* x, float* y, const float* gamma, const float* beta, float* workspace, void* split_out,
+                                          float* inv_scale, int B, int HW, int C, int G, float eps, int relu, void* stream) {
+    if (B == 0 || HW == 0) return 0;
+    PSALM_CHECK_ARG(G >= 1 && G <= 256 && C % G == 0 && C % 64 == 0 && C <= 512 && (C & (C - 1)) == 0 && B <= 65535,
+                    "psalm_groupnorm_nhwc_split: need G <= 256, C % G == 0, C = 64 / 128 / 256 / 512");
+    PSALM_CHECK_ARG(x && gamma && beta && workspace && split_out && inv_scale && (uintptr_t)x % 16 == 0 && (uintptr_t)y % 16 == 0 &&
+                        (uintptr_t)split_out % 16 == 0, "psalm_groupnorm_nhwc_split: 16-byte aligned tensors");
+    hipStream_t s = (hipStream_t)stream;
+    float* stats = nullptr;
+    if (groupnorm_stats_launch(x, PSALM_F32, workspace, B, HW, C, G, eps, s, &stats) != 0) return -1;
+#define GNS_LAUNCH(LPR_) hipLaunchKernelGGL((groupnorm_apply_split_kernel<LPR_>), dim3(cdiv(HW, 4 * (64 / LPR_)), B), dim3(256), 0, s, x, y, stats, gamma, \
+                                            beta, (unsigned short*)split_out, inv_scale, HW, C, G, relu)
+    if (C == 64) GNS_LAUNCH(8); else if (C == 128) GNS_LAUNCH(16); else if (C == 256) GNS_LAUNCH(32); else GNS_LAUNCH(64);
+#undef GNS_LAUNCH
+    PSALM_LAUNCH_END("psalm_groupnorm_nhwc_split");
 }
 
 template <typename TA, typename TB, typename TO>
@@ -766,6 +796,77 @@
                            (const TB*)b, (TO*)out, rows, C, b_rows);
     })));
     PSALM_LAUNCH_END("psalm_add_bcast");
+}
+
+template <int LPR>
+__global__ void __launch_bounds__(256) rows_split2_kernel(const float* __restrict__ x, long ldx, const float* __restrict__ add_a, long add_a_rows,
+                                                          const float* __restrict__ add_b, long add_b_rows, unsigned short* __restrict__ sa,
+                                                          float* __restrict__ inva, unsigned short* __restrict__ sb, float* __restrict__ invb,
+                                                          long ld_sp, int rows, int C, int Kp) {
+    constexpr int RPW = 64 / LPR, NI = LPR == 64 ? 4 : 1;
+    const int lane = (threadIdx.x & 63) % LPR;
+    const long row = ((long)blockIdx.x * 4 + (threadIdx.x >> 6)) * RPW + (threadIdx.x & 63) / LPR;
+    if (row >= rows) return;
+    const float* xr = x + row * ldx;
+    const float* ar = add_a ? add_a + (row % add_a_rows) * C : nullptr;
+    const float* br = add_b ? add_b + (row % add_b_rows) * C : nullptr;
+    float va[NI][8], vb[NI][8];
+    float ma = 0.f, mb = 0.f;
+#pragma unroll
+    for (int i = 0; i < NI; ++i) {
+        const int c = (i * LPR + lane) * 8;
+#pragma unroll
+        for (int k = 0; k < 8; ++k) { va[i][k] = 0.f; vb[i][k] = 0.f; }
+        if (c < C) {
+            float v[8], d8[8];
+            ld8(xr + c, v);
+#pragma unroll
+            for (int k = 0; k < 8; ++k) va[i][k] = vb[i][k] = v[k];
+            if (ar) {
+                ld8(ar + c, d8);
+#pragma unroll
+                for (int k = 0; k < 8; ++k) va[i][k] = v[k] + d8[k];
+            }
+            if (sb && br) {
+                ld8(br + c, d8);
+#pragma unroll
+                for (int k = 0; k < 8; ++k) vb[i][k] = v[k] + d8[k];
+            }
+#pragma unroll
+            for (int k = 0; k < 8; ++k) { ma = fmaxf(ma, fabsf(va[i][k])); mb = fmaxf(mb, fabsf(vb[i][k])); }
+        }
+    }
+    float sca, iva, scb = 1.f, ivb = 1.f;
+    split_scale(seg_max<LPR>(ma), sca, iva);
+    if (sb) split_scale(seg_max<LPR>(mb), scb, ivb);
+    if (lane == 0) {
+        inva[row] = iva;
+        if (sb) invb[row] = ivb;
+    }
+#pragma unroll
+    for (int i = 0; i < NI; ++i) {
+        const int c = (i * LPR + lane) * 8;
+        if (c < Kp) {
+            emit_split8(va[i], sca, sa + row * ld_sp + c, sa + row * ld_sp + Kp + c);
+            if (sb) emit_split8(vb[i], scb, sb + row * ld_sp + c, sb + row * ld_sp + Kp + c);
+        }
+    }
+}
+
+extern "C" int psalm_rows_split2(const float* x, long ldx, const float* add_a, long add_a_rows, const float* add_b, long add_b_rows, void* sp_a,
+                                 float* inv_a, void* sp_b, float* inv_b, long ld_sp, int rows, int C, void* stream) {
+    if (rows == 0) return 0;
+    const int Kp = (C + 63) / 64 * 64;
+    PSALM_CHECK_ARG(C % 8 == 0 && C > 0 && C <= 2048, "psalm_rows_split2: C % 8 == 0, C <= 2048");
+    PSALM_CHECK_ARG(x && (uintptr_t)x % 16 == 0 && (ldx * 4) % 16 == 0 && (!add_a || ((uintptr_t)add_a % 16 == 0 && add_a_rows > 0)) &&
+                        (!add_b || ((uintptr_t)add_b % 16 == 0 && add_b_rows > 0)), "psalm_rows_split2: 16-byte aligned rows, addend row counts > 0");
+    PSALM_CHECK_ARG(sp_a && inv_a && (uintptr_t)sp_a % 16 == 0 && (!sp_b || (inv_b && (uintptr_t)sp_b % 16 == 0)) && (ld_sp * 2) % 16 == 0 && ld_sp >= 2L * Kp,
+                    "psalm_rows_split2: operand rows of >= 2*ceil64(C) f16, 16-byte aligned, with their scale arrays");
+#define RS2_LAUNCH(LPR_) hipLaunchKernelGGL((rows_split2_kernel<LPR_>), dim3(cdiv(rows, 4 * (64 / LPR_))), dim3(256), 0, (hipStream_t)stream, x, ldx, add_a, \
+                                            add_a_rows, add_b, add_b_rows, (unsigned short*)sp_a, inv_a, (unsigned short*)sp_b, inv_b, ld_sp, rows, C, Kp)
+    if (C <= 128) RS2_LAUNCH(16); else if (C <= 256) RS2_LAUNCH(32); else RS2_LAUNCH(64);
+#undef RS2_LAUNCH
+    PSALM_LAUNCH_END("psalm_rows_split2");
 }
 
 struct GatherSrc { const void* p[4]; int dtype[4]; };
diff --git a/psalm_amd/csrc/stages.hip b/psalm_amd/csrc/stages.hip
--- a/psalm_amd/csrc/stages.hip
+++ b/psalm_amd/csrc/stages.hip
@@ -541,7 +541,11 @@
         PD(psalm_gemm_x3(tokp, 2L * Kp, tokinv, d->ip_w[l], 2L * Kp, d->ip_ws[l], Kp, d->ip_b[l], nullptr, 0, t, D, hwl, D, 0, 0, gemm_workspace, gemm_workspace_bytes, stream));
         PD(psalm_groupnorm_nhwc(t, PSALM_F32, s0 + g.start[l] * D, PSALM_F32, d->ip_gn_g[l], d->ip_gn_b[l], gnws, 1, hwl, D, d->G, eps, 0, stream));
     }
-    PD(psalm_add_bcast(s0, PSALM_F32, lvl_pos, PSALM_F32, qin, PSALM_F32, S, D, S, stream));
+    const bool pdf = psalm_get_tuning(PSALM_TUNE_PD_FUSE) != 0;
+    const bool pdf_rows = pdf && (uintptr_t)lvl_pos % 16 == 0;
+    const bool pdf_msda = pdf && psalm_msda_fused_split_ok(d->M, 32);
+    const bool pdf_gns = pdf && D % 64 == 0 && D <= 512 && (D & (D - 1)) == 0;
+    if (!pdf_rows) PD(psalm_add_bcast(s0, PSALM_F32, lvl_pos, PSALM_F32, qin, PSALM_F32, S, D, S, stream));
     const int64_t shapes[6] = {g.h[3], g.w[3], g.h[2], g.w[2], g.h[1], g.w[1]};
     const int64_t starts[3] = {g.start[0], g.start[1], g.start[2]};
     int cur = 0;
@@ -550,7 +554,11 @@
         const bool more = i + 1 < d->num_layers;
         float* sc = src[cur];
         float* sn = src[cur ^ 1];
-        if (i == 0) {
+        if (i == 0 && pdf_rows) {
+            PD(psalm_rows_split2(sc, D, nullptr, 0, lvl_pos, S, sp2, inv2, sp3, inv3, 2L * KpD, S, D, stream));
+            PD(psalm_gemm_x3(sp2, 2L * KpD, inv2, ly->value_w, 2L * KpD, ly->value_ws, KpD, ly->value_b, nullptr, 0, value, D, S, D, 0, 0, gemm_workspace, gemm_workspace_bytes, stream));
+            PD(psalm_gemm_x3(sp3, 2L * KpD, inv3, ly->ow_w, 2L * KpD, ly->ow_ws, KpD, ly->ow_b, nullptr, 0, ow, NOW, S, NOW, 0, 0, gemm_workspace, gemm_workspace_bytes, stream));
+        } else if (i == 0) {
             PD(psalm_split_f16(sc, D, sp2, 2L * KpD, inv2, S, D, stream));
             PD(psalm_gemm_x3(sp2, 2L * KpD, inv2, ly->value_w, 2L * KpD, ly->value_ws, KpD, ly->value_b, nullptr, 0, value, D, S, D, 0, 0, gemm_workspace, gemm_workspace_bytes, stream));
             PD(psalm_split_f16(qin, D, sp3, 2L * KpD, inv3, S, D, stream));
@@ -559,8 +567,12 @@
             PD(psalm_gemm_x3(sp2, 2L * KpD, inv2, ly->value_w, 2L * KpD, ly->value_ws, KpD, ly->value_b, nullptr, 0, value, D, S, D, 0, 0, gemm_workspace, gemm_workspace_bytes, stream));
             PD(psalm_gemm_x3(sp3, 2L * KpD, inv3, ly->ow_w, 2L * KpD, ly->ow_ws, KpD, ly->ow_b, nullptr, 0, ow, NOW, S, NOW, 0, 0, gemm_workspace, gemm_workspace_bytes, stream));
         }
-        PD(psalm_msda_fused(value, PSALM_F32, shapes, starts, ow, att, PSALM_F32, 1, S, d->M, 32, 3, 4, stream));
-        PD(psalm_split_f16(att, D, sp1, 2L * KpD, inv1, S, D, stream));
+        if (pdf_msda) {
+            PD(psalm_msda_fused_split(value, shapes, starts, ow, sp1, inv1, 1, S, d->M, 32, 3, 4, stream));
+        } else {
+            PD(psalm_msda_fused(value, PSALM_F32, shapes, starts, ow, att, PSALM_F32, 1, S, d->M, 32, 3, 4, stream));
+            PD(psalm_split_f16(att, D, sp1, 2L * KpD, inv1, S, D, stream));
+        }
         PD(psalm_gemm_x3(sp1, 2L * KpD, inv1, ly->out_w, 2L * KpD, ly->out_ws, KpD, ly->out_b, sc, D, x1, D, S, D, 0, 0, gemm_workspace, gemm_workspace_bytes, stream));
         PD(psalm_layernorm_split(x1, D, sn, D, ly->n1_g, ly->n1_b, S, D, eps, sp1, inv1, nullptr, 0, nullptr, nullptr, stream));
         if (Kf != F) PD(psalm_memset_zero(hdd, (long)S * 2 * Kf * 2, stream));
@@ -578,8 +590,12 @@
         PD(psalm_upsample_add_nhwc(lat2, PSALM_F32, ms_out + g.start[2] * D, PSALM_F32, y, PSALM_F32, 1, hs, ws_, H2, W2, D, stream));
         PD(psalm_im2col_split_f16(y, cols, colsinv, 1, H2, W2, D, 3, 1, 1, stream));
         PD(psalm_gemm_x3(cols, 2L * Kp9, colsinv, d->layer_w, 2L * Kp9, d->layer_ws, Kp9, d->layer_b, nullptr, 0, y2, D, HW2, D, 0, 0, gemm_workspace, gemm_workspace_bytes, stream));
-        PD(psalm_groupnorm_nhwc(y2, PSALM_F32, y, PSALM_F32, d->layer_gn_g, d->layer_gn_b, gnws, 1, HW2, D, d->G, eps, 1, stream));
-        PD(psalm_split_f16(y, D, cols, 2L * KpD, colsinv, HW2, D, stream));
+        if (pdf_gns) {
+            PD(psalm_groupnorm_nhwc_split(y2, nullptr, d->layer_gn_g, d->layer_gn_b, gnws, cols, colsinv, 1, HW2, D, d->G, eps, 1, stream));
+        } else {
+            PD(psalm_groupnorm_nhwc(y2, PSALM_F32, y, PSALM_F32, d->layer_gn_g, d->layer_gn_b, gnws, 1, HW2, D, d->G, eps, 1, stream));
+            PD(psalm_split_f16(y, D, cols, 2L * KpD, colsinv, HW2, D, stream));
+        }
         PD(psalm_gemm_x3(cols, 2L * KpD, colsinv, d->mf_w, 2L * KpD, d->mf_ws, KpD, d->mf_b, nullptr, 0, mask_features, d->mask_dim, HW2, d->mask_dim, 0, 0, gemm_workspace,
                          gemm_workspace_bytes, stream));
     }
@@ -587,7 +603,7 @@
     return 0;
 }
 
-struct PrLayout { long kin, vin, sp, spinv, K[3], V[3], mfp, mfinv, dec, me0, me1, me2, mes, mesinv, masks, amask, flags, outq, qp, a, x1, out[2], qk, v, hdd, mha, t0, t1, total; };
+struct PrLayout { long kin, vin, sp, spinv, sp2, spinv2, K[3], V[3], mfp, mfinv, dec, me0, me1, me2, mes, mesinv, masks, amask, flags, outq, qp, a, x1, out[2], qk, v, hdd, mha, t0, t1, total; };
 static PrLayout pr_layout(const psalm_pr_desc* d, const int* hwl, int H2, int W2, int n_extra) {
     const long D = d->D, Q = d->Q, HW2 = (long)H2 * W2;
     long mhw = 0, mmha = 0;
@@ -602,6 +618,7 @@
     o.kin = p; p += al256(mhw * D * 4);
     o.vin = p; p += al256(mhw * D * 4);
     o.sp = p; p += al256(mhw * 2 * c64((int)D) * 2); o.spinv = p; p += al256(mhw * 4);
+    o.sp2 = p; p += al256(mhw * 2 * c64((int)D) * 2); o.spinv2 = p; p += al256(mhw * 4);
     for (int l = 0; l < 3; ++l) {
         const long hw = l < d->num_levels ? (long)hwl[2 * l] * hwl[2 * l + 1] : 0;
         const long nl_l = l < d->num_levels ? (d->num_layers - l + d->num_levels - 1) / d->num_levels : 0;
@@ -637,13 +654,22 @@
     const int D = d->D, nl = d->num_layers, nlev = d->num_levels, HW2 = H2 * W2, MD = d->mask_dim;
     float* kin = (float*)(ws + lo.kin); float* vin = (float*)(ws + lo.vin);
     void* sp = ws + lo.sp; float* spinv = (float*)(ws + lo.spinv);
+    void* sp2 = ws + lo.sp2; float* spinv2 = (float*)(ws + lo.spinv2);
     const int KpD = c64(D), KpM = c64(MD);
+    bool pdf = psalm_get_tuning(PSALM_TUNE_PD_FUSE) != 0 && D <= 2048 && (uintptr_t)d->level_embed % 16 == 0;
+    for (int l = 0; l < nlev; ++l) pdf = pdf && (uintptr_t)ms_host[l] % 16 == 0 && (uintptr_t)prpos_host[l] % 16 == 0;
     int rc;
 #define PR(call) do { rc = (call); if (rc) return rc; } while (0)
     for (int l = 0; l < nlev; ++l) {
         const int hw = hw_levels_host[2 * l] * hw_levels_host[2 * l + 1];
         const int N = ((nl - l + nlev - 1) / nlev) * D;
         float* Kl = (float*)(ws + lo.K[l]); float* Vl = (float*)(ws + lo.V[l]);
+        if (pdf) {
+            PR(psalm_rows_split2(ms_host[l], D, prpos_host[l], hw, d->level_embed + (long)l * D, 1, sp, spinv, sp2, spinv2, 2L * KpD, hw, D, stream));
+            PR(psalm_gemm_x3(sp, 2L * KpD, spinv, d->lvl_k_w[l], 2L * KpD, d->lvl_k_ws[l], KpD, d->lvl_k_b[l], nullptr, 0, Kl, N, hw, N, 0, 0, gemm_workspace, gemm_workspace_bytes, stream));
+            PR(psalm_gemm_x3(sp2, 2L * KpD, spinv2, d->lvl_v_w[l], 2L * KpD, d->lvl_v_ws[l], KpD, d->lvl_v_b[l], nullptr, 0, Vl, N, hw, N, 0, 0, gemm_workspace, gemm_workspace_bytes, stream));
+            continue;
+        }
         PR(psalm_add_bcast(ms_host[l], PSALM_F32, prpos_host[l], PSALM_F32, kin, PSALM_F32, hw, D, hw, stream));
         PR(psalm_add_bcast(ms_host[l], PSALM_F32, d->level_embed + (long)l * D, PSALM_F32, vin, PSALM_F32, hw, D, 1, stream));
         PR(psalm_split_f16(kin, D, sp, 2L * KpD, spinv, hw, D, stream));
diff --git a/psalm_amd/hip_ops.py b/psalm_amd/hip_ops.py
--- a/psalm_amd/hip_ops.py
+++ b/psalm_amd/hip_ops.py
@@ -36,7 +36,7 @@
         raise PsalmHipError(f"unsupported dtype {t.dtype} (float32 / bfloat16 only)")
 
 
-ABI_VERSION = 18
+ABI_VERSION = 19
 
 
 class _ProfiledLib:
@@ -869,6 +869,7 @@
 
     TUNE_GEMM_XCD_KSPLIT, TUNE_ATTN_XCD_HEADS, TUNE_GEMM_MID, TUNE_DECODER_FUSE, TUNE_ROW_GROUPS, TUNE_MHA_QTILE_WAVES = 0, 1, 2, 3, 4, 5
     TUNE_PHI_ROPE_EPILOGUE = 6
+    TUNE_PD_FUSE = 7
 
     def set_tuning(self, key: int, value: int):
         self._check(self.lib.psalm_set_tuning(int(key), int(value)), "psalm_set_tuning")
@@ -1047,6 +1048,34 @@
                                       c_long(b.shape[0]), self._stream())
         self._check(rc, "psalm_add_bcast")
         return out
+
+    def rows_split2(self, x, add_a=None, add_b=None, two=True):
+        rows, C = x.shape
+        if x.dtype != torch.float32 or x.stride(1) != 1:
+            raise PsalmHipError("rows_split2: float32 rows")
+        for a in (add_a, add_b):
+            if a is not None and (a.dtype != torch.float32 or a.dim() != 2 or a.shape[1] != C or not a.is_contiguous()):
+                raise PsalmHipError("rows_split2: contiguous float32 (r, C) addends")
+        Kp = (C + 63) // 64 * 64
+        sa, ia = self.empty(rows, 2 * Kp, dtype=torch.float16), self.empty(rows, dtype=torch.float32)
+        sb, ib = (self.empty(rows, 2 * Kp, dtype=torch.float16), self.empty(rows, dtype=torch.float32)) if two else (None, None)
+        rc = self.lib.psalm_rows_split2(self._pv(x), c_long(x.stride(0)), self._pv(add_a), c_long(add_a.shape[0] if add_a is not None else 0),
+                                        self._pv(add_b), c_long(add_b.shape[0] if add_b is not None else 0), self._p(sa), self._p(ia),
+                                        self._pv(sb), self._pv(ib), c_long(2 * Kp), rows, C, self._stream())
+        self._check(rc, "psalm_rows_split2")
+        return SplitF16(sa, ia, C), (SplitF16(sb, ib, C) if two else None)
+
+    def groupnorm_nhwc_split(self, x, gamma, beta, B, HW, groups, eps=1e-5, relu=False, want_y=False):
+        C = x.shape[-1]
+        if x.dtype != torch.float32:
+            raise PsalmHipError("groupnorm_nhwc_split: float32 rows")
+        y = self.empty(B * HW, C, dtype=torch.float32) if want_y else None
+        t, inv = self.empty(B * HW, 2 * C, dtype=torch.float16), self.empty(B * HW, dtype=torch.float32)
+        ws = self.empty(B * ((HW + 63) // 64 + 1) * groups * 2, dtype=torch.float32)
+        rc = self.lib.psalm_groupnorm_nhwc_split(self._p(x), self._pv(y), self._p(gamma), self._p(beta), self._p(ws), self._p(t), self._p(inv),
+                                                 B, HW, C, groups, c_float(eps), int(relu), self._stream())
+        self._check(rc, "psalm_groupnorm_nhwc_split")
+        return SplitF16(t, inv, C), y
 
     def gather_rows(self, srcs, src_id, src_row, C, out_dtype=torch.float32):
         srcs = list(srcs) + [None] * (4 - len(srcs))
@@ -1590,6 +1619,21 @@
         self._check(rc, "psalm_msda_fused")
         return out
 
+    def msda_fused_split(self, value, spatial_shapes, level_start, offsets_logits, M):
+        B, S, C = value.shape
+        L, P = len(spatial_shapes), 4
+        D = C // M
+        if value.dtype != torch.float32 or offsets_logits.dtype != torch.float32 or offsets_logits.shape[-1] != M * L * P * 3:
+            raise PsalmHipError("msda_fused_split: float32 value, offsets_logits float32 (B,S,M*L*P*3)")
+        if not self._cdll_raw.psalm_msda_fused_split_ok(M, D):
+            raise PsalmHipError("msda_fused_split: M * D / 8 a power of two <= 64, M * D % 64 == 0")
+        t, inv = self.empty(B * S, 2 * C, dtype=torch.float16), self.empty(B * S, dtype=torch.float32)
+        sh = (ctypes.c_int64 * (2 * L))(*[int(x) for hw in spatial_shapes for x in hw])
+        st = (ctypes.c_int64 * L)(*[int(x) for x in level_start])
+        rc = self.lib.psalm_msda_fused_split(self._p(value), sh, st, self._p(offsets_logits), self._p(t), self._p(inv), B, S, M, D, L, P, self._stream())
+        self._check(rc, "psalm_msda_fused_split")
+        return SplitF16(t, inv, C)
+
 
     @staticmethod
     def _want(t, dtype, shape, what):
```

Result: no change. 56.15 images/s (median of 6 runs) (+0.6%).
